# tiems90/mosaic

Measured on AMD Instinct MI355X. Metric: PIP-join points/sec (H3 res 9) at 1/2/4/8 GPUs + achieved HBM GB/s, higher is better.
Workload: dtype f64

## Files before the change

include/mosaic_gpu.h:

```cpp
#ifndef MOSAIC_GPU_H
#define MOSAIC_GPU_H

#include <stdint.h>

#ifdef __cplusplus
extern "C" {
#endif

#define MGPU_OK 0
#define MGPU_E_INVALID_ARG -1
#define MGPU_E_RESOLUTION -2
#define MGPU_E_NAN -3
#define MGPU_E_WKB -4
#define MGPU_E_CAPACITY -5
#define MGPU_E_DEVICE -6
#define MGPU_E_INTERNAL -7
#define MGPU_E_UNSUPPORTED -8
#define MGPU_E_EMPTY -9

#define MGPU_H3 0
#define MGPU_BNG 1

typedef struct mgpu_ctx mgpu_ctx;
typedef struct mgpu_chips mgpu_chips;
// ... 88 lines not shown

int32_t mgpu_grid_polyfill(mgpu_ctx* ctx, int32_t index_system, int32_t res, int64_t n_polys,
                           const int64_t* poly_part_off, const int64_t* part_ring_off, const int64_t* ring_off,
                           const double* xy, int64_t* out_cells, int64_t capacity, int64_t* out_offsets,
                           int64_t* out_total, void* stream);

int32_t mgpu_chips_upload(mgpu_ctx* ctx, int32_t index_system, int64_t n_chips, const int64_t* cell,
                          const int32_t* polygon_id, const uint8_t* is_core, const int64_t* wkb_offsets,
                          const uint8_t* wkb, mgpu_chips** out);
int32_t mgpu_chips_destroy(mgpu_chips* chips);
int32_t mgpu_chips_device_blob(const mgpu_chips* chips, void** device_ptr, int64_t* bytes);
int32_t mgpu_chips_from_device_blob(mgpu_ctx* ctx, const void* device_ptr, int64_t bytes, mgpu_chips** out);
int32_t mgpu_chips_info(const mgpu_chips* chips, int64_t* n_chips, int64_t* n_cells, int64_t* n_vertices);
int32_t mgpu_chips_raster_info(const mgpu_chips* chips, int64_t* mode, int64_t* n_classes);
int32_t mgpu_chips_polygons(const mgpu_chips* chips, int32_t* out_ids, int64_t cap, int64_t* out_n);

int32_t mgpu_chips_host_blob(int32_t index_system, int64_t n_chips, const int64_t* cell, const int32_t* polygon_id,
                             const uint8_t* is_core, const int64_t* wkb_offsets, const uint8_t* wkb, uint8_t** out,
                             int64_t* bytes);
int32_t mgpu_chips_host_blob_ex(int32_t index_system, int64_t n_chips, const int64_t* cell, const int32_t* polygon_id,
                                const uint8_t* is_core, const int64_t* wkb_offsets, const uint8_t* wkb,
                                const mgpu_build_opts* opts, uint8_t** out, int64_t* bytes);
int32_t mgpu_host_free(void* p);
int32_t mgpu_host_blob_info(const void* host_blob, int64_t bytes, int32_t* index_system, int64_t* n_chips,
                            int64_t* n_cells, int64_t* n_vertices);
int32_t mgpu_chips_upload_blob(mgpu_ctx* ctx, const void* host_blob, int64_t bytes, mgpu_chips** out);

#define MGPU_COMM_ID_BYTES 128
int32_t mgpu_comm_unique_id(uint8_t* out_id);
int32_t mgpu_comm_init(mgpu_ctx* ctx, const uint8_t* unique_id, int32_t rank, int32_t world);
int32_t mgpu_comm_info(mgpu_ctx* ctx, int32_t* rank, int32_t* world);
int32_t mgpu_comm_destroy(mgpu_ctx* ctx);
int32_t mgpu_chips_broadcast(mgpu_ctx* ctx, const mgpu_chips* chips, int32_t root, mgpu_chips** out, void* stream);
int32_t mgpu_pair_offsets(mgpu_ctx* ctx, int64_t local_pairs, int64_t* out_offset, int64_t* out_total,
                          int64_t* out_counts, void* stream);
int32_t mgpu_test_receive_blob(mgpu_ctx* ctx, const void* dev_blob, int32_t fail_alloc, mgpu_chips** out);

int32_t mgpu_ring_join(mgpu_ctx* ctx, int32_t index_system, int32_t res, int32_t k, int32_t loop_only,
                       const double* left_x, const double* left_y, int64_t n_left, const double* right_x,
                       const double* right_y, int64_t n_right, int64_t left_id_base, int32_t max_per_left,
                       double max_distance, int64_t capacity, int64_t* out_n, int64_t* out_left, int64_t* out_right,
                       double* out_dist, void* stream);
#define MGPU_RING_LEFT_OUTER 1
int32_t mgpu_ring_join_ex(mgpu_ctx* ctx, int32_t index_system, int32_t res, int32_t k, int32_t loop_only,
                          const double* left_x, const double* left_y, int64_t n_left, const double* right_x,
                          const double* right_y, int64_t n_right, int64_t left_id_base, int32_t max_per_left,
                          double max_distance, int32_t flags, int64_t capacity, int64_t* out_n, int64_t* out_left,
                          int64_t* out_right, double* out_dist, void* stream);
int32_t mgpu_ring_join_final(mgpu_ctx* ctx, int32_t index_system, int32_t res, const double* left_x,
                             const double* left_y, const double* radius, const int32_t* k_iterated, int64_t n_left,
                             const double* right_x, const double* right_y, int64_t n_right, int64_t left_id_base,
                             int32_t max_per_left, double max_distance, int32_t flags, int64_t capacity,
                             int64_t* out_n, int64_t* out_left, int64_t* out_right, double* out_dist, void* stream);

int32_t mgpu_st_contains(mgpu_ctx* ctx, const mgpu_chips* chips, const int64_t* chip_row,
                         const double* x, const double* y, int64_t n, int8_t* out, void* stream);

int32_t mgpu_pip_join(mgpu_ctx* ctx, const mgpu_chips* chips, int32_t index_system, int32_t res,
                      const double* x, const double* y, const int64_t* point_id, int64_t point_id_base,
                      int64_t n, int64_t capacity, int64_t* out_n_pairs, int64_t* out_point_id,
                      int32_t* out_polygon_id, void* stream, mgpu_stats* stats);

int32_t mgpu_pip_join_fetch(mgpu_ctx* ctx, int64_t capacity, int64_t* out_n_pairs, int64_t* out_point_id,
                            int32_t* out_polygon_id, void* stream);

int32_t mgpu_pip_join_count(mgpu_ctx* ctx, const mgpu_chips* chips, int32_t index_system, int32_t res,
                            const double* x, const double* y, const int64_t* weight, int64_t n, int64_t n_slots,
                            int64_t* count, int64_t* sum, int32_t accumulate, void* stream, mgpu_stats* stats);

int32_t mgpu_pip_join_lookup(mgpu_ctx* ctx, const mgpu_chips* chips, int32_t index_system, int32_t res,
                             const double* x, const double* y, int64_t n, int32_t null_id,
                             int32_t* out_polygon, int32_t* out_matches, void* stream, mgpu_stats* stats);

typedef struct mgpu_cell_agg mgpu_cell_agg;
int32_t mgpu_cell_agg_create(mgpu_ctx* ctx, int32_t index_system, int32_t res, int32_t with_sum,
                             int64_t initial_cells, mgpu_cell_agg** out);
int32_t mgpu_cell_agg_add_points(mgpu_ctx* ctx, mgpu_cell_agg* agg, const double* x, const double* y,
                                 const int64_t* weight, int64_t n, void* stream, mgpu_stats* stats);
int32_t mgpu_cell_agg_add_cells(mgpu_ctx* ctx, mgpu_cell_agg* agg, const int64_t* cells, const uint8_t* valid,
                                int64_t valid_offset, const int64_t* weight, int64_t n, void* stream);
int32_t mgpu_cell_agg_add_counted(mgpu_ctx* ctx, mgpu_cell_agg* agg, const int64_t* cells, const int64_t* count,
                                  const int64_t* sum, int64_t n, void* stream);
int32_t mgpu_cell_agg_size(mgpu_ctx* ctx, const mgpu_cell_agg* agg, int64_t* n_cells, void* stream);
int32_t mgpu_cell_agg_fetch(mgpu_ctx* ctx, const mgpu_cell_agg* agg, int64_t capacity, int64_t* out_cell,
                            int64_t* out_count, int64_t* out_sum, int64_t* out_n, void* stream);
int32_t mgpu_cell_agg_clear(mgpu_ctx* ctx, mgpu_cell_agg* agg, void* stream);
int32_t mgpu_cell_agg_destroy(mgpu_cell_agg* agg);

int32_t mgpu_pip_join_async(mgpu_ctx* ctx, const mgpu_chips* chips, int32_t index_system, int32_t res,
                            const double* x, const double* y, const int64_t* point_id, int64_t point_id_base,
                            int64_t n, int64_t capacity, int64_t* d_n_pairs, int64_t* out_point_id,
                            int32_t* out_polygon_id, void* stream);
int32_t mgpu_pip_join_finish(mgpu_ctx* ctx, int64_t* out_n_pairs, mgpu_stats* stats);
int32_t mgpu_ctx_reserve(mgpu_ctx* ctx, int64_t max_points);

int32_t mgpu_last_near_ties(mgpu_ctx* ctx, int64_t* out_index, int64_t cap, int64_t* out_n);

int32_t mgpu_pip_join_host(mgpu_ctx* ctx, const mgpu_chips* chips, int32_t index_system, int32_t res,
                           const double* x, const double* y, const int64_t* point_id, int64_t n,
                           int64_t capacity, int64_t* out_n_pairs, int64_t* out_point_id,
                           int32_t* out_polygon_id);

typedef struct mgpu_tess mgpu_tess;
int32_t mgpu_tessellate(int32_t index_system, int32_t res, int64_t n_polys, const int32_t* polygon_id,
                        const int64_t* poly_part_off, const int64_t* part_ring_off, const int64_t* ring_off,
                        const double* xy, int32_t keep_core_geometries, mgpu_tess** out);
#define MGPU_CORE_MOSAICFILL 0
#define MGPU_CORE_CLIP 1
#define MGPU_CORE_DISTANCE 2
int32_t mgpu_tessellate_ex(int32_t index_system, int32_t res, int64_t n_polys, const int32_t* polygon_id,
                           const int64_t* poly_part_off, const int64_t* part_ring_off, const int64_t* ring_off,
                           const double* xy, int32_t keep_core_geometries, int32_t core_rule, mgpu_tess** out);
#define MGPU_CHIPS_OVERLAY 0
#define MGPU_CHIPS_SUTHERLAND_HODGMAN 1
int32_t mgpu_tessellate_geom(int32_t index_system, int32_t res, int64_t n_polys, const int32_t* polygon_id,
                             const int64_t* poly_part_off, const int64_t* part_ring_off, const int64_t* ring_off,
                             const double* xy, const uint8_t* poly_type, int32_t keep_core_geometries,
                             int32_t core_rule, int32_t chip_geometry, mgpu_tess** out);
int32_t mgpu_tess_result_stats(const mgpu_tess* t, int64_t* out6);
int32_t mgpu_tess_result_core_stats(const mgpu_tess* t, int64_t* out, int32_t n);
int32_t mgpu_tess_result_sizes(const mgpu_tess* t, int64_t* n_chips, int64_t* wkb_bytes);
int32_t mgpu_tess_result_copy(const mgpu_tess* t, int64_t* cell, int32_t* polygon_id, uint8_t* is_core,
                              int64_t* wkb_offsets, uint8_t* wkb);
int32_t mgpu_tess_result_undecided(const mgpu_tess* t, int64_t* n, int64_t* wkb_bytes, int64_t* cell, int32_t* poly,
                                   uint8_t* kind_kept_core, int64_t* wkb_offsets, uint8_t* wkb);
int32_t mgpu_tess_destroy(mgpu_tess* t);

int32_t mgpu_test_chip_contains_host(int32_t index_system, int64_t n_chips, const int64_t* cell,
                                     const int32_t* polygon_id, const uint8_t* is_core, const int64_t* wkb_offsets,
                                     const uint8_t* wkb, int64_t n, const int64_t* chip_row, const double* x,
                                     const double* y, int8_t* out_join_path, int8_t* out_point_locator);

int32_t mgpu_test_overlay_verify(int32_t on, int64_t* out2);

int32_t mgpu_test_parse_number(const char* s, int32_t len, double* out);
int32_t mgpu_test_h3_elementary_host(int32_t fn, const double* a, const double* b, int64_t n, double* out);
int32_t mgpu_test_h3_route_host(const double* lon, const double* lat, int64_t n, int32_t res, int64_t* out_cell);
int32_t mgpu_test_h3_glibc_host(const double* lon, const double* lat, int64_t n, int32_t res, int64_t* out_cell);
int32_t mgpu_test_h3_boundary_host(const int64_t* cells, int64_t n, double* out_lonlat, int32_t* out_nverts,
                                   double* out_center);
int32_t mgpu_test_cell_geometry_host(int32_t index_system, const int64_t* cells, int64_t n, double* out_xy,
                                     int32_t* out_nverts, double* out_center, double* out_area);
int32_t mgpu_test_grid_polyfill_host(int32_t index_system, int32_t res, int64_t n_polys, const int64_t* poly_part_off,
                                     const int64_t* part_ring_off, const int64_t* ring_off, const double* xy,
                                     int64_t* out_cells, int64_t capacity, int64_t* out_offsets, int64_t* out_total);
int32_t mgpu_test_grid_polyfill_last(int64_t* out8);
int32_t mgpu_test_geometry_kring_host(int32_t index_system, int64_t n_geoms, const int64_t* row_off, const int64_t* cell,
                                      const uint8_t* is_core, int32_t k, int32_t loop_only, int64_t* out_cells,
                                      int64_t capacity, int64_t* out_offsets, int64_t* out_total);
int32_t mgpu_test_geometry_kring_last(int64_t* out8);
int32_t mgpu_test_h3_cell_wkb_host(int64_t cell, uint8_t* out, int64_t cap, int64_t* out_len);
int32_t mgpu_test_decode_point(int32_t format, const uint8_t* data, int64_t len, double* x, double* y);
int32_t mgpu_test_join_counters(mgpu_ctx* ctx, uint64_t* out16);
int32_t mgpu_test_poly_slots_host(const int32_t* polygon_id, int64_t n, int32_t* out_ids, int64_t* out_n,
                                  uint32_t* out_slot_of_row);

int32_t mgpu_test_internal_centroid(int64_t n, const int32_t* type_id, const int64_t* row_part, const int64_t* part_ring,
                                    const int64_t* ring_off, const double* xy, double* x, double* y, int32_t* status);

int32_t mgpu_test_blob_contains_host(const void* host_blob, int64_t bytes, int64_t n, const int64_t* chip_row,
                                     const double* x, const double* y, int8_t* out);

int32_t mgpu_test_raster_host(int32_t index_system, int32_t res, int64_t n_chips, const int64_t* cell,
                              const int32_t* polygon_id, const uint8_t* is_core, const int64_t* wkb_offsets,
                              const uint8_t* wkb, int64_t n, const double* x, const double* y, int8_t* out_kind,
                              uint32_t* out_first, uint32_t* out_mask, int32_t* out_chip_poly);

int32_t mgpu_test_cell_answers_host(int32_t index_system, int32_t res, int64_t n_chips, const int64_t* cell,
                                    const int32_t* polygon_id, const uint8_t* is_core, const int64_t* wkb_offsets,
                                    const uint8_t* wkb, int64_t n, const double* x, const double* y, int8_t* out_kind,
                                    uint32_t* out_first, uint32_t* out_mask, int32_t* out_chip_poly);

int32_t mgpu_test_whole_cells_host(int32_t index_system, int32_t res, int64_t n_chips, const int64_t* cell,
                                   const int32_t* polygon_id, const uint8_t* is_core, const int64_t* wkb_offsets,
                                   const uint8_t* wkb, int64_t n, const double* x, const double* y, int8_t* out_kind,
                                   uint32_t* out_first, uint32_t* out_mask, int32_t* out_chip_poly);

#ifdef __cplusplus
}
#endif

#endif
```

mosaic_amd/_native.py:

```python
import ctypes
import os

_HERE = os.path.dirname(os.path.abspath(__file__))
LIB_PATH = os.environ.get("MOSAIC_AMD_LIB") or os.path.join(_HERE, "libmosaic_gpu.so")

MGPU_OK = 0
MGPU_E_INVALID_ARG = -1
MGPU_E_RESOLUTION = -2
MGPU_E_NAN = -3
MGPU_E_WKB = -4
MGPU_E_CAPACITY = -5
MGPU_RING_LEFT_OUTER = 1
MGPU_E_DEVICE = -6
MGPU_E_INTERNAL = -7
MGPU_E_UNSUPPORTED = -8
MGPU_E_EMPTY = -9

MGPU_H3 = 0
MGPU_BNG = 1

EXPORTS = (
    "mgpu_last_error", "mgpu_version", "mgpu_join_tile_points", "mgpu_ctx_create", "mgpu_ctx_destroy", "mgpu_check_resolution",
    "mgpu_points_to_cells", "mgpu_points_to_cells_host", "mgpu_bng_format", "mgpu_bng_parse",
    "mgpu_bng_format_device", "mgpu_format_cells_device", "mgpu_grid_kring",
    "mgpu_chips_upload", "mgpu_chips_destroy", "mgpu_chips_device_blob", "mgpu_chips_from_device_blob",
    "mgpu_chips_info", "mgpu_st_contains", "mgpu_pip_join", "mgpu_pip_join_async", "mgpu_pip_join_finish", "mgpu_ctx_reserve",
    "mgpu_last_near_ties",    "mgpu_pip_join_host", "mgpu_tessellate", "mgpu_tess_result_sizes", "mgpu_tess_result_copy", "mgpu_tessellate_ex", "mgpu_tessellate_geom", "mgpu_tess_result_undecided", "mgpu_tess_result_stats", "mgpu_tess_result_core_stats",
    "mgpu_tess_destroy", "mgpu_test_chip_contains_host", "mgpu_test_raster_host", "mgpu_test_cell_answers_host", "mgpu_test_whole_cells_host", "mgpu_pip_join_fetch",
    "mgpu_chips_host_blob", "mgpu_host_free", "mgpu_host_blob_info", "mgpu_chips_upload_blob",
    "mgpu_comm_unique_id", "mgpu_comm_init", "mgpu_comm_info", "mgpu_comm_destroy", "mgpu_chips_broadcast",
    "mgpu_pair_offsets", "mgpu_test_blob_contains_host", "mgpu_points_from_geometry", "mgpu_geometry_to_cells",
    "mgpu_geometry_to_cells_arrow", "mgpu_pip_join_arrow", "mgpu_test_parse_number", "mgpu_test_decode_point",
    "mgpu_test_h3_elementary_host", "mgpu_test_h3_route_host", "mgpu_test_h3_boundary_host", "mgpu_test_h3_cell_wkb_host",
    "mgpu_ctx_set_option", "mgpu_ctx_get_option", "mgpu_build_opts_default", "mgpu_chips_host_blob_ex",
    "mgpu_test_h3_glibc_host", "mgpu_internal_geometry_to_cells", "mgpu_test_internal_centroid", "mgpu_test_join_counters",
    "mgpu_test_receive_blob", "mgpu_ring_join", "mgpu_ring_join_ex", "mgpu_ring_join_final",
    "mgpu_test_overlay_verify",
    "mgpu_chips_polygons", "mgpu_pip_join_count", "mgpu_test_poly_slots_host", "mgpu_chips_raster_info",
    "mgpu_pip_join_lookup",
    "mgpu_cell_agg_create", "mgpu_cell_agg_add_points", "mgpu_cell_agg_add_cells", "mgpu_cell_agg_add_counted",
    "mgpu_cell_agg_size", "mgpu_cell_agg_fetch", "mgpu_cell_agg_clear", "mgpu_cell_agg_destroy",
    "mgpu_cells_to_centers", "mgpu_cells_to_boundaries", "mgpu_cells_boundary_wkb", "mgpu_cells_area",
    "mgpu_test_cell_geometry_host",
    "mgpu_grid_polyfill", "mgpu_test_grid_polyfill_last", "mgpu_test_grid_polyfill_host",
    "mgpu_geometry_kring", "mgpu_test_geometry_kring_host", "mgpu_test_geometry_kring_last",
)
MGPU_GEOM_WKB = 0
MGPU_GEOM_WKT = 1
MGPU_GEOM_HEX = 2
MGPU_GEOM_GEOJSON = 3
MGPU_COMM_ID_BYTES = 128
MGPU_PIPELINE_AUTO = -1
MGPU_PIPELINE_FUSED = 0
MGPU_PIPELINE_SPLIT = 1
MGPU_PIPELINE_BINNED = 2
MGPU_LIBM_REFERENCE = 0
MGPU_LIBM_CORRECTLY_ROUNDED = 1


class MosaicGpuError(RuntimeError):

    def __init__(self, code, msg):
        super().__init__("%s (status %d)" % (msg, code))
        self.code = code


class IllegalArgumentException(MosaicGpuError, ValueError):
    pass


class IllegalStateException(MosaicGpuError):
    pass


class CapacityError(MosaicGpuError):
    def __init__(self, code, msg, required):
        super().__init__(code, msg)
        self.required = required


class MgpuStats(ctypes.Structure):
    _fields_ = [("n_points", ctypes.c_int64), ("n_pairs", ctypes.c_int64), ("n_near_ties", ctypes.c_int64),
                ("n_candidates", ctypes.c_int64), ("kernel_ms", ctypes.c_float),
                ("stream_kernel_ms", ctypes.c_float), ("mixed_kernel_ms", ctypes.c_float),
                ("emit_kernel_ms", ctypes.c_float), ("pipeline", ctypes.c_int32), ("libm_overrides", ctypes.c_int32)]

    def as_dict(self):
        return {k: getattr(self, k) for k, _ in self._fields_}


class BuildOpts(ctypes.Structure):
    _fields_ = [("raster", ctypes.c_int32), ("raster_bng", ctypes.c_int32), ("raster_sub", ctypes.c_int32),
                ("raster_milli", ctypes.c_int32)]


_lib = None

P = ctypes.c_void_p
I32 = ctypes.c_int32
I64 = ctypes.c_int64


def lib():
    global _lib
    if _lib is not None:
        return _lib
    if not os.path.exists(LIB_PATH):
        raise RuntimeError("mosaic_amd/libmosaic_gpu.so is not built: run `python -c 'import __graft_entry__ as g; "
                           "g.build()'` (the HIP path has no CPU fallback)")
    L = ctypes.CDLL(LIB_PATH)
    sig = {
        "mgpu_last_error": (ctypes.c_char_p, []),
        "mgpu_version": (ctypes.c_char_p, []),
        "mgpu_join_tile_points": (ctypes.c_int32, []),
        "mgpu_ctx_create": (I32, [I32, ctypes.POINTER(P)]),
        "mgpu_ctx_destroy": (I32, [P]),
        "mgpu_check_resolution": (I32, [I32, I32]),
        "mgpu_points_to_cells": (I32, [P, I32, I32, P, P, I64, P, P, ctypes.POINTER(MgpuStats)]),
        "mgpu_points_to_cells_host": (I32, [P, I32, I32, P, P, I64, P]),
        "mgpu_bng_format": (I32, [P, I64, P, I64, P]),
        "mgpu_bng_format_device": (I32, [P, P, I64, P, I64, P, ctypes.POINTER(I64), P]),
        "mgpu_format_cells_device": (I32, [P, I32, P, I64, P, I64, P, ctypes.POINTER(I64), P]),
        "mgpu_grid_kring": (I32, [P, I32, P, I64, I32, I32, P, I64, P, ctypes.POINTER(I64), P]),
        "mgpu_bng_parse": (I32, [P, P, I64, P]),
        "mgpu_chips_upload": (I32, [P, I32, I64, P, P, P, P, P, ctypes.POINTER(P)]),
        "mgpu_chips_destroy": (I32, [P]),
        "mgpu_chips_device_blob": (I32, [P, ctypes.POINTER(P), ctypes.POINTER(I64)]),
        "mgpu_chips_from_device_blob": (I32, [P, P, I64, ctypes.POINTER(P)]),
        "mgpu_chips_info": (I32, [P, ctypes.POINTER(I64), ctypes.POINTER(I64), ctypes.POINTER(I64)]),
        "mgpu_chips_raster_info": (I32, [P, ctypes.POINTER(I64), ctypes.POINTER(I64)]),
        "mgpu_st_contains": (I32, [P, P, P, P, P, I64, P, P]),
        "mgpu_pip_join": (I32, [P, P, I32, I32, P, P, P, I64, I64, I64, ctypes.POINTER(I64), P, P, P,
                                ctypes.POINTER(MgpuStats)]),
        "mgpu_pip_join_async": (I32, [P, P, I32, I32, P, P, P, I64, I64, I64, P, P, P, P]),
        "mgpu_pip_join_finish": (I32, [P, ctypes.POINTER(I64), ctypes.POINTER(MgpuStats)]),
        "mgpu_ctx_reserve": (I32, [P, I64]),
        "mgpu_last_near_ties": (I32, [P, P, I64, ctypes.POINTER(I64)]),
        "mgpu_pip_join_host": (I32, [P, P, I32, I32, P, P, P, I64, I64, ctypes.POINTER(I64), P, P]),
        "mgpu_tessellate": (I32, [I32, I32, I64, P, P, P, P, P, I32, ctypes.POINTER(P)]),
        "mgpu_tessellate_ex": (I32, [I32, I32, I64, P, P, P, P, P, I32, I32, ctypes.POINTER(P)]),
        "mgpu_tessellate_geom": (I32, [I32, I32, I64, P, P, P, P, P, P, I32, I32, I32, ctypes.POINTER(P)]),
        "mgpu_tess_result_undecided": (I32, [P, P, P, P, P, P, P, P]),
        "mgpu_tess_result_stats": (I32, [P, P]),
        "mgpu_tess_result_core_stats": (I32, [P, P, I32]),
        "mgpu_tess_result_sizes": (I32, [P, ctypes.POINTER(I64), ctypes.POINTER(I64)]),
        "mgpu_tess_result_copy": (I32, [P, P, P, P, P, P]),
        "mgpu_tess_destroy": (I32, [P]),
        "mgpu_test_chip_contains_host": (I32, [I32, I64, P, P, P, P, P, I64, P, P, P, P, P]),
        "mgpu_pip_join_fetch": (I32, [P, I64, ctypes.POINTER(I64), P, P, P]),
        "mgpu_test_raster_host": (I32, [I32, I32, I64, P, P, P, P, P, I64, P, P, P, P, P, P]),
        "mgpu_test_cell_answers_host": (I32, [I32, I32, I64, P, P, P, P, P, I64, P, P, P, P, P, P]),
        "mgpu_test_whole_cells_host": (I32, [I32, I32, I64, P, P, P, P, P, I64, P, P, P, P, P, P]),
        "mgpu_chips_host_blob": (I32, [I32, I64, P, P, P, P, P, ctypes.POINTER(P), ctypes.POINTER(I64)]),
        "mgpu_host_free": (I32, [P]),
        "mgpu_host_blob_info": (I32, [P, I64, ctypes.POINTER(I32), ctypes.POINTER(I64), ctypes.POINTER(I64),
                                      ctypes.POINTER(I64)]),
        "mgpu_chips_upload_blob": (I32, [P, P, I64, ctypes.POINTER(P)]),
        "mgpu_comm_unique_id": (I32, [P]),
        "mgpu_comm_init": (I32, [P, P, I32, I32]),
        "mgpu_comm_info": (I32, [P, ctypes.POINTER(I32), ctypes.POINTER(I32)]),
        "mgpu_comm_destroy": (I32, [P]),
        "mgpu_chips_broadcast": (I32, [P, P, I32, ctypes.POINTER(P), P]),
        "mgpu_pair_offsets": (I32, [P, I64, ctypes.POINTER(I64), ctypes.POINTER(I64), P, P]),
        "mgpu_test_blob_contains_host": (I32, [P, I64, I64, P, P, P, P]),
        "mgpu_points_from_geometry": (I32, [P, I32, P, P, P, I64, I64, P, P, P]),
        "mgpu_geometry_to_cells": (I32, [P, I32, I32, I32, P, P, P, I64, I64, P, P, P, ctypes.POINTER(MgpuStats)]),
        "mgpu_geometry_to_cells_arrow": (I32, [P, I32, I32, P, P, P, P, P]),
        "mgpu_pip_join_arrow": (I32, [P, P, I32, I32, P, P, P, I64, ctypes.POINTER(I64), P, P, P,
                                      ctypes.POINTER(MgpuStats)]),
        "mgpu_test_parse_number": (I32, [ctypes.c_char_p, I32, ctypes.POINTER(ctypes.c_double)]),
        "mgpu_test_decode_point": (I32, [I32, P, I64, ctypes.POINTER(ctypes.c_double), ctypes.POINTER(ctypes.c_double)]),
        "mgpu_test_h3_elementary_host": (I32, [I32, P, P, I64, P]),
        "mgpu_test_h3_route_host": (I32, [P, P, I64, I32, P]),
        "mgpu_test_h3_boundary_host": (I32, [P, I64, P, P, P]),
        "mgpu_test_overlay_verify": (I32, [ctypes.c_int32, P]),
        "mgpu_test_h3_cell_wkb_host": (I32, [I64, P, I64, P]),
        "mgpu_ctx_set_option": (I32, [P, ctypes.c_char_p, I64]),
        "mgpu_ctx_get_option": (I32, [P, ctypes.c_char_p, ctypes.POINTER(I64)]),
        "mgpu_build_opts_default": (None, [ctypes.POINTER(BuildOpts)]),
        "mgpu_chips_host_blob_ex": (I32, [I32, I64, P, P, P, P, P, ctypes.POINTER(BuildOpts), ctypes.POINTER(P),
                                          ctypes.POINTER(I64)]),
        "mgpu_test_h3_glibc_host": (I32, [P, P, I64, I32, P]),
        "mgpu_internal_geometry_to_cells": (I32, [P, I32, I32, I64, P, P, P, P, P, P, I64, P, P, P,
                                                  ctypes.POINTER(MgpuStats)]),
        "mgpu_test_internal_centroid": (I32, [I64, P, P, P, P, P, P, P, P]),
        "mgpu_test_join_counters": (I32, [P, P]),
        "mgpu_test_receive_blob": (I32, [P, P, I32, ctypes.POINTER(P)]),
        "mgpu_chips_polygons": (I32, [P, P, I64, ctypes.POINTER(I64)]),
        "mgpu_pip_join_count": (I32, [P, P, I32, I32, P, P, P, I64, I64, P, P, I32, P, ctypes.POINTER(MgpuStats)]),
        "mgpu_pip_join_lookup": (I32, [P, P, I32, I32, P, P, I64, I32, P, P, P, ctypes.POINTER(MgpuStats)]),
        "mgpu_test_poly_slots_host": (I32, [P, I64, P, ctypes.POINTER(I64), P]),
        "mgpu_cell_agg_create": (I32, [P, I32, I32, I32, I64, ctypes.POINTER(P)]),
        "mgpu_cell_agg_add_points": (I32, [P, P, P, P, P, I64, P, ctypes.POINTER(MgpuStats)]),
        "mgpu_cell_agg_add_cells": (I32, [P, P, P, P, I64, P, I64, P]),
        "mgpu_cell_agg_add_counted": (I32, [P, P, P, P, P, I64, P]),
        "mgpu_cell_agg_size": (I32, [P, P, ctypes.POINTER(I64), P]),
        "mgpu_cell_agg_fetch": (I32, [P, P, I64, P, P, P, ctypes.POINTER(I64), P]),
        "mgpu_cell_agg_clear": (I32, [P, P, P]),
        "mgpu_cell_agg_destroy": (I32, [P]),
        "mgpu_cells_to_centers": (I32, [P, I32, P, P, I64, I64, P, P, P, P]),
        "mgpu_cells_to_boundaries": (I32, [P, I32, P, P, I64, I64, P, P, P, P]),
        "mgpu_cells_boundary_wkb": (I32, [P, I32, P, P, I64, I64, P, I64, P, ctypes.POINTER(I64), P, P]),
        "mgpu_cells_area": (I32, [P, I32, P, P, I64, I64, P, P, P]),
        "mgpu_test_cell_geometry_host": (I32, [I32, P, I64, P, P, P, P]),
        "mgpu_grid_polyfill": (I32, [P, I32, I32, I64, P, P, P, P, P, I64, P, ctypes.POINTER(I64), P]),
        "mgpu_test_grid_polyfill_last": (I32, [P]),
        "mgpu_test_grid_polyfill_host": (I32, [I32, I32, I64, P, P, P, P, P, I64, P, ctypes.POINTER(I64)]),
        "mgpu_geometry_kring": (I32, [P, I32, I64, P, P, P, I32, I32, P, I64, P, ctypes.POINTER(I64), P]),
        "mgpu_test_geometry_kring_host": (I32, [I32, I64, P, P, P, I32, I32, P, I64, P, ctypes.POINTER(I64)]),
        "mgpu_test_geometry_kring_last": (I32, [P]),
        "mgpu_ring_join": (I32, [P, I32, I32, I32, I32, P, P, I64, P, P, I64, I64, I32, ctypes.c_double, I64,
                                 ctypes.POINTER(I64), P, P, P, P]),
        "mgpu_ring_join_ex": (I32, [P, I32, I32, I32, I32, P, P, I64, P, P, I64, I64, I32, ctypes.c_double, I32,
                                    I64, ctypes.POINTER(I64), P, P, P, P]),
        "mgpu_ring_join_final": (I32, [P, I32, I32, P, P, P, P, I64, P, P, I64, I64, I32, ctypes.c_double, I32, I64,
                                       ctypes.POINTER(I64), P, P, P, P]),
    }
    for name, (rt, args) in sig.items():
        f = getattr(L, name)
        f.restype = rt
        f.argtypes = args
    _lib = L
    return L


def last_error():
    m = lib().mgpu_last_error()
    return m.decode() if m else ""


def check(status, what="", required=None):
    if status == MGPU_OK:
        return
    msg = last_error() or what
    if status == MGPU_E_CAPACITY:
        raise CapacityError(status, msg, required)
    if status in (MGPU_E_RESOLUTION, MGPU_E_NAN, MGPU_E_INTERNAL, MGPU_E_EMPTY):
        raise IllegalStateException(status, msg)
    if status in (MGPU_E_INVALID_ARG, MGPU_E_WKB):
        raise IllegalArgumentException(status, msg)
    raise MosaicGpuError(status, msg)
```

mosaic_amd/chips.py:

```python
import ctypes

import numpy as np

from . import _native as N


class ChipTable:

    def __init__(self, cell, polygon_id, is_core, wkb_offsets, wkb, index_system=N.MGPU_H3):
        self.cell = np.ascontiguousarray(cell, dtype=np.int64)
        self.polygon_id = np.ascontiguousarray(polygon_id, dtype=np.int32)
        self.is_core = np.ascontiguousarray(is_core, dtype=np.uint8)
        self.wkb_offsets = np.ascontiguousarray(wkb_offsets, dtype=np.int64)
        self.wkb = np.ascontiguousarray(np.frombuffer(wkb, dtype=np.uint8) if isinstance(wkb, (bytes, bytearray))
                                        else wkb, dtype=np.uint8)
        self.index_system = int(index_system)
        n = self.cell.shape[0]
        assert self.polygon_id.shape[0] == n and self.is_core.shape[0] == n and self.wkb_offsets.shape[0] == n + 1

    def __len__(self):
        return self.cell.shape[0]

    def row(self, i):
        b, e = self.wkb_offsets[i], self.wkb_offsets[i + 1]
        return (bool(self.is_core[i]), int(self.cell[i]), bytes(self.wkb[b:e]) if e > b else None,
                int(self.polygon_id[i]))

    @classmethod
    def from_rows(cls, rows, index_system=N.MGPU_H3):
        rows = list(rows)
        blobs = [r[2] or b"" for r in rows]
        off = np.zeros(len(rows) + 1, dtype=np.int64)
        off[1:] = np.cumsum([len(b) for b in blobs])
        return cls([r[1] for r in rows], [r[3] for r in rows], [1 if r[0] else 0 for r in rows], off,
                   np.frombuffer(b"".join(blobs) or b"", dtype=np.uint8), index_system)

    def upload(self, ctx=None):
        from .context import default_context
        return DeviceChips(self, ctx or default_context())

    def stats(self):
        return {"chips": len(self), "core": int(self.is_core.sum()), "cells": int(np.unique(self.cell).shape[0]),
                "wkb_bytes": int(self.wkb_offsets[-1])}


class DeviceChips:

    def __init__(self, table, ctx, handle=None):
        self.ctx = ctx
        self.table = table
        if handle is None:
            h = ctypes.c_void_p()
            wkb = table.wkb if table.wkb.size else np.zeros(1, np.uint8)
            N.check(N.lib().mgpu_chips_upload(ctx.handle, table.index_system, len(table), table.cell.ctypes.data,
                                              table.polygon_id.ctypes.data, table.is_core.ctypes.data,
                                              table.wkb_offsets.ctypes.data, wkb.ctypes.data, ctypes.byref(h)))
            handle = h
        self.handle = handle

    @classmethod
    def from_device_blob(cls, ctx, ptr, nbytes, table=None):
        h = ctypes.c_void_p()
        N.check(N.lib().mgpu_chips_from_device_blob(ctx.handle, ptr, int(nbytes), ctypes.byref(h)))
        return cls(table, ctx, handle=h)

    def device_blob(self):
        p = ctypes.c_void_p()
        b = ctypes.c_int64()
        N.check(N.lib().mgpu_chips_device_blob(self.handle, ctypes.byref(p), ctypes.byref(b)))
        return p.value, b.value

    def info(self):
        a, b, c = ctypes.c_int64(), ctypes.c_int64(), ctypes.c_int64()
        N.check(N.lib().mgpu_chips_info(self.handle, ctypes.byref(a), ctypes.byref(b), ctypes.byref(c)))
        p, n = self.device_blob()
        m, k = ctypes.c_int64(), ctypes.c_int64()
        N.check(N.lib().mgpu_chips_raster_info(self.handle, ctypes.byref(m), ctypes.byref(k)))
        return {"chips": a.value, "cells": b.value, "vertices": c.value, "bytes": n, "raster_mode": m.value,
                "raster_ncls": k.value}

    def polygons(self):
        if getattr(self, "_polygons", None) is not None:
            return self._polygons
        n = ctypes.c_int64()
        st = N.lib().mgpu_chips_polygons(self.handle, None, 0, ctypes.byref(n))
        if st != N.MGPU_E_CAPACITY:
            N.check(st)
        ids = np.zeros(n.value, np.int32)
        N.check(N.lib().mgpu_chips_polygons(self.handle, ids.ctypes.data, n.value, ctypes.byref(n)))
        ids.setflags(write=False)
        self._polygons = ids
        return ids

    def polygons_device(self):
        import torch
        if getattr(self, "_polygons_dev", None) is None:
            self._polygons_dev = torch.from_numpy(self.polygons().copy()).to(self.ctx.device)
        return self._polygons_dev

    def close(self):
        if self.handle:
            N.lib().mgpu_chips_destroy(self.handle)
            self.handle = None

    def __del__(self):
        try:
            self.close()
        except Exception:
            pass


class Polygons:

    def __init__(self, poly_id, poly_part_off, part_ring_off, ring_off, xy, poly_type=None):
        self.poly_id = np.ascontiguousarray(poly_id, dtype=np.int32)
        self.poly_part_off = np.ascontiguousarray(poly_part_off, dtype=np.int64)
        self.part_ring_off = np.ascontiguousarray(part_ring_off, dtype=np.int64)
        self.ring_off = np.ascontiguousarray(ring_off, dtype=np.int64)
        self.xy = np.ascontiguousarray(xy, dtype=np.float64).reshape(-1, 2)
        self.poly_type = None if poly_type is None else np.ascontiguousarray(poly_type, dtype=np.uint8)
        assert self.poly_type is None or self.poly_type.shape[0] == self.poly_id.shape[0]

    def __len__(self):
        return self.poly_id.shape[0]

    @classmethod
    def from_npz(cls, path):
        z = np.load(path, allow_pickle=False)
        return cls(z["poly_id"], z["poly_part_off"], z["part_ring_off"], z["ring_off"], z["xy"],
                   z["poly_type"] if "poly_type" in z.files else None)

    @classmethod
    def from_lists(cls, polys, poly_type=None):
        ids, pp, pr, ro, xy = [], [0], [0], [0], []
        for pid, parts in polys:
            ids.append(pid)
            for part in parts:
                for ring in part:
                    xy.extend(ring)
                    ro.append(len(xy))
                pr.append(len(ro) - 1)
            pp.append(len(pr) - 1)
        return cls(ids, pp, pr, ro, np.array(xy, dtype=np.float64).reshape(-1, 2), poly_type)

    def select(self, idx):
        out = []
        for p in idx:
            parts = []
            for q in range(self.poly_part_off[p], self.poly_part_off[p + 1]):
                rings = []
                for r in range(self.part_ring_off[q], self.part_ring_off[q + 1]):
                    rings.append([tuple(v) for v in self.xy[self.ring_off[r]:self.ring_off[r + 1]]])
                parts.append(rings)
            out.append((int(self.poly_id[p]), parts))
        return Polygons.from_lists(out, None if self.poly_type is None else self.poly_type[list(idx)])

    def bounds(self):
        return self.xy[:, 0].min(), self.xy[:, 1].min(), self.xy[:, 0].max(), self.xy[:, 1].max()


CORE_RULES = {"mosaicfill": 0, "clip": 1, "distance": 2}
CORE_STATS = ("rows", "core", "demoted", "promoted", "dropped", "ambiguous", "carved_tests", "band_tests",
              "core_below_r", "border_above_r", "band_dropped", "dp_sensitive", "unresolved", "carved_empty",
              "overlay_chips", "multi_piece", "coerced", "coerce_nodes", "lower_dim")
CHIP_GEOMETRY = {"overlay": 0, "sutherland_hodgman": 1}


def tessellate(polygons, index_system, resolution, keep_core_geometries=True, core_rule="mosaicfill",
               chip_geometry="overlay"):
    res = index_system.get_resolution(resolution)
    L = N.lib()
    h = ctypes.c_void_p()
    p = polygons
    st = L.mgpu_tessellate_geom(index_system.code, res, len(p), p.poly_id.ctypes.data, p.poly_part_off.ctypes.data,
                                p.part_ring_off.ctypes.data, p.ring_off.ctypes.data, p.xy.ctypes.data,
                                None if p.poly_type is None else p.poly_type.ctypes.data,
                                1 if keep_core_geometries else 0, CORE_RULES[core_rule],
                                CHIP_GEOMETRY[chip_geometry], ctypes.byref(h))
    N.check(st, "tessellation failed")
    try:
        stats = np.zeros(len(CORE_STATS), np.int64)
        N.check(L.mgpu_tess_result_core_stats(h, stats.ctypes.data, len(CORE_STATS)))
        n, b = ctypes.c_int64(), ctypes.c_int64()
        N.check(L.mgpu_tess_result_sizes(h, ctypes.byref(n), ctypes.byref(b)))
        cell = np.zeros(n.value, np.int64)
        pid = np.zeros(n.value, np.int32)
        core = np.zeros(n.value, np.uint8)
        off = np.zeros(n.value + 1, np.int64)
        wkb = np.zeros(max(b.value, 1), np.uint8)
        N.check(L.mgpu_tess_result_copy(h, cell.ctypes.data, pid.ctypes.data, core.ctypes.data, off.ctypes.data,
                                        wkb.ctypes.data))
        nu, ub = ctypes.c_int64(), ctypes.c_int64()
        N.check(L.mgpu_tess_result_undecided(h, ctypes.byref(nu), ctypes.byref(ub), None, None, None, None, None))
        ucell, upoly = np.zeros(nu.value, np.int64), np.zeros(nu.value, np.int32)
        ukkc, uoff, uwkb = np.zeros((nu.value, 3), np.uint8), np.zeros(nu.value + 1, np.int64), np.zeros(max(ub.value, 1), np.uint8)
        N.check(L.mgpu_tess_result_undecided(h, ctypes.byref(nu), ctypes.byref(ub), ucell.ctypes.data, upoly.ctypes.data,
                                             ukkc.ctypes.data, uoff.ctypes.data, uwkb.ctypes.data))
    finally:
        L.mgpu_tess_destroy(h)
    t = ChipTable(cell, pid, core, off, wkb[:b.value], index_system.code)
    t.core_stats = dict(zip(CORE_STATS, stats.tolist()))
    t.undecided = ChipTable(ucell, upoly, ukkc[:, 2], uoff, uwkb[:ub.value], index_system.code)
    t.undecided.kind, t.undecided.kept = ukkc[:, 0].copy(), ukkc[:, 1].copy()
    return t
```

mosaic_amd/csrc/capi.cpp:

```cpp
#include <hip/hip_runtime.h>

#include <algorithm>
#include <cmath>
#include <cstdarg>
#include <cstdio>
#include <cstring>
#include <cstdlib>
#include <string>
#include <memory>
#include <functional>
#include <mutex>
#include <vector>

#include "../../include/mosaic_arrow.h"
#include "../../include/mosaic_gpu.h"
#include "error.h"
#include "h3_core.h"
#include "kernels.h"
#include "parallel.h"
#include "poly_slots.h"
#include "capi_internal.h"
#include "chip_build.h"
#include "geom_decode.h"
#include "h3_glibc.h"
// ... 111 lines not shown
  }
  return hipStreamSynchronize(s);
}

struct TieRec {
  int64_t pos;
  double x, y;
  uint64_t key;
};

int32_t read_ties(mgpu_ctx* ctx, int64_t n, std::vector<TieRec>& out) {
  out.resize((size_t)n);
  const uint64_t* head = ctx->pin + 16;
  const int64_t nh = std::min(n, kTqHead);
  if (nh) memcpy(out.data(), head + 2, (size_t)nh * 32);
  if (n > nh) HIP_TRY(hipMemcpy(out.data() + nh, ctx->tq + 2 + 4 * nh, (size_t)(n - nh) * 32, hipMemcpyDeviceToHost));
  return MGPU_OK;
}

std::vector<std::pair<int64_t, uint64_t>> libm_reference_keys(std::vector<TieRec>& ties, int res) {
  std::sort(ties.begin(), ties.end(), [](const TieRec& a, const TieRec& b) { return a.pos < b.pos; });
  std::vector<std::pair<int64_t, uint64_t>> out(ties.size());
  mgpu::parallel_for((int64_t)ties.size(), 256, [&](int64_t b, int64_t e, int) {
    for (int64_t k = b; k < e; k++) out[k] = {ties[k].pos, mgpu::h3glibc::lattice_key(ties[k].x, ties[k].y, res)};
  });
  return out;
}

std::vector<std::pair<int64_t, uint64_t>> libm_second_opinion(const std::vector<TieRec>& ties, int res, bool cells) {
  std::vector<uint64_t> ref(ties.size());
  mgpu::parallel_for((int64_t)ties.size(), 256, [&](int64_t b, int64_t e, int) {
    for (int64_t k = b; k < e; k++)
      ref[k] = cells ? mgpu::h3glibc::point_to_cell(ties[k].x, ties[k].y, res)
                     : mgpu::h3glibc::lattice_key(ties[k].x, ties[k].y, res);
  });
  std::vector<std::pair<int64_t, uint64_t>> diff;
  for (size_t k = 0; k < ties.size(); k++)
    if (ref[k] != ties[k].key) diff.push_back({ties[k].pos, ref[k]});
  std::sort(diff.begin(), diff.end());
  return diff;
}

int32_t check_res(int32_t is, int32_t res) {
  if (is == MGPU_H3) {
    if (res < 0 || res > 15) return fail(MGPU_E_RESOLUTION, "H3 resolution has to be between 0 and 15; found %d", res);
    return MGPU_OK;
  }
  if (is == MGPU_BNG) {
    if (res == 0 || res < -6 || res > 6) return fail(MGPU_E_RESOLUTION, "BNG resolution not supported; found %d", res);
    return MGPU_OK;
  }
  return fail(MGPU_E_INVALID_ARG, "unknown index system %d (0 = H3, 1 = BNG)", is);
}

int32_t set_device(int dev) {
  HIP_TRY(hipSetDevice(dev));
  return MGPU_OK;
}

}

namespace mgpu {
int32_t begin_call(mgpu_ctx* ctx) {
  if (int32_t st = set_device(ctx->device)) return st;
  return ensure_ws(ctx, 1);
}
}

extern "C" {

const char* mgpu_last_error(void) { return g_err.c_str(); }
const char* mgpu_version(void) { return "mosaic-mi355x 0.1.0 (gfx950)"; }
int32_t mgpu_join_tile_points(void) { return (int32_t)mgpu::join_tile_points(); }

int32_t mgpu_check_resolution(int32_t index_system, int32_t res) { return check_res(index_system, res); }

int32_t mgpu_ctx_create(int32_t device_id, mgpu_ctx** out) {
  if (!out) return fail(MGPU_E_INVALID_ARG, "out is NULL");
  int n = 0;
  HIP_TRY(hipGetDeviceCount(&n));
  if (device_id < 0 || device_id >= n) return fail(MGPU_E_INVALID_ARG, "device %d not present (%d GPUs)", device_id, n);
  HIP_TRY(hipSetDevice(device_id));
  mgpu_ctx* c = new mgpu_ctx();
  c->device = device_id;
  int32_t st = MGPU_OK;
  if (hipEventCreate(&c->ev0) != hipSuccess || hipEventCreate(&c->ev1) != hipSuccess ||
      hipEventCreate(&c->ev2) != hipSuccess || hipEventCreate(&c->ev3) != hipSuccess ||
      hipHostMalloc((void**)&c->pin, kPinWords * 8, hipHostMallocDefault) != hipSuccess)
    st = fail(MGPU_E_DEVICE, "mgpu_ctx_create: events / pinned page");
  if (!st && hipHostGetDevicePointer((void**)&c->pin_dev, c->pin, 0) != hipSuccess)
    st = fail(MGPU_E_DEVICE, "mgpu_ctx_create: the pinned page is not device-visible");
  if (!st) st = ensure_ws(c, 1);
  if (!st) st = ensure_tq(c, kTqInit);
  if (st) {
    mgpu_ctx_destroy(c);
    return st;
  }
  *out = c;
  return MGPU_OK;
}

int32_t mgpu_ctx_destroy(mgpu_ctx* ctx) {
  if (!ctx) return MGPU_OK;
  mgpu_comm_destroy(ctx);
  hipSetDevice(ctx->device);
  if (ctx->split_ws) hipFree(ctx->split_ws);
  if (ctx->bin_ws) hipFree(ctx->bin_ws);
  if (ctx->scratch) hipFree(ctx->scratch);
  if (ctx->redo) hipFree(ctx->redo);
  if (ctx->tq) hipFree(ctx->tq);
  if (ctx->ovr) hipFree(ctx->ovr);
  if (ctx->ws) hipFree(ctx->ws);
  if (ctx->pin) hipHostFree(ctx->pin);
  if (ctx->ev0) hipEventDestroy(ctx->ev0);
  if (ctx->ev1) hipEventDestroy(ctx->ev1);
  if (ctx->ev2) hipEventDestroy(ctx->ev2);
  if (ctx->ev3) hipEventDestroy(ctx->ev3);
  delete ctx;
  return MGPU_OK;
}

int32_t mgpu_ctx_set_option(mgpu_ctx* ctx, const char* key, int64_t v) {
  if (!ctx || !key) return fail(MGPU_E_INVALID_ARG, "ctx/key is NULL");
  mgpu_options& o = ctx->opt;
  const std::string k = key;
  auto bad = [&]() { return fail(MGPU_E_INVALID_ARG, "option %s: value %lld out of range", key, (long long)v); };
  if (k == "h3_libm") {
    if (v != MGPU_LIBM_REFERENCE && v != MGPU_LIBM_CORRECTLY_ROUNDED) return bad();
    o.h3_libm = v;
  } else if (k == "pipeline") {
    if (v < MGPU_PIPELINE_AUTO || v > MGPU_PIPELINE_BINNED) return bad();
    o.pipeline = v;
  } else if (k == "bin_count") {
    if (v < 1 || v > mgpu::bin_max()) return bad();
    o.bin_count = v;
  } else if (k == "bin_min_mb") {
    if (v < 0) return bad();
    o.bin_min_mb = v;
  } else if (k == "bin_min_points") {
    if (v < 0) return bad();
    o.bin_min_points = v;
  } else if (k == "bin_xcd") {
    if (v != 0 && v != 1) return bad();
    o.bin_xcd = v;
  } else if (k == "bin_keys") {
    if (v != 0 && v != 1) return bad();
    o.bin_keys = v;
  } else if (k == "ring_batch") {
    if (v < 1) return bad();
    o.ring_batch = v;
  } else if (k == "bng_split") {
    if (v != 0 && v != 1) return bad();
    o.bng_split = v;
  } else if (k == "count_lds_slots") {
    if (v < 0 || v > mgpu::kCountLdsSlotsMax) return bad();
    o.count_lds_slots = v;
  } else if (k == "count_groups") {
    if (v < 0 || v > mgpu::kCountGroupsMax) return bad();
    o.count_groups = v;
  } else if (k == "cellagg_groups") {
    if (v < 0 || v > mgpu::kCountGroupsMax) return bad();
    o.cellagg_groups = v;
  } else if (k == "cellagg_bin_min") {
    if (v < 0) return bad();
    o.cellagg_bin_min = v;
  } else if (k == "cellagg_lds") {
    if (v != 0 && v != 1) return bad();
    o.cellagg_lds = v;
  } else if (k == "kring_batch") {
    if (v < 0 || v > 2147483647LL) return bad();
    o.kring_batch = v;
  } else if (k == "polyfill_slab") {
    if (v < 256 || v > ((int64_t)1 << 28)) return bad();
    o.polyfill_slab = v;
  } else if (k == "geomring_slab") {
    if (v < 1 || v > ((int64_t)1 << 24)) return bad();
    o.geomring_slab = v;
  } else if (k == "geomring_lds_slots") {
    if (v != 0 && v < 64) return bad();
    o.geomring_lds_slots = v;
  } else if (k == "spin_us") {
    if (v < 0 || v > 10000000) return bad();
    o.spin_us = v;
  } else if (k == "raster" || k == "raster_bng") {
    if (v != 0 && v != 1) return bad();
    (k == "raster" ? o.raster : o.raster_bng) = v;
  } else if (k == "raster_sub") {
    if (!(v == 0 || (v >= 2 && v <= 16))) return bad();
    o.raster_sub = v;
  } else if (k == "raster_milli") {
    if (v < 10 || v > 1000) return bad();
    o.raster_milli = v;
  } else {
    return fail(MGPU_E_INVALID_ARG, "unknown option %s", key);
  }
  return MGPU_OK;
}

int32_t mgpu_ctx_get_option(const mgpu_ctx* ctx, const char* key, int64_t* v) {
  if (!ctx || !key || !v) return fail(MGPU_E_INVALID_ARG, "NULL argument");
  const mgpu_options& o = ctx->opt;
  const std::pair<const char*, int64_t> all[] = {
      {"h3_libm", o.h3_libm},       {"pipeline", o.pipeline}, {"bin_count", o.bin_count},
      {"bin_min_mb", o.bin_min_mb}, {"bin_min_points", o.bin_min_points}, {"bin_xcd", o.bin_xcd},
      {"bin_keys", o.bin_keys},     {"spin_us", o.spin_us},   {"ring_batch", o.ring_batch},       {"raster", o.raster},     {"raster_bng", o.raster_bng},
      {"bng_split", o.bng_split},   {"count_lds_slots", o.count_lds_slots}, {"count_groups", o.count_groups},
      {"kring_batch", o.kring_batch}, {"cellagg_groups", o.cellagg_groups}, {"cellagg_lds", o.cellagg_lds}, {"cellagg_bin_min", o.cellagg_bin_min},
      {"raster_sub", o.raster_sub}, {"raster_milli", o.raster_milli}, {"polyfill_slab", o.polyfill_slab},
      {"geomring_slab", o.geomring_slab}, {"geomring_lds_slots", o.geomring_lds_slots}};
  for (const auto& kv : all)
    if (strcmp(kv.first, key) == 0) {
      *v = kv.second;
      return MGPU_OK;
    }
  return fail(MGPU_E_INVALID_ARG, "unknown option %s", key);
}

int32_t mgpu_ctx_reserve(mgpu_ctx* ctx, int64_t max_points) {
  if (!ctx) return fail(MGPU_E_INVALID_ARG, "ctx is NULL");
  if (int32_t st = set_device(ctx->device)) return st;
  const int64_t tiles = mgpu::join_tiles(max_points);
  return ensure_ws(ctx, tiles, max_points);
}

}

int32_t cells_impl(mgpu_ctx* ctx, int32_t is, int32_t res, const double* x, const double* y, int64_t n,
                          int64_t* out_cell, hipStream_t s, const uint8_t* valid, int64_t voff, mgpu_stats* stats) {
  auto* counters = (unsigned long long*)ctx->ws;
  auto* ties = (unsigned long long*)((uint8_t*)ctx->ws + ws_layout(1, 0).ties);
  int64_t n_ties = 0, n_fixed = 0;
  for (int attempt = 0;; attempt++) {
    HIP_TRY(hipMemsetAsync(counters, 0, kWsCounters, s));
    HIP_TRY(hipMemsetAsync(ties, 0, 8, s));
    HIP_TRY(hipMemsetAsync(ctx->tq, 0, 16, s));
    HIP_TRY(hipEventRecord(ctx->ev0, s));
    HIP_TRY(mgpu::launch_cells(is, res, x, y, n, out_cell, counters, ties, kTieCap, ctx->tq, ctx->tq_cap, s, valid, voff));
    HIP_TRY(hipEventRecord(ctx->ev1, s));
    HIP_TRY(hipMemcpyAsync(ctx->pin, counters, 16 * 8, hipMemcpyDeviceToHost, s));
    HIP_TRY(hipMemcpyAsync(ctx->pin + 16, ctx->tq, (2 + 4 * kTqHead) * 8, hipMemcpyDeviceToHost, s));
    HIP_TRY(stream_wait(ctx, s));
    if (ctx->pin[2]) {
      if (is == MGPU_BNG) return fail(MGPU_E_NAN, "NaN coordinates are not supported. (%llu points)", (unsigned long long)ctx->pin[2]);
      return fail(MGPU_E_INVALID_ARG, "Latitude or longitude were invalid. (%llu points)", (unsigned long long)ctx->pin[2]);
    }
    n_ties = (int64_t)ctx->pin[16];
    if (n_ties > ctx->tq_cap) {
      if (attempt >= 2) return fail(MGPU_E_INTERNAL, "near-tie queue overflowed twice");
      if (int32_t st = ensure_tq(ctx, n_ties + n_ties / 4 + 1024)) return st;
      continue;
    }
    break;
  }
  if (stats) {
    memset(stats, 0, sizeof *stats);
    stats->n_points = n;
    stats->n_near_ties = n_ties;
    float ms = 0;
    hipEventElapsedTime(&ms, ctx->ev0, ctx->ev1);
    stats->kernel_ms = stats->stream_kernel_ms = ms;
  }
  if (is == MGPU_H3 && n_ties > 0 && ctx->opt.h3_libm == MGPU_LIBM_REFERENCE) {
    std::vector<TieRec> tr;
    if (int32_t st = read_ties(ctx, n_ties, tr)) return st;
    const auto diff = libm_second_opinion(tr, res, true);
    n_fixed = (int64_t)diff.size();
    if (n_fixed) {
      std::vector<int64_t> hv(2 * diff.size());
      for (size_t k = 0; k < diff.size(); k++) hv[k] = diff[k].first, hv[diff.size() + k] = (int64_t)diff[k].second;
      if (int32_t st = ensure_ovr(ctx, (int64_t)hv.size())) return st;
      HIP_TRY(hipMemcpyAsync(ctx->ovr, hv.data(), hv.size() * 8, hipMemcpyHostToDevice, s));
      HIP_TRY(mgpu::launch_scatter_i64((const int64_t*)ctx->ovr, (const int64_t*)ctx->ovr + n_fixed, n_fixed, out_cell, s));
      HIP_TRY(stream_wait(ctx, s));
    }
  }
  if (stats) stats->libm_overrides = (int32_t)n_fixed;
  return MGPU_OK;
}

extern "C" {

int32_t mgpu_points_to_cells(mgpu_ctx* ctx, int32_t is, int32_t res, const double* x, const double* y, int64_t n,
                             int64_t* out_cell, void* stream, mgpu_stats* stats) {
  if (!ctx) return fail(MGPU_E_INVALID_ARG, "ctx is NULL");
  if (int32_t r = check_res(is, res)) return r;
  if (n < 0 || (n > 0 && (!x || !y || !out_cell))) return fail(MGPU_E_INVALID_ARG, "bad point arrays");
  if (int32_t st = set_device(ctx->device)) return st;
  if (int32_t st = ensure_ws(ctx, 1)) return st;
  return cells_impl(ctx, is, res, x, y, n, out_cell, (hipStream_t)stream, nullptr, 0, stats);
}

int32_t mgpu_format_cells_device(mgpu_ctx* ctx, int32_t index_system, const int64_t* cells, int64_t n, char* out,
                                 int64_t out_bytes, int64_t* out_offsets, int64_t* out_total, void* stream) {
  if (!ctx || n < 0 || (n > 0 && (!cells || !out)) || !out_offsets || out_bytes < 0)
    return fail(MGPU_E_INVALID_ARG, "format_cells_device: bad arguments");
  if (index_system != MGPU_H3 && index_system != MGPU_BNG)
    return fail(MGPU_E_INVALID_ARG, "unknown index system %d (0 = H3, 1 = BNG)", index_system);
  if (int32_t st = set_device(ctx->device)) return st;
  hipStream_t s = (hipStream_t)stream;
  if (int32_t st = ensure_ws(ctx, mgpu::join_tiles(n))) return st;
  auto* counters = (unsigned long long*)ctx->ws;
  auto* chunk = (int64_t*)((uint8_t*)ctx->ws + ws_layout(mgpu::join_tiles(n), 0).where);
  HIP_TRY(hipMemsetAsync(counters, 0, kWsCounters, s));
  HIP_TRY(mgpu::launch_format_cells(index_system, cells, n, out, out_bytes, out_offsets, chunk, counters, s));
  unsigned long long h[4] = {0};
  int64_t total = 0;
  HIP_TRY(hipMemcpyAsync(h, counters, sizeof h, hipMemcpyDeviceToHost, s));
  HIP_TRY(hipMemcpyAsync(&total, out_offsets + n, sizeof total, hipMemcpyDeviceToHost, s));
  HIP_TRY(hipStreamSynchronize(s));
  if (out_total) *out_total = total;
  if (h[2]) return fail(MGPU_E_INVALID_ARG, "%llu BNG cell ids have no string form", h[2]);
  if (total > out_bytes) return fail(MGPU_E_CAPACITY, "format_cells_device: %lld bytes needed, %lld given",
                                     (long long)total, (long long)out_bytes);
  return MGPU_OK;
}

int32_t mgpu_grid_kring(mgpu_ctx* ctx, int32_t index_system, const int64_t* cells, int64_t n, int32_t k,
                        int32_t loop_only, int64_t* out_cells, int64_t capacity, int64_t* out_offsets,
                        int64_t* out_total, void* stream) {
  if (!ctx || n < 0 || (n > 0 && !cells) || !out_offsets || capacity < 0 || (capacity > 0 && !out_cells))
    return fail(MGPU_E_INVALID_ARG, "grid_kring: bad arguments");
  if (index_system != MGPU_BNG && index_system != MGPU_H3)
    return fail(MGPU_E_INVALID_ARG, "grid_kring: unknown index system %d", index_system);
  if (k < 0 || k > 1024) return fail(MGPU_E_INVALID_ARG, "grid_kring: k must be in [0, 1024]");
  if (int32_t st = set_device(ctx->device)) return st;
  hipStream_t s = (hipStream_t)stream;
  if (int32_t st = ensure_ws(ctx, mgpu::join_tiles(n))) return st;
  const WsLayout L = ws_layout(mgpu::join_tiles(n), 0);
  auto* base = (uint8_t*)ctx->ws;
  auto* counters = (unsigned long long*)base;
  auto* chunk = (int64_t*)(base + L.where);
  auto* mc = (int64_t*)(base + L.recs);
  auto* fb_idx = (uint32_t*)(base + L.recs + (size_t)std::max<int64_t>(n, 1) * 8);
  HIP_TRY(hipMemsetAsync(counters, 0, kWsCounters, s));
  HIP_TRY(mgpu::launch_kring_count(index_system, cells, n, k, loop_only, mc, chunk, fb_idx, counters, s));
  unsigned long long h[6] = {0};
  HIP_TRY(hipMemcpyAsync(h, counters, sizeof h, hipMemcpyDeviceToHost, s));
  HIP_TRY(hipStreamSynchronize(s));
  if (h[2] && index_system == MGPU_H3)
    return fail(MGPU_E_INVALID_ARG, "%llu cells are not H3 cell ids", h[2]);
  if (h[2])
    return fail(MGPU_E_INVALID_ARG, "%llu cells are not BNG cells or reach ids BNGIndexSystem.isValid cannot parse "
                "(NumberFormatException in the reference)", h[2]);
  const int64_t n_fb = (int64_t)h[3];
  uint64_t* scratch = nullptr;
  struct Free {
    uint64_t*& p;
    ~Free() {
      if (p) hipFree(p);
    }
  } free_scratch{scratch};
  int64_t batch = 0;
  if (n_fb) {
    const int64_t words = mgpu::kring_fallback_words(k);
    batch = std::max<int64_t>(1, std::min<int64_t>(n_fb, ((int64_t)256 << 20) / 8 / words));
    if (ctx->opt.kring_batch > 0) batch = std::min(batch, ctx->opt.kring_batch);
    HIP_TRY(hipMalloc(&scratch, (size_t)batch * words * 8));
    for (int64_t j0 = 0; j0 < n_fb; j0 += batch)
      HIP_TRY(mgpu::launch_kring_fallback(cells, fb_idx, j0, std::min(n_fb, j0 + batch), k, loop_only, mc, chunk,
                                          out_offsets, out_cells, capacity, scratch, 0, counters, s));
  }
  HIP_TRY(mgpu::launch_kring_write(index_system, cells, n, k, loop_only, mc, chunk, out_offsets, out_cells, capacity,
                                   s));
  for (int64_t j0 = 0; j0 < n_fb; j0 += batch)
    HIP_TRY(mgpu::launch_kring_fallback(cells, fb_idx, j0, std::min(n_fb, j0 + batch), k, loop_only, mc, chunk,
                                        out_offsets, out_cells, capacity, scratch, 1, counters, s));
  int64_t total = 0;
  HIP_TRY(hipMemcpyAsync(h, counters, sizeof h, hipMemcpyDeviceToHost, s));
  HIP_TRY(hipMemcpyAsync(&total, out_offsets + n, sizeof total, hipMemcpyDeviceToHost, s));
  HIP_TRY(hipStreamSynchronize(s));
  if (out_total) *out_total = total;
  if (h[4])
    return fail(MGPU_E_INTERNAL, "grid_kring: %llu pentagon walks overflowed their hash set (inconsistent tables)", h[4]);
  if (total > capacity)
    return fail(MGPU_E_CAPACITY, "grid_kring: %lld ids, capacity %lld", (long long)total, (long long)capacity);
  return MGPU_OK;
}

int32_t mgpu_bng_format_device(mgpu_ctx* ctx, const int64_t* cells, int64_t n, char* out, int64_t out_bytes,
                               int64_t* out_offsets, int64_t* out_total, void* stream) {
  return mgpu_format_cells_device(ctx, MGPU_BNG, cells, n, out, out_bytes, out_offsets, out_total, stream);
}

int32_t mgpu_points_to_cells_host(mgpu_ctx* ctx, int32_t is, int32_t res, const double* x, const double* y, int64_t n,
                                  int64_t* out_cell) {
  if (!ctx) return fail(MGPU_E_INVALID_ARG, "ctx is NULL");
  if (n == 0) return check_res(is, res);
  if (int32_t st = set_device(ctx->device)) return st;
  double *dx = nullptr, *dy = nullptr;
  int64_t* dc = nullptr;
  HIP_TRY(hipMalloc(&dx, n * 8));
  HIP_TRY(hipMalloc(&dy, n * 8));
  HIP_TRY(hipMalloc(&dc, n * 8));
  HIP_TRY(hipMemcpy(dx, x, n * 8, hipMemcpyHostToDevice));
  HIP_TRY(hipMemcpy(dy, y, n * 8, hipMemcpyHostToDevice));
  int32_t st = mgpu_points_to_cells(ctx, is, res, dx, dy, n, dc, nullptr, nullptr);
  if (st == MGPU_OK) HIP_TRY(hipMemcpy(out_cell, dc, n * 8, hipMemcpyDeviceToHost));
  hipFree(dx);
  hipFree(dy);
  hipFree(dc);
  return st;
}


}

static mgpu_build_opts build_opts_of(const mgpu_ctx* ctx) {
  mgpu_build_opts o;
  o.raster = (int32_t)ctx->opt.raster;
  o.raster_bng = (int32_t)ctx->opt.raster_bng;
  o.raster_sub = (int32_t)ctx->opt.raster_sub;
  o.raster_milli = (int32_t)ctx->opt.raster_milli;
  return o;
}

namespace mgpu {
int32_t adopt_device_blob(mgpu_ctx* ctx, void* dev_blob, int64_t bytes, mgpu_chips** out) {
  BlobHeader hdr;
  HIP_TRY(hipMemcpy(&hdr, dev_blob, sizeof hdr, hipMemcpyDeviceToHost));
  if (int32_t st = check_header(hdr, bytes)) return st;
  mgpu_chips* ch = new mgpu_chips();
  ch->device = ctx->device;
  ch->blob = dev_blob;
  ch->bytes = (size_t)bytes;
  ch->index_system = hdr.index_system;
  ch->view = view_from_header(hdr, (uint8_t*)ch->blob);
  ch->n_vertices = hdr.n_vertices;
  *out = ch;
  return MGPU_OK;
}
}

struct PolySlotsDev {
  std::vector<int32_t> ids;
  int32_t* d_ids = nullptr;
  uint32_t* d_chip_slot = nullptr;
  uint32_t* d_dense = nullptr;
};

static std::mutex g_slots_mu;

static void free_poly_slots(mgpu_chips* chips) {
  auto* ps = (PolySlotsDev*)chips->slots;
  if (!ps) return;
  if (ps->d_ids) hipFree(ps->d_ids);
  if (ps->d_chip_slot) hipFree(ps->d_chip_slot);
  if (ps->d_dense) hipFree(ps->d_dense);
  delete ps;
  chips->slots = nullptr;
}

static int32_t ensure_poly_slots(const mgpu_chips* chips, const PolySlotsDev** out) {
  std::lock_guard<std::mutex> lock(g_slots_mu);
  if (chips->slots) {
    *out = (const PolySlotsDev*)chips->slots;
    return MGPU_OK;
  }
  if (int32_t st = set_device(chips->device)) return st;
  const int64_t nch = chips->view.n_chips;
  std::vector<int32_t> poly((size_t)nch);
  if (nch) HIP_TRY(hipMemcpy(poly.data(), chips->view.chip_poly, (size_t)nch * 4, hipMemcpyDeviceToHost));
  mgpu::PolySlots hs = mgpu::poly_slots(poly.data(), nch);
  auto ps = std::make_unique<PolySlotsDev>();
  auto upload = [&](auto** d, const void* src, size_t bytes) -> hipError_t {
    if (hipError_t e = hipMalloc((void**)d, std::max<size_t>(bytes, 4))) return e;
    return bytes ? hipMemcpy(*d, src, bytes, hipMemcpyHostToDevice) : hipSuccess;
  };
  hipError_t e = upload(&ps->d_ids, hs.ids.data(), hs.ids.size() * 4);
  if (e == hipSuccess) e = upload(&ps->d_chip_slot, hs.slot_of_row.data(), hs.slot_of_row.size() * 4);
  if (e == hipSuccess && mgpu::poly_slots_dense(hs.ids)) {
    std::vector<uint32_t> dense((size_t)((int64_t)hs.ids.back() - hs.ids.front() + 1), 0u);
    for (size_t k = 0; k < hs.ids.size(); k++) dense[(size_t)((int64_t)hs.ids[k] - hs.ids.front())] = (uint32_t)k;
    e = upload(&ps->d_dense, dense.data(), dense.size() * 4);
  }
  if (e != hipSuccess) {
    if (ps->d_ids) hipFree(ps->d_ids);
    if (ps->d_chip_slot) hipFree(ps->d_chip_slot);
    if (ps->d_dense) hipFree(ps->d_dense);
    return fail(MGPU_E_DEVICE, "polygon slots: %s", hipGetErrorString(e));
  }
  ps->ids = std::move(hs.ids);
  chips->slots = ps.release();
  *out = (const PolySlotsDev*)chips->slots;
  return MGPU_OK;
}

static hipError_t stage_to_device(void* d, size_t bytes, const std::function<void(uint8_t*, size_t, size_t)>& fill) {
  constexpr size_t kPiece = (size_t)64 << 20;
  if (bytes <= 2 * kPiece) {
    std::vector<uint8_t> tmp(bytes);
    mgpu::parallel_for((int64_t)((bytes + (1 << 20) - 1) >> 20), 1, [&](int64_t b, int64_t en, int) {
      const size_t lo = (size_t)b << 20, hi = std::min(bytes, (size_t)en << 20);
      fill(tmp.data() + lo, lo, hi - lo);
    });
    return hipMemcpy(d, tmp.data(), bytes, hipMemcpyHostToDevice);
  }
  void* stage[2] = {nullptr, nullptr};
  hipEvent_t done[2] = {nullptr, nullptr};
  hipStream_t s = nullptr;
  hipError_t e = hipStreamCreateWithFlags(&s, hipStreamNonBlocking);
  for (int k = 0; k < 2 && e == hipSuccess; k++) {
    e = hipHostMalloc(&stage[k], kPiece, hipHostMallocDefault);
    if (e == hipSuccess) e = hipEventCreateWithFlags(&done[k], hipEventDisableTiming);
  }
  for (size_t off = 0, k = 0; off < bytes && e == hipSuccess; off += kPiece, k ^= 1) {
    const size_t n = std::min(kPiece, bytes - off);
    if (off >= 2 * kPiece) e = hipEventSynchronize(done[k]);
    if (e != hipSuccess) break;
    auto* dst = (uint8_t*)stage[k];
    mgpu::parallel_for((int64_t)((n + (1 << 20) - 1) >> 20), 1, [&](int64_t b, int64_t en, int) {
      const size_t lo = (size_t)b << 20, hi = std::min(n, (size_t)en << 20);
      fill(dst + lo, off + lo, hi - lo);
    });
    e = hipMemcpyAsync((uint8_t*)d + off, stage[k], n, hipMemcpyHostToDevice, s);
    if (e == hipSuccess) e = hipEventRecord(done[k], s);
  }
  if (s) {
    const hipError_t e2 = hipStreamSynchronize(s);
    if (e == hipSuccess) e = e2;
    hipStreamDestroy(s);
  }
  for (int k = 0; k < 2; k++) {
    if (done[k]) hipEventDestroy(done[k]);
    if (stage[k]) hipHostFree(stage[k]);
  }
  return e;
}

extern "C" {

int32_t mgpu_chips_upload_blob(mgpu_ctx* ctx, const void* host_blob, int64_t bytes, mgpu_chips** out) {
  if (!ctx || !out) return fail(MGPU_E_INVALID_ARG, "ctx/out is NULL");
  if (int32_t st = mgpu_host_blob_info(host_blob, bytes, nullptr, nullptr, nullptr, nullptr)) return st;
  if (int32_t st = set_device(ctx->device)) return st;
  void* d = nullptr;
  HIP_TRY(hipMalloc(&d, (size_t)bytes));
  hipError_t e = stage_to_device(d, (size_t)bytes, [&](uint8_t* dst, size_t off, size_t n) {
    memcpy(dst, (const uint8_t*)host_blob + off, n);
  });
  if (e != hipSuccess) {
    hipFree(d);
    return fail(MGPU_E_DEVICE, "hipMemcpy: %s", hipGetErrorString(e));
  }
  int32_t st = mgpu::adopt_device_blob(ctx, d, bytes, out);
  if (st) hipFree(d);
  return st;
}

int32_t mgpu_chips_upload(mgpu_ctx* ctx, int32_t index_system, int64_t n_chips, const int64_t* cell,
                          const int32_t* polygon_id, const uint8_t* is_core, const int64_t* wkb_offsets,
                          const uint8_t* wkb, mgpu_chips** out) {
  if (!ctx || !out) return fail(MGPU_E_INVALID_ARG, "ctx/out is NULL");
  mgpu::HostBlob host;
  mgpu::BlobHeader hdr;
  if (int32_t st = set_device(ctx->device)) return st;
  void* d = nullptr;
  size_t bytes = 0;
  const mgpu::BlobSink sink = [&](size_t total, const std::vector<mgpu::BlobPiece>& pieces) -> int32_t {
    BLOB_T0();
    HIP_TRY(hipMalloc(&d, total));
    BLOB_MARK("sink:malloc");
    bytes = total;
    const hipError_t e = stage_to_device(d, total, [&](uint8_t* dst, size_t off, size_t n) {
      mgpu::fill_from_pieces(pieces, dst, off, n);
    });
    if (e != hipSuccess) return fail(MGPU_E_DEVICE, "hipMemcpy: %s", hipGetErrorString(e));
    return MGPU_OK;
  };
  BLOB_T0();
  int32_t st = mgpu::build_blob(index_system, n_chips, cell, polygon_id, is_core, wkb_offsets, wkb, host, hdr,
                                build_opts_of(ctx), &sink);
  BLOB_MARK("upl:build");
  if (st == MGPU_OK) st = mgpu::adopt_device_blob(ctx, d, (int64_t)bytes, out);
  BLOB_MARK("upl:adopt");
  if (st && d) hipFree(d);
  return st;
}

int32_t mgpu_chips_destroy(mgpu_chips* chips) {
  if (!chips) return MGPU_OK;
  hipSetDevice(chips->device);
  if (chips->blob) hipFree(chips->blob);
  free_poly_slots(chips);
  delete chips;
  return MGPU_OK;
}

int32_t mgpu_chips_info(const mgpu_chips* chips, int64_t* n_chips, int64_t* n_cells, int64_t* n_vertices) {
  if (!chips) return fail(MGPU_E_INVALID_ARG, "chips is NULL");
  if (n_chips) *n_chips = chips->view.n_chips;
  if (n_cells) *n_cells = chips->view.n_cells;
  if (n_vertices) *n_vertices = chips->n_vertices;
  return MGPU_OK;
}

int32_t mgpu_chips_raster_info(const mgpu_chips* chips, int64_t* mode, int64_t* n_classes) {
  if (!chips) return fail(MGPU_E_INVALID_ARG, "chips is NULL");
  if (mode) *mode = chips->view.raster_mode;
  if (n_classes) *n_classes = chips->view.raster_mode != mgpu::kRasterNone ? (int64_t)chips->view.raster_ncls : 0;
  return MGPU_OK;
}

int32_t mgpu_chips_device_blob(const mgpu_chips* chips, void** device_ptr, int64_t* bytes) {
  if (!chips || !device_ptr || !bytes) return fail(MGPU_E_INVALID_ARG, "NULL argument");
  *device_ptr = chips->blob;
  *bytes = (int64_t)chips->bytes;
  return MGPU_OK;
}

int32_t mgpu_chips_from_device_blob(mgpu_ctx* ctx, const void* device_ptr, int64_t bytes, mgpu_chips** out) {
  if (!ctx || !device_ptr || !out || bytes <= 0) return fail(MGPU_E_INVALID_ARG, "NULL argument");
  if (int32_t st = set_device(ctx->device)) return st;
  if (bytes < (int64_t)mgpu::kBlobHeaderBytes) return fail(MGPU_E_INVALID_ARG, "blob too small");
  mgpu::BlobHeader hdr;
  HIP_TRY(hipMemcpy(&hdr, device_ptr, sizeof hdr, hipMemcpyDeviceToHost));
  if (int32_t st = mgpu::check_header(hdr, bytes)) return st;
  void* d = nullptr;
  HIP_TRY(hipMalloc(&d, bytes));
  hipError_t e = hipMemcpy(d, device_ptr, bytes, hipMemcpyDeviceToDevice);
  if (e != hipSuccess) {
    hipFree(d);
    return fail(MGPU_E_DEVICE, "hipMemcpy: %s", hipGetErrorString(e));
  }
  int32_t st = mgpu::adopt_device_blob(ctx, d, bytes, out);
  if (st) hipFree(d);
  return st;
}

int32_t mgpu_st_contains(mgpu_ctx* ctx, const mgpu_chips* chips, const int64_t* chip_row, const double* x,
                         const double* y, int64_t n, int8_t* out, void* stream) {
  if (!ctx || !chips) return fail(MGPU_E_INVALID_ARG, "ctx/chips is NULL");
  if (n < 0 || (n > 0 && (!chip_row || !x || !y || !out))) return fail(MGPU_E_INVALID_ARG, "bad arrays");
  if (int32_t st = set_device(ctx->device)) return st;
  if (chips->device != ctx->device)
    return fail(MGPU_E_INVALID_ARG, "chip table lives on device %d, context on device %d", chips->device, ctx->device);
  hipStream_t s = (hipStream_t)stream;
  if (int32_t st = ensure_ws(ctx, 1)) return st;
  auto* counters = (unsigned long long*)ctx->ws;
  HIP_TRY(hipMemsetAsync(counters, 0, kWsCounters, s));
  HIP_TRY(mgpu::launch_st_contains(chips->view, chip_row, x, y, n, out, counters, s));
  unsigned long long h[4] = {0};
  HIP_TRY(hipMemcpyAsync(h, counters, sizeof h, hipMemcpyDeviceToHost, s));
  HIP_TRY(hipStreamSynchronize(s));
  if (h[2])
    return fail(MGPU_E_INVALID_ARG, "st_contains: %llu chip rows outside [0, %u)", h[2], chips->view.n_chips);
  return MGPU_OK;
}


static bool plan_bins(const mgpu_options& o, const mgpu_chips* chips, int32_t is, int32_t res, int64_t n,
                      const uint8_t* valid, const mgpu::JoinArgs& a, mgpu::BinArgs& b) {
  const bool forced = o.pipeline == MGPU_PIPELINE_BINNED;
  if (!(forced || o.pipeline == MGPU_PIPELINE_AUTO) || n <= 0 || valid || !a.res_match) return false;
  if (n >= (int64_t)1 << 32 || chips->view.max_cell_chips > 32) return false;
  const mgpu::ChipTableView& v = chips->view;
  double x0, y0, W, H, aspect;
  if (is == MGPU_H3) {
    if (v.probe_mode == mgpu::kProbeCellId || !(v.bbox[2] - v.bbox[0] < 360.0) || !(v.bbox[3] - v.bbox[1] < 180.0))
      return false;
    x0 = v.bbox[0], y0 = v.bbox[1], W = v.bbox[2] - v.bbox[0], H = v.bbox[3] - v.bbox[1];
    const double latc = std::min(std::max(std::fabs(v.bbox[1]), std::fabs(v.bbox[3])), 85.0);
    aspect = W * std::cos(latc * kPi / 180.0) / std::max(H, 1e-12);
  } else {
    if (v.probe_mode != mgpu::kProbeDense || res != v.res || v.bng_edge == 0) return false;
    const mgpu::DenseFace& D = v.dense[0];
    x0 = (double)D.a0 * v.bng_edge, y0 = (double)D.b0 * v.bng_edge;
    W = (double)D.w * v.bng_edge, H = (double)D.h * v.bng_edge;
    aspect = W / std::max(H, 1e-12);
  }
  if (!(W > 0) || !(H > 0)) return false;
  if (!forced && ((double)chips->bytes < (double)o.bin_min_mb * 1048576.0 || n < o.bin_min_points)) return false;
  const int nb = (int)std::min<int64_t>(std::max<int64_t>(o.bin_count, 1), mgpu::bin_max());
  int nbx = (int)std::lround(std::sqrt(nb * aspect));
  nbx = std::min(std::max(nbx, 1), nb);
  const int nby = std::max(nb / nbx, 1);
  b.x0 = x0, b.y0 = y0;
  b.nbx = nbx, b.nby = nby;
  b.inv_bx = nbx / W, b.inv_by = nby / H;
  b.xcd_runs = (int32_t)o.bin_xcd;
  return true;
}

static int32_t join_impl(mgpu_ctx* ctx, const mgpu_chips* chips, int32_t is, int32_t res, const double* x,
                         const double* y, const int64_t* point_id, int64_t id_base, int64_t n, int64_t capacity,
                         int64_t* out_point, int32_t* out_poly, hipStream_t s, bool timed,
                         const uint8_t* valid = nullptr, int64_t valid_off = 0, int64_t n_ovr = 0,
                         int tie_host = 0, int64_t count_pool = -1) {
  if (!ctx || !chips) return fail(MGPU_E_INVALID_ARG, "ctx/chips is NULL");
  if (int32_t r = check_res(is, res)) return r;
  if (chips->index_system != is)
    return fail(MGPU_E_INVALID_ARG, "chip table built for index system %d, join asked for %d", chips->index_system, is);
  if (chips->device != ctx->device)
    return fail(MGPU_E_INVALID_ARG, "chip table lives on device %d, context on device %d", chips->device, ctx->device);
  if (n < 0 || (n > 0 && (!x || !y))) return fail(MGPU_E_INVALID_ARG, "bad point arrays");
  if (capacity < 0 || (capacity > 0 && (!out_point || !out_poly))) return fail(MGPU_E_INVALID_ARG, "bad output arrays");
  if (int32_t st = set_device(ctx->device)) return st;
  int64_t tiles = mgpu::join_tiles(n);
  const bool emit = count_pool < 0;
  const int64_t pool = emit ? capacity : count_pool;
  if (int32_t st = ensure_ws(ctx, tiles, pool)) return st;
  auto* base = (uint8_t*)ctx->ws;
  const WsLayout L = ws_layout(tiles, pool);
  const mgpu_options& o = ctx->opt;
  mgpu::JoinArgs a;
  a.x = x;
  a.y = y;
  a.n = n;
  a.n_tiles = tiles;
  a.res = res;
  a.res_match = (is == MGPU_BNG || chips->view.res < 0 || chips->view.res == res) ? 1 : 0;
  a.chips = chips->view;
  a.counters = (unsigned long long*)base;
  a.pool_used = a.counters + 5;
  a.n_dirty = (uint32_t*)(a.counters + 6);
  a.dirty = (uint32_t*)(base + L.dirty);
  a.pool_cap = pool;
  a.tile_count = (uint32_t*)(base + L.count);
  a.tile_where = (uint64_t*)(base + L.where);
  a.recs = (uint64_t*)(base + L.recs);
  a.tie_queue = ctx->tq;
  a.tie_cap = ctx->tq_cap;
  a.ovr = ctx->ovr;
  a.n_ovr = n_ovr;
  a.tie_host = (is == MGPU_H3 && tie_host) ? 1 : 0;
  a.pos_of = nullptr;
  mgpu::EmitArgs e;
  e.tile_count = a.tile_count;
  e.group_off = (uint64_t*)(base + L.off);
  a.group_sum = (uint32_t*)(base + L.gsum);
  a.group_cand = a.group_sum + (tiles / 32 + 1);
  e.tile_where = a.tile_where;
  e.recs = a.recs;
  e.point_id = point_id;
  e.id_base = id_base;
  e.capacity = capacity;
  e.out_point = out_point;
  e.out_poly = out_poly;
  a.valid = valid;
  a.valid_off = valid_off;
  a.mixed_idx = nullptr;
  a.mixed_res = nullptr;
  a.chunk_mixed = nullptr;
  a.extra = nullptr;
  a.n_extra = nullptr;
  a.poly_answers = 0;
  static_assert(kWsCounters == mgpu::kCounterWords * 8, "launch_join_clear clears the counters");
  HIP_TRY(mgpu::launch_join_clear(a.counters, ctx->tq, s));
  const bool bng_grid = is == MGPU_BNG && chips->view.raster_mode == mgpu::kRasterNone &&
                        chips->view.probe_mode == mgpu::kProbeDense && o.bng_split;
  const bool split = (o.pipeline == MGPU_PIPELINE_AUTO || o.pipeline == MGPU_PIPELINE_SPLIT) && n > 0 &&
                     (chips->view.raster_mode != mgpu::kRasterNone || bng_grid) && a.res_match &&
                     (is == MGPU_H3 || res == chips->view.res) && chips->view.max_cell_chips <= 32;
  mgpu::SplitArgs sa{};
  if (split) {
    const int64_t nc = mgpu::split_chunks(n), C = mgpu::split_chunk();
    size_t off = 0;
    auto carve = [&](size_t bytes) {
      const size_t o_ = off;
      off = align_up(off + bytes, 256);
      return o_;
    };
    const size_t o_codes = carve((size_t)nc * C * 4), o_idx = carve((size_t)nc * C * 2), o_res = carve((size_t)nc * C * 8);
    const size_t o_pairs = carve(nc * 4), o_mixed = carve(nc * 4), o_cand = carve(nc * 4), o_off = carve(nc * 8);
    const size_t o_extra = carve((size_t)nc * (C / mgpu::join_tile_points()) * 4);
    if (off > ctx->split_bytes) {
      if (ctx->split_ws) HIP_TRY(hipFree(ctx->split_ws));
      ctx->split_ws = nullptr;
      ctx->split_bytes = 0;
      HIP_TRY(hipMalloc(&ctx->split_ws, off));
      ctx->split_bytes = off;
    }
    auto* sb = (uint8_t*)ctx->split_ws;
    sa.codes = sb + o_codes;
    sa.mixed_idx = (uint16_t*)(sb + o_idx);
    sa.chunk_pairs = (uint32_t*)(sb + o_pairs);
    sa.chunk_mixed = (uint32_t*)(sb + o_mixed);
    sa.chunk_off = (uint64_t*)(sb + o_off);
    a.extra = sa.extra = (uint32_t*)(sb + o_extra);
    a.n_extra = (uint32_t*)(a.counters + 7);
    a.group_sum = sa.chunk_pairs;
    a.group_cand = (uint32_t*)(sb + o_cand);
    a.mixed_idx = sa.mixed_idx;
    a.mixed_res = (uint64_t*)(sb + o_res);
    a.chunk_mixed = sa.chunk_mixed;
    sa.point_id = point_id;
    sa.id_base = id_base;
    sa.capacity = capacity;
    sa.out_point = out_point;
    sa.out_poly = out_poly;
    sa.j = a;
  }
  mgpu::BinArgs ba{};
  const bool binned = !split && plan_bins(o, chips, is, res, n, valid, a, ba);
  if (binned) {
    const int64_t nc = mgpu::split_chunks(n), C = mgpu::split_chunk();
    const int64_t K = mgpu::bin_chunks(n), G = mgpu::bin_groups(n), nb = (int64_t)ba.nbx * ba.nby;
    size_t off = 0;
    auto carve = [&](size_t bytes) {
      const size_t o_ = off;
      off = align_up(off + bytes, 256);
      return o_;
    };
    const size_t o_perm = carve((size_t)n * 4), o_rorig = carve((size_t)n * 8);
    const size_t o_bx = carve((size_t)n * 8), o_by = carve((size_t)n * 8),
                 o_pre = carve((size_t)K * nb * 4), o_res = carve((size_t)nc * C * 8), o_cnt = carve((size_t)K * nb * 4),
                 o_gs = carve((size_t)G * nb * 4), o_pairs = carve(nc * 4), o_off = carve(nc * 8),
                 o_gperm = carve(nc * 4), o_gcand = carve(nc * 4);
    const mgpu::ChipTableView& cv = chips->view;
    uint64_t grid_entries = 0;
    for (int f = 0; f < 20; f++) grid_entries = std::max<uint64_t>(grid_entries, (uint64_t)cv.dense[f].base + (uint64_t)cv.dense[f].w * cv.dense[f].h);
    const bool keyed = is == MGPU_H3 && cv.probe_mode == mgpu::kProbeDense && o.bin_keys && grid_entries < (1ull << 30);
    const size_t o_key = keyed ? carve((size_t)n * 4) : 0;
    if (off > ctx->bin_bytes) {
      if (ctx->bin_ws) HIP_TRY(hipFree(ctx->bin_ws));
      ctx->bin_ws = nullptr;
      ctx->bin_bytes = 0;
      HIP_TRY(hipMalloc(&ctx->bin_ws, off));
      ctx->bin_bytes = off;
    }
    auto* bb = (uint8_t*)ctx->bin_ws;
    ba.x = x;
    ba.y = y;
    ba.bx = (double*)(bb + o_bx);
    ba.by = (double*)(bb + o_by);
    ba.pre = (uint32_t*)(bb + o_pre);
    ba.perm = (uint32_t*)(bb + o_perm);
    ba.res = (uint64_t*)(bb + o_rorig);
    ba.cnt = (uint32_t*)(bb + o_cnt);
    ba.gsum = (uint32_t*)(bb + o_gs);
    ba.key = keyed ? (uint32_t*)(bb + o_key) : nullptr;
    mgpu::JoinArgs j = a;
    j.bin_key = ba.key;
    j.x = ba.bx;
    j.y = ba.by;
    j.mixed_idx = nullptr;
    j.chunk_mixed = nullptr;
    j.poly_answers = 1;
    j.pos_of = ba.perm;
    j.mixed_res = (uint64_t*)(bb + o_res);
    j.group_sum = (uint32_t*)(bb + o_gperm);
    j.group_cand = (uint32_t*)(bb + o_gcand);
    ba.s.j = j;
    ba.s.chunk_pairs = (uint32_t*)(bb + o_pairs);
    ba.s.chunk_off = (uint64_t*)(bb + o_off);
    ba.s.point_id = point_id;
    ba.s.id_base = id_base;
    ba.s.capacity = capacity;
    ba.s.out_point = out_point;
    ba.s.out_poly = out_poly;
    HIP_TRY(hipMemsetAsync(bb + o_gperm, 0, align_up(nc * 4, 256) + nc * 4, s));
  } else if (!split) {
    HIP_TRY(hipMemsetAsync(base + L.gsum, 0, 2 * ((size_t)tiles / 32 + 1) * 4, s));
  }
  if (timed) HIP_TRY(hipEventRecord(ctx->ev0, s));
  if (split)
    HIP_TRY(mgpu::launch_split(is, sa, s, timed ? ctx->ev2 : nullptr, timed ? ctx->ev3 : nullptr, emit));
  else if (binned)
    HIP_TRY(mgpu::launch_binned(is, ba, s, timed ? ctx->ev3 : nullptr, timed ? ctx->ev2 : nullptr, emit));
  else
    HIP_TRY(mgpu::launch_join(is, a, e, s, timed ? ctx->ev2 : nullptr, emit));
  if (timed) HIP_TRY(hipEventRecord(ctx->ev1, s));
  auto& L2 = ctx->last;
  L2.split = split;
  L2.sargs = sa;
// ... 578 lines not shown

int32_t mgpu_internal_geometry_to_cells(mgpu_ctx* ctx, int32_t index_system, int32_t res, int64_t n,
                                        const int32_t* type_id, const int64_t* row_part, const int64_t* part_ring,
                                        const int64_t* ring_off, const double* xy, const uint8_t* valid,
                                        int64_t valid_offset, int64_t* out_cell, uint8_t* out_valid, void* stream,
                                        mgpu_stats* stats) {
  if (!ctx) return fail(MGPU_E_INVALID_ARG, "ctx is NULL");
  if (int32_t r = check_res(index_system, res)) return r;
  if (n < 0 || (n > 0 && (!out_cell || !type_id || !row_part || !part_ring || !ring_off || !xy)))
    return fail(MGPU_E_INVALID_ARG, "bad internal geometry arrays");
  if (int32_t st = set_device(ctx->device)) return st;
  hipStream_t s = (hipStream_t)stream;
  if (int32_t st = ensure_ws(ctx, 1)) return st;
  if (int32_t st = ensure_scratch(ctx, (size_t)std::max<int64_t>(n, 1) * 16)) return st;
  double* x = (double*)ctx->scratch;
  double* y = x + std::max<int64_t>(n, 1);
  HIP_TRY(hipMemsetAsync(ctx->ws, 0, kWsCounters, s));
  HIP_TRY(mgpu::launch_decode_internal(type_id, row_part, part_ring, ring_off, xy, valid, valid_offset, n, x, y,
                                       (unsigned long long*)ctx->ws, s));
  if (int32_t st = decode_status(ctx, 4, s)) return st;
  if (int32_t st = cells_impl(ctx, index_system, res, x, y, n, out_cell, s, valid, valid_offset, stats)) return st;
  if (out_valid) {
    HIP_TRY(mgpu::launch_valid_and(valid, valid_offset, nullptr, 0, n, out_valid, s));
    HIP_TRY(stream_wait(ctx, s));
  }
  return MGPU_OK;
}

int32_t mgpu_geometry_to_cells_arrow(mgpu_ctx* ctx, int32_t index_system, int32_t res,
                                     const struct ArrowDeviceArray* geom, const struct ArrowSchema* schema,
                                     int64_t* out_cell, uint8_t* out_valid, void* stream) {
  if (!ctx || !geom || !schema || !schema->format) return fail(MGPU_E_INVALID_ARG, "NULL argument");
  const char f = schema->format[0];
  if (!((f == 'z' || f == 'Z' || f == 'u' || f == 'U') && schema->format[1] == 0))
    return fail(MGPU_E_INVALID_ARG, "geometry column format '%s': binary (WKB) or utf8 (WKT) expected", schema->format);
  if (geom->device_type != ARROW_DEVICE_ROCM || geom->device_id != ctx->device)
    return fail(MGPU_E_INVALID_ARG, "geometry column not on this context's GPU");
  if (geom->array.n_buffers < 3 || !geom->array.buffers) return fail(MGPU_E_INVALID_ARG, "not a binary Arrow array");
  if (geom->sync_event) HIP_TRY(hipEventSynchronize((hipEvent_t)geom->sync_event));
  const bool o32 = f == 'z' || f == 'u';
  const uint8_t* offs = (const uint8_t*)geom->array.buffers[1] + (size_t)geom->array.offset * (o32 ? 4 : 8);
  const uint8_t* valid = geom->array.null_count != 0 ? (const uint8_t*)geom->array.buffers[0] : nullptr;
  return geometry_cells(ctx, index_system, res, (f == 'z' || f == 'Z') ? MGPU_GEOM_WKB : MGPU_GEOM_WKT,
                        (const uint8_t*)geom->array.buffers[2], offs, o32 ? 1 : 0, valid, geom->array.offset,
                        geom->array.length, out_cell, out_valid, (hipStream_t)stream, nullptr);
}

int32_t mgpu_pip_join_arrow(mgpu_ctx* ctx, const mgpu_chips* chips, int32_t index_system, int32_t res,
                            const struct ArrowDeviceArray* x, const struct ArrowDeviceArray* y,
                            const struct ArrowDeviceArray* point_id, int64_t capacity, int64_t* out_n_pairs,
                            int64_t* out_point_id, int32_t* out_polygon_id, void* stream, mgpu_stats* stats) {
  if (!ctx) return fail(MGPU_E_INVALID_ARG, "ctx is NULL");
  if (int32_t st = set_device(ctx->device)) return st;
  hipStream_t s = (hipStream_t)stream;
  const void *xd, *yd, *pd = nullptr;
  const uint8_t *xv, *yv, *pv = nullptr;
  int64_t xo, yo, po = 0;
  if (int32_t st = arrow_column(ctx, x, 8, &xd, &xv, &xo, "x")) return st;
  if (int32_t st = arrow_column(ctx, y, 8, &yd, &yv, &yo, "y")) return st;
  const int64_t n = x->array.length;
  if (y->array.length != n) return fail(MGPU_E_INVALID_ARG, "x and y differ in length");
  if (point_id) {
    if (int32_t st = arrow_column(ctx, point_id, 8, &pd, &pv, &po, "point_id")) return st;
    if (point_id->array.length != n) return fail(MGPU_E_INVALID_ARG, "point_id and x differ in length");
    if (pv) return fail(MGPU_E_INVALID_ARG, "point_id has nulls");
  }
  const uint8_t* valid = nullptr;
  int64_t voff = 0;
  if (xv && yv) {
    if (int32_t st = ensure_scratch(ctx, (size_t)(n + 7) / 8 + 1)) return st;
    HIP_TRY(mgpu::launch_valid_and(xv, xo, yv, yo, n, (uint8_t*)ctx->scratch, s));
    valid = (const uint8_t*)ctx->scratch;
  } else if (xv || yv) {
    valid = xv ? xv : yv;
    voff = xv ? xo : yo;
  }
  return pip_join_sync(ctx, chips, index_system, res, (const double*)xd, (const double*)yd, (const int64_t*)pd,
                       point_id ? 0 : x->array.offset, n, capacity, out_n_pairs, out_point_id, out_polygon_id, stream, stats, valid,
                       voff);
}

int32_t mgpu_test_parse_number(const char* s, int32_t len, double* out) {
  return mgpu::dec::parse_number(s, len, out);
}

int32_t mgpu_test_h3_elementary_host(int32_t fn, const double* a, const double* b, int64_t n, double* out) {
  namespace X = mgpu::exact;
  for (int64_t i = 0; i < n; ++i) {
    const double x = a[i], y = b ? b[i] : 0.0;
    double r = 0.0;
    switch (fn) {
      case 0: r = X::cr_sin(x); break;
      case 1: r = X::cr_cos(x); break;
      case 2: r = X::cr_tan(x); break;
      case 3: r = X::cr_acos(x); break;
      case 4: r = X::cr_atan2(x, y); break;
      case 5: r = X::x80_to_double(X::x80_add(X::x80_from_double(x), X::kX2Pi)); break;
      case 6: r = X::x80_to_double(X::x80_add(X::x80_from_double(x), X::x80_neg(X::kX2Pi))); break;
      case 7: r = X::x80_to_double(X::x80_mul(X::x80_from_double(x), X::kXSqrt7)); break;
      case 8: r = X::x80_to_double(X::x80_div(X::x80_from_double(x), X::kXSin60)); break;
      case 9: r = X::x80_to_double(X::x80_add(X::x80_from_double(x), X::x80_neg(X::kXAp7Rot))); break;
      case 10: r = X::x80_to_double(X::x80_div(X::x80_from_double(x), X::kXSqrt7)); break;
      case 11: r = X::x80_to_double(X::x80_add(X::x80_from_double(x), X::kXAp7Rot)); break;
      case 12: r = X::x80_cmp(X::x80_from_double(x), X::kXEpsilon) < 0 ? 1.0 : 0.0; break;
      case 13: r = X::x80_cmp(X::x80_from_double(x), X::kX2Pi) >= 0 ? 1.0 : 0.0; break;
      case 14: r = X::cr_asin(x); break;
      case 15: r = X::cr_atan(x); break;
      default: return MGPU_E_INVALID_ARG;
    }
    out[i] = r;
  }
  return MGPU_OK;
}

int32_t mgpu_test_h3_route_host(const double* lon, const double* lat, int64_t n, int32_t res, int64_t* out_cell) {
  if (res < 0 || res > 15) return MGPU_E_RESOLUTION;
  mgpu::parallel_for(n, 4096, [&](int64_t b, int64_t e, int) {
    for (int64_t i = b; i < e; ++i) {
      bool tie;
      out_cell[i] = (int64_t)mgpu::h3::point_to_cell(lon[i], lat[i], res, &tie);
    }
  });
  return MGPU_OK;
}

int32_t mgpu_test_h3_glibc_host(const double* lon, const double* lat, int64_t n, int32_t res, int64_t* out_cell) {
  if (res < 0 || res > 15) return MGPU_E_RESOLUTION;
  mgpu::parallel_for(n, 4096, [&](int64_t b, int64_t e, int) {
    for (int64_t i = b; i < e; ++i) out_cell[i] = (int64_t)mgpu::h3glibc::point_to_cell(lon[i], lat[i], res);
  });
  return MGPU_OK;
}

int32_t mgpu_test_decode_point(int32_t format, const uint8_t* data, int64_t len, double* x, double* y) {
  switch (format) {
    case MGPU_GEOM_WKB: return mgpu::geom::wkb_centroid(data, len, x, y);
    case MGPU_GEOM_WKT: return mgpu::geom::wkt_centroid((const char*)data, len, x, y);
    case MGPU_GEOM_HEX: return mgpu::geom::hex_centroid((const char*)data, len, x, y);
    case MGPU_GEOM_GEOJSON: return mgpu::geom::json_centroid((const char*)data, len, x, y);
  }
  return mgpu::geom::kDecUnsupported;
}

int32_t mgpu_test_join_counters(mgpu_ctx* ctx, uint64_t* out16) {
  if (!ctx || !out16) return fail(MGPU_E_INVALID_ARG, "bad arguments");
  memset(out16, 0, 16 * 8);
  if (!ctx->ws) return MGPU_OK;
  if (int32_t st = set_device(ctx->device)) return st;
  HIP_TRY(hipDeviceSynchronize());
  HIP_TRY(hipMemcpy(out16, ctx->ws, 16 * 8, hipMemcpyDeviceToHost));
  return MGPU_OK;
}

int32_t mgpu_test_internal_centroid(int64_t n, const int32_t* type_id, const int64_t* row_part, const int64_t* part_ring,
                                    const int64_t* ring_off, const double* xy, double* x, double* y, int32_t* status) {
  for (int64_t i = 0; i < n; i++)
    status[i] = mgpu::geom::internal_centroid(type_id[i], row_part[i], row_part[i + 1], part_ring, ring_off, xy, &x[i], &y[i]);
  return MGPU_OK;
}

}
```

mosaic_amd/csrc/capi_internal.h:

```cpp
#pragma once
#include <hip/hip_runtime.h>
#include <stdint.h>

#include "../../include/mosaic_gpu.h"
#include "chip_table.h"
#include "kernels.h"

struct mgpu_options {
  int64_t h3_libm = MGPU_LIBM_REFERENCE;
  int64_t pipeline = MGPU_PIPELINE_AUTO;
  int64_t bin_count = 64;
  int64_t bin_min_mb = 256;
  int64_t bin_min_points = 1 << 21;
  int64_t bin_xcd = 1;
  int64_t bin_keys = 0;
  int64_t spin_us = 2000;
  int64_t ring_batch = (int64_t)1 << 26;
  int64_t count_lds_slots = 4096;
  int64_t count_groups = 0;
  int64_t kring_batch = 0;
  int64_t cellagg_groups = 0;
  int64_t cellagg_lds = 1;
  int64_t cellagg_bin_min = (int64_t)1 << 22;
  int64_t polyfill_slab = (int64_t)1 << 24;
  int64_t geomring_slab = (int64_t)1 << 16;
  int64_t geomring_lds_slots = 0;
  int64_t bng_split = 0;
  int64_t raster = 1, raster_bng = 0, raster_sub = 16, raster_milli = 250;
};

struct mgpu_ctx {
  int device = 0;
  mgpu_options opt;
  void* ws = nullptr;
  size_t ws_bytes = 0;
  hipEvent_t ev0 = nullptr, ev1 = nullptr, ev2 = nullptr, ev3 = nullptr;
  void* comm = nullptr;
  void* split_ws = nullptr;
  size_t split_bytes = 0;
  void* bin_ws = nullptr;
  size_t bin_bytes = 0;
  uint64_t* tq = nullptr;
  int64_t tq_cap = 0;
  uint64_t* ovr = nullptr;
  int64_t ovr_cap = 0;
  uint64_t* pin = nullptr;
  uint64_t* pin_dev = nullptr;
  void* scratch = nullptr;
  size_t scratch_bytes = 0;
  void* redo = nullptr;
  size_t redo_bytes = 0;
  struct {
    bool valid = false, pool_ok = false;
    const mgpu_chips* chips = nullptr;
    int32_t is = 0, res = 0;
    const double *x = nullptr, *y = nullptr;
    const int64_t* point_id = nullptr;
    int64_t id_base = 0, n = 0, total = 0;
    const uint8_t* pts_valid = nullptr;
    int64_t pts_valid_off = 0;
    mgpu::EmitArgs emit{};
    mgpu::JoinArgs jargs{};
    int64_t n_tiles = 0;
    int64_t n_ovr = 0;
    int tie_host = 0;
    bool split = false;
    mgpu::SplitArgs sargs{};
    bool binned = false;
    mgpu::BinArgs bargs{};
    bool async_pending = false;
    int64_t* d_n_pairs = nullptr;
    void* stream = nullptr;
    int64_t capacity = 0;
    int64_t* out_point = nullptr;
    int32_t* out_poly = nullptr;
    int64_t pool = 0, pool_used = 0;
  } last;
};

struct mgpu_chips {
  int device = 0;
  int32_t index_system = MGPU_H3;
  void* blob = nullptr;
  size_t bytes = 0;
  mgpu::ChipTableView view{};
  int64_t n_vertices = 0;
  mutable void* slots = nullptr;
};

namespace mgpu {
int32_t set_error(int32_t code, const char* fmt, ...);
int64_t blob_bytes_of_header(const void* header);
constexpr int64_t kBlobHeaderSize = 1024;
int32_t adopt_device_blob(mgpu_ctx* ctx, void* dev_blob, int64_t bytes, mgpu_chips** out);
int32_t begin_call(mgpu_ctx* ctx);
}

int32_t cells_impl(mgpu_ctx* ctx, int32_t is, int32_t res, const double* x, const double* y, int64_t n,
                   int64_t* out_cell, hipStream_t s, const uint8_t* valid, int64_t voff, mgpu_stats* stats);
int32_t ensure_scratch(mgpu_ctx* ctx, size_t bytes);
```

mosaic_amd/csrc/chip_build.cpp:

```cpp

#include <hip/hip_runtime.h>

#include <algorithm>
#include <unordered_map>
#include <unordered_set>
#include <chrono>
#include <sched.h>
#include <array>
#include <atomic>
#include <cmath>
#include <cstdio>
#include <cstring>
#include <cstdlib>
#include <limits>
#include <map>
#include <string>
#include <functional>
#include <tuple>
#include <mutex>
#include <thread>
#include <vector>

#include "../../include/mosaic_gpu.h"
#include "bng_core.h"
#include "chip_build.h"
#include "chip_table.h"
#include "error.h"
#include "h3_core.h"
#include "parallel.h"
#include "pip_core.h"
#include "raster.h"
#include "wkb.h"
#include "h3_boundary.h"

namespace {

size_t align_up(size_t v, size_t a) { return (v + a - 1) / a * a; }

}

namespace mgpu {
mgpu::ChipTableView view_from_header(const BlobHeader& h, uint8_t* base) {
  mgpu::ChipTableView v;
  v.slots = (const mgpu::HashSlot*)(base + h.off[kArrSlots]);
  v.hash_mask = h.hash_mask;
  v.max_probe = h.max_probe;
  v.n_chips = h.n_chips;
  v.n_cells = h.n_cells;
  v.chip_poly = (const int32_t*)(base + h.off[kArrChipPoly]);
  v.chip_flags = (const uint8_t*)(base + h.off[kArrChipFlags]);
  v.chip_part = (const uint32_t*)(base + h.off[kArrChipPart]);
  v.chip_env = (const double*)(base + h.off[kArrChipEnv]);
  v.chip_row = (const int64_t*)(base + h.off[kArrChipRow]);
  v.part_ring = (const uint32_t*)(base + h.off[kArrPartRing]);
  v.ring_vtx = (const uint32_t*)(base + h.off[kArrRingVtx]);
  v.ring_env = (const double*)(base + h.off[kArrRingEnv]);
  v.vtx = (const double*)(base + h.off[kArrVtx]);
  v.row_to_chip = (const uint32_t*)(base + h.off[kArrRowToChip]);
  v.chip_strip = (const uint32_t*)(base + h.off[kArrChipStrip]);
  v.chip_sy = (const double*)(base + h.off[kArrChipSy]);
  v.strip_edge = (const uint32_t*)(base + h.off[kArrStripEdge]);
  v.edges = (const double*)(base + h.off[kArrEdges]);
  v.edge_ring = (const uint8_t*)(base + h.off[kArrEdgeRing]);
  v.chip_hdr = (const mgpu::ChipHdr*)(base + h.off[kArrChipHdr]);
  v.grid = (const uint64_t*)(base + h.off[kArrGrid]);
  for (int f = 0; f < 20; f++) v.dense[f] = h.dense[f];
  v.probe_mode = h.probe_mode;
  v.res = h.res;
  v.face_mask = h.face_mask;
  for (int k = 0; k < 4; k++) v.bbox[k] = h.bbox[k];
  v.k_res = h.k_res;
  v.bng_edge = h.bng_edge;
  v.bng_inv_edge = h.bng_inv_edge;
  v.max_cell_chips = h.max_cell_chips;
  v.raster_mode = h.raster_mode;
  v.raster_nx = h.raster_nx;
  v.raster_ny = h.raster_ny;
  v.raster_pix = h.raster_pix;
  v.raster_px0 = h.raster_px0;
  v.raster_py0 = h.raster_py0;
  v.raster_x0 = h.raster_x0;
  v.raster_y0 = h.raster_y0;
  v.raster_inv_dx = h.raster_inv_dx;
  v.raster_inv_dy = h.raster_inv_dy;
  for (int k = 0; k < 4; k++) v.raster_pc[k] = h.raster_pc[k];
  v.raster = (const uint16_t*)(base + h.off[kArrRaster]);
  v.raster_cls = (const uint64_t*)(base + h.off[kArrRasterCls]);
  v.raster_sub_n = h.raster_sub_n;
  v.raster_sub_w = h.raster_sub_w;
  v.raster_band_shift = h.raster_band_shift;
  v.raster_nband = h.raster_nband;
  v.raster_band = h.raster_nband ? (const uint32_t*)(base + h.off[kArrRasterBand]) : nullptr;
  v.raster_rank = h.raster_sub_n && !h.raster_nband ? (const mgpu::RankWord*)(base + h.off[kArrRasterRank]) : nullptr;
  v.cell_ans_g = h.cell_ans_g;
  v.cell_ans_sw = h.cell_ans_sw;
  v.cell_ans_inv_sw = h.cell_ans_sw ? 1.0 / h.cell_ans_sw : 0.0;
  v.cell_ans_row = h.cell_ans_g ? (const uint32_t*)(base + h.off[kArrCellAnsRow]) : nullptr;
  v.cell_ans = (const uint16_t*)(base + h.off[kArrCellAns]);
  v.raster_sub = (const uint16_t*)(base + h.off[kArrRasterSub]);
  v.raster_pal = h.raster_pal ? (const uint64_t*)(base + h.off[kArrRasterPal]) : nullptr;
  v.raster_idx2 = (const uint8_t*)(base + h.off[kArrRasterIdx2]);
  v.raster_bshift = h.raster_bshift;
  v.raster_bnx = h.raster_bnx;
  v.raster_bny = h.raster_bny;
  v.raster_blk = h.raster_bshift ? (const uint16_t*)(base + h.off[kArrRasterBlk]) : nullptr;
  v.raster_ncls = h.raster_ncls;
  v.raster_cls_poly = (const int32_t*)(base + h.off[kArrRasterClsPoly]);
  return v;
}
}

namespace {

bool build_bng_dense(const std::vector<mgpu::HashSlot>& cells, int32_t* res_out, mgpu::DenseFace* D,
                     uint32_t* edge_out, std::vector<uint64_t>& grid) {
  if (cells.empty()) return false;
  auto p10 = [](int k) {
    int64_t v = 1;
    while (k-- > 0) v *= 10;
    return v;
  };
  int p = -1;
  for (int q = 1; q <= 6; q++)
    if ((int64_t)cells[0].cell >= p10(2 * q + 3) && (int64_t)cells[0].cell < 2 * p10(2 * q + 3)) p = q;
  if (p < 0) return false;
  const bool quad = cells[0].cell % 10 != 0;
  if (quad && p > 5) return false;
  const int res = quad ? -(p + 1) : p;
  const int64_t d = p10(6 - p);
  const int64_t edge = quad ? d / 2 : d;
  const int64_t B = p10(p - 1);
  std::vector<std::pair<int64_t, int64_t>> cr(cells.size());
  int64_t c0 = INT64_MAX, c1 = INT64_MIN, r0 = INT64_MAX, r1 = INT64_MIN;
  for (size_t k = 0; k < cells.size(); k++) {
    const int64_t id = (int64_t)cells[k].cell;
    int64_t rem = id - p10(2 * p + 3);
    if (rem < 0 || rem >= p10(2 * p + 3)) return false;
    const int64_t eL = rem / p10(2 * p + 1);
    rem %= p10(2 * p + 1);
    const int64_t nL = rem / p10(2 * p - 1);
    rem %= p10(2 * p - 1);
    const int64_t eB = rem / p10(p);
    rem %= p10(p);
    const int64_t nB = rem / 10, q = rem % 10;
    if (eB >= B || nB >= B || (quad ? (q < 1 || q > 4) : q != 0)) return false;
    int64_t col = eL * B + eB, row = nL * B + nB;
    if (quad) col = 2 * col + (q == 3 || q == 4), row = 2 * row + (q == 2 || q == 3);
    int64_t back = 0;
    mgpu::bng::point_to_cell((col + 0.5) * (double)edge, (row + 0.5) * (double)edge, res, &back);
    if (back != id || (col + 1) * edge > 10000000 || (row + 1) * edge > 10000000) return false;
    cr[k] = {col, row};
    c0 = std::min(c0, col), c1 = std::max(c1, col), r0 = std::min(r0, row), r1 = std::max(r1, row);
  }
  const int64_t total = (c1 - c0 + 1) * (r1 - r0 + 1);
  if (total > std::max<int64_t>(16 * (int64_t)cells.size(), 1 << 20) || total > (1LL << 26)) return false;
  memset(D, 0, sizeof(mgpu::DenseFace));
  D->a0 = (int32_t)c0;
  D->b0 = (int32_t)r0;
  D->w = (uint32_t)(c1 - c0 + 1);
  D->h = (uint32_t)(r1 - r0 + 1);
  D->base = 0;
  grid.assign((size_t)total, 0);
  for (size_t k = 0; k < cells.size(); k++) {
    const mgpu::HashSlot& e = cells[k];
    grid[(size_t)((cr[k].second - r0) * D->w + (cr[k].first - c0))] =
        (uint64_t)e.first | ((uint64_t)e.count << 32) | ((uint64_t)e.core_mask << 48);
  }
  *res_out = res;
  *edge_out = (uint32_t)edge;
  return true;
}

constexpr double kPi = 3.14159265358979323846;

double angle_between(const double* a, const double* b) {
  double d = a[0] * b[0] + a[1] * b[1] + a[2] * b[2];
  d = d > 1 ? 1 : (d < -1 ? -1 : d);
  return acos(d);
}

constexpr int64_t kMaxDimCII[17] = {2, -1, 14, -1, 98, -1, 686, -1, 4802, -1, 33614, -1, 235298, -1, 1647086, -1, 11529602};

bool build_lattice(const std::vector<mgpu::HashSlot>& cells, std::vector<std::pair<uint64_t, uint32_t>>& keys,
                   int* res_out, uint32_t* face_mask, double bbox[4], std::vector<uint8_t>* interior_out = nullptr) {
  namespace H = mgpu::h3;
  if (cells.empty()) return false;
  int res = (int)((cells[0].cell >> 52) & 15);
  if (res < 5) return false;
  const double rho = 0.3 / pow(H::kSqrt7, res);
  double k_res = H::k_of_res(res);
  if (interior_out) interior_out->assign(cells.size(), 0);
  const int64_t grain = 4096;
  const int T = mgpu::parallel_slots((int64_t)cells.size(), grain);
  std::vector<std::vector<std::pair<uint64_t, uint32_t>>> tkeys(T);
  std::vector<std::array<double, 4>> text(T, std::array<double, 4>{1e9, -1e9, 1e9, -1e9});
  std::atomic<bool> bad{false};
// ... 2064 lines not shown
```

mosaic_amd/csrc/chip_table.h:

```cpp
#pragma once
#include <stdint.h>

#ifdef __HIPCC__
#define MGPU_HDI_FWD __host__ __device__ __forceinline__
#else
#define MGPU_HDI_FWD inline
#endif

namespace mgpu {

enum ChipFlags : uint8_t {
  kChipCore = 1,
  kChipRect = 2,
  kChipMulti = 4,
  kChipEmpty = 8,
  kChipNoGeom = 16,
  kChipNoStrips = 32,
};

constexpr int kMaxStrips = 64;
constexpr int kStripRings = 32;

MGPU_HDI_FWD int strip_of(double y, double y0, double inv_h, int S) {
  double v = (y - y0) * inv_h;
  int s = v < (double)S ? (int)v : S - 1;
  return s < 0 ? 0 : s;
}

struct alignas(16) HashSlot {
  uint64_t cell;
  uint32_t first;
  uint16_t count;
  uint16_t core_mask;
};

constexpr int kGrid = 16;
struct alignas(64) ChipHdr {
  double env[4];
  double sx, sy;
  double inv_h;
  uint32_t strip_base;
  uint16_t n_strips;
  uint8_t flags;
  uint8_t single_ring;
  uint32_t grid[kGrid];
};
static_assert(sizeof(ChipHdr) == 128, "ChipHdr is two lines");

enum GridState { kCellOut = 0, kCellIn = 1, kCellMixed = 2 };

MGPU_HDI_FWD int grid_index(double v, double v0, double scale) {
  double g = (v - v0) * scale;
  int i = g < (double)kGrid ? (int)g : kGrid - 1;
  return i < 0 ? 0 : i;
}

struct DenseFace {
  int32_t a0, b0;
  uint32_t w, h;
  uint32_t base;
};

struct alignas(8) RankWord {
  uint32_t bits;
  uint32_t base;
};

struct ChipTableView {
  const HashSlot* slots;
  uint32_t hash_mask;
  uint32_t max_probe;
  uint32_t n_chips;
  uint32_t n_cells;
  const int32_t* chip_poly;
  const uint8_t* chip_flags;
  const uint32_t* chip_part;
  const double* chip_env;
  const int64_t* chip_row;
  const uint32_t* part_ring;
  const uint32_t* ring_vtx;
  const double* ring_env;
  const double* vtx;
  const uint32_t* row_to_chip;
  const uint32_t* chip_strip;
  const double* chip_sy;
  const uint32_t* strip_edge;
  const double* edges;
  const uint8_t* edge_ring;
  const ChipHdr* chip_hdr;
  int32_t probe_mode;
  int32_t res;
  uint32_t face_mask;
  double bbox[4];
  double k_res;
  const uint64_t* grid;
  DenseFace dense[20];
  uint32_t bng_edge;
  double bng_inv_edge;
  uint32_t max_cell_chips;
  int32_t raster_mode;
  uint32_t raster_nx, raster_ny;
  uint32_t raster_pix;
  int32_t raster_px0, raster_py0;
  double raster_x0, raster_y0, raster_inv_dx, raster_inv_dy;
  uint32_t raster_pc[4];
  const uint16_t* raster;
  const uint64_t* raster_cls;
  const int32_t* raster_cls_poly;
  uint32_t raster_ncls;
  uint32_t raster_sub_n, raster_sub_w;
  const RankWord* raster_rank;
  uint32_t raster_band_shift, raster_nband;
  const uint32_t* raster_band;
  uint32_t cell_ans_g, cell_ans_sw;
  double cell_ans_inv_sw;
  const uint32_t* cell_ans_row;
  const uint16_t* cell_ans;
  const uint16_t* raster_sub;
  const uint64_t* raster_pal;
  const uint8_t* raster_idx2;
  uint32_t raster_bshift, raster_bnx, raster_bny;
  const uint16_t* raster_blk;
};

enum RasterMode { kRasterNone = 0, kRasterLonLat = 1, kRasterBng = 2 };
constexpr uint32_t kCellAnsChips = 15;
constexpr uint16_t kCellAnsMixed = 0xFFFF;
constexpr uint32_t kNoCellAns = 0xFFFFFFFFu;
constexpr uint64_t kCellAnsFlag = 1ull << 47;
constexpr uint32_t kCoreWhole = 0x8000u;
MGPU_HDI_FWD uint32_t grid_count(uint64_t e, bool ans) {
  return (uint32_t)(e >> 32) & ((ans && (e & kCellAnsFlag)) ? 0xFu : 0xFFFFu);
}
MGPU_HDI_FWD uint32_t cell_ans_index(uint64_t e) { return (uint32_t)((e >> 36) & 0x7FF) | (uint32_t)(e >> 63) << 11; }
constexpr uint16_t kPixEmpty = 0;
constexpr uint16_t kPixMixed = 0xFFFF;
constexpr uint64_t kPalFull = 1ull << 63;

enum ProbeMode { kProbeCellId = 0, kProbeLattice = 1, kProbeDense = 2 };

#ifdef __HIPCC__
#define MGPU_HDI __host__ __device__ __forceinline__
#else
#define MGPU_HDI inline
#endif

MGPU_HDI uint32_t cell_hash(uint64_t cell) {
  uint64_t z = cell * 0x9E3779B97F4A7C15ULL;
  z ^= z >> 29;
  z *= 0xBF58476D1CE4E5B9ULL;
  return (uint32_t)(z >> 32);
}

}
```

mosaic_amd/csrc/kernels.h:

```cpp
#pragma once
#include <hip/hip_runtime.h>
#include <stdint.h>

#include "../../include/mosaic_gpu.h"
#include "chip_table.h"

namespace mgpu {

struct JoinArgs {
  const double* x;
  const double* y;
  int64_t n;
  int64_t n_tiles;
  int res;
  int res_match;
  ChipTableView chips;
  uint32_t* tile_count;
  uint32_t* group_sum;
  uint32_t* group_cand;
  uint64_t* tile_where;
  uint64_t* recs;
  int64_t pool_cap;
  unsigned long long* pool_used;
  uint32_t* dirty;
  uint32_t* n_dirty;
  unsigned long long* counters;
  uint64_t* tie_queue;
  int64_t tie_cap;
  const uint64_t* ovr;
  int64_t n_ovr;
  int tie_host;
  const uint32_t* pos_of;
  const uint16_t* mixed_idx;
  uint64_t* mixed_res;
  const uint32_t* chunk_mixed;
  uint32_t* extra;
  uint32_t* n_extra;

  const uint8_t* valid;
  int64_t valid_off;
  int poly_answers;
  const uint32_t* bin_key = nullptr;
  uint32_t* in_chunk_pairs = nullptr;
};

struct RedoArgs {
  const uint32_t* list;
  uint32_t* old;
  uint8_t* affected;
  uint32_t* changed;
  uint32_t* first;
};

struct SplitArgs {
  JoinArgs j;
  void* codes;
  uint32_t* chunk_pairs;
  uint32_t* chunk_mixed;
  uint16_t* mixed_idx;
  uint32_t* extra;
  uint64_t* chunk_off;
  const int64_t* point_id;
  int64_t id_base;
  int64_t capacity;
  int64_t* out_point;
  int32_t* out_poly;
  const uint32_t* redo_first = nullptr;
  const uint8_t* redo_affected = nullptr;
};
int64_t split_chunk();
int64_t split_chunk_tiles();
int64_t split_chunks(int64_t n);
hipError_t launch_split(int is, const SplitArgs& a, hipStream_t s, hipEvent_t after_classify, hipEvent_t after_mixed,
                        bool emit = true);
hipError_t launch_split_emit(int is, const SplitArgs& a, hipStream_t s);
hipError_t launch_split_redo(int is, const SplitArgs& sa, const RedoArgs& R, int64_t n, hipStream_t s,
                             bool emit = true);

struct BinArgs {
  SplitArgs s;
  const double* x;
  const double* y;
  double* bx;
  double* by;
  uint32_t* perm;
  uint64_t* res;
  uint32_t* cnt;
  uint32_t* pre;
  uint32_t* gsum;
  double x0, y0, inv_bx, inv_by;
  int32_t nbx, nby;
  int32_t xcd_runs;
  uint32_t* key;
};
int64_t bin_chunk();
int64_t bin_chunks(int64_t n);
int64_t bin_groups(int64_t n);
int32_t bin_max();
hipError_t launch_binned(int is, const BinArgs& a, hipStream_t s, hipEvent_t after_bin, hipEvent_t after_join,
                         bool emit = true);
hipError_t launch_bin_emit(const BinArgs& a, hipStream_t s);

struct EmitArgs {
  const uint32_t* tile_count;
  uint64_t* group_off;
  const uint64_t* tile_where;
  const uint64_t* recs;
  const int64_t* point_id;
  int64_t id_base;
  int64_t capacity;
  int64_t* out_point;
  int32_t* out_poly;
  const uint32_t* redo_first = nullptr;
  const uint8_t* redo_affected = nullptr;
};


hipError_t launch_cells(int is, int res, const double* x, const double* y, int64_t n, int64_t* out,
                        unsigned long long* counters, unsigned long long* ties, int64_t tie_cap,
                        uint64_t* tie_queue, int64_t tq_cap, hipStream_t s, const uint8_t* valid = nullptr,
                        int64_t voff = 0);
constexpr int kCounterWords = 16;
hipError_t launch_join_clear(unsigned long long* counters, uint64_t* tie_queue, hipStream_t s);
hipError_t launch_join_readback(const unsigned long long* counters, const uint64_t* tie_queue, int tq_words,
                                uint64_t* pin, hipStream_t s);
hipError_t launch_scatter_i64(const int64_t* pos, const int64_t* val, int64_t n, int64_t* out, hipStream_t s);
hipError_t launch_gather_xy(const double* x, const double* y, const int64_t* pos, int64_t n, double* xy,
                            hipStream_t s);
hipError_t launch_decode_internal(const int32_t* type_id, const int64_t* row_part, const int64_t* part_ring,
                                  const int64_t* ring_off, const double* xy, const uint8_t* valid, int64_t voff,
                                  int64_t n, double* x, double* y, unsigned long long* counters, hipStream_t s);
hipError_t launch_decode_points(int format, const uint8_t* data, const void* offsets, int off32, const uint8_t* valid,
                                int64_t voff, int64_t n, double* x, double* y, unsigned long long* counters,
                                hipStream_t s);
hipError_t launch_scan_sums(int64_t* v, int64_t n, hipStream_t s);
hipError_t launch_valid_and(const uint8_t* a, int64_t aoff, const uint8_t* b, int64_t boff, int64_t n, uint8_t* out,
                            hipStream_t s);
int64_t join_tiles(int64_t n);
int64_t join_tile_points();
int64_t join_slot_records();
hipError_t launch_join(int is, const JoinArgs& a, const EmitArgs& e, hipStream_t s, hipEvent_t after_stream,
                       bool emit = true);
hipError_t launch_join_redo(int is, const JoinArgs& a, const EmitArgs& e, const RedoArgs& R, int64_t n, hipStream_t s,
                            bool emit = true);
hipError_t launch_emit(const EmitArgs& e, int64_t n_tiles, hipStream_t s);

struct CountArgs {
  const int32_t* ids;
  uint32_t n_slots;
  const uint32_t* chip_slot;
  const uint32_t* dense;
  int32_t min_id;
  uint32_t contiguous;
  uint32_t lds_slots;
  uint32_t hash_slots;
  uint32_t stage_n;
  const int64_t* weight;
  unsigned long long* count;
  unsigned long long* sum;
  uint32_t* dropped;
  uint32_t max_groups;
};
constexpr int64_t kCountLdsSlotsMax = 4096;
constexpr int64_t kCountGroupsMax = 65536;
constexpr uint32_t kCountHash = 4096;
constexpr int64_t kCountStageMax = 2048;
hipError_t launch_split_count(int is, const SplitArgs& a, const CountArgs& c, hipStream_t s);
hipError_t launch_tile_count(const EmitArgs& e, int64_t n_tiles, const CountArgs& c, hipStream_t s);
hipError_t launch_bin_count(const BinArgs& b, const CountArgs& c, hipStream_t s);

struct LookupArgs {
  int32_t* out_polygon;
  int32_t* out_matches;
  int32_t null_id;
  uint32_t* dropped;
};
hipError_t launch_split_lookup(int is, const SplitArgs& a, const LookupArgs& o, hipStream_t s);
hipError_t launch_tile_lookup(const EmitArgs& e, int64_t n, int64_t n_tiles, const LookupArgs& o, hipStream_t s);
hipError_t launch_bin_lookup(const BinArgs& b, const LookupArgs& o, hipStream_t s);
int64_t format_chunks(int64_t n);
hipError_t launch_format_cells(int is, const int64_t* cells, int64_t n, char* out, int64_t out_bytes,
                               int64_t* offsets, int64_t* chunk, unsigned long long* counters, hipStream_t s);
int64_t format_chunks(int64_t n);
hipError_t launch_kring_count(int is, const int64_t* cells, int64_t n, int k, int loop_only, int64_t* mc,
                              int64_t* chunk, uint32_t* fb_idx, unsigned long long* counters, hipStream_t s);
int64_t kring_fallback_words(int k);
int32_t kring_fallback_max_k();
hipError_t launch_kring_fallback(const int64_t* cells, const uint32_t* fb_idx, int64_t j0, int64_t j1, int k,
                                 int loop_only, int64_t* mc, int64_t* chunk, const int64_t* offsets, int64_t* out,
                                 int64_t capacity, uint64_t* scratch, int write, unsigned long long* counters,
                                 hipStream_t s);
hipError_t launch_kring_write(int is, const int64_t* cells, int64_t n, int k, int loop_only, const int64_t* mc,
                              int64_t* chunk, int64_t* offsets, int64_t* out, int64_t capacity, hipStream_t s);
int64_t sort_pairs_hist_words(int64_t n);
hipError_t launch_sort_pairs(unsigned long long** k0, unsigned long long** v0, unsigned long long** k1,
                             unsigned long long** v1, int64_t n, unsigned long long differ, uint32_t* hist, hipStream_t s);
hipError_t launch_st_contains(const ChipTableView& t, const int64_t* row, const double* x, const double* y, int64_t n,
                              int8_t* out, unsigned long long* counters, hipStream_t s);

}
```

mosaic_amd/csrc/kernels.hip:

```cpp
#include <hip/hip_runtime.h>
#include <stdint.h>
#include <type_traits>

#include <map>
#include <mutex>

#define H3T_QUAL static __constant__ const
#include "h3_core.h"
#include "bng_core.h"
#include "pip_core.h"
#include "h3_ring.h"
#include "kernels.h"
#include "raster.h"

namespace mgpu {

#ifndef MGPU_BLOCK
#define MGPU_BLOCK 64
#endif
constexpr int kBlock = MGPU_BLOCK;
constexpr int kItems = 4;
constexpr int kTile = kBlock * kItems;
constexpr int kStreamBlock = 256;
static_assert(kTile <= 1024, "point-in-tile indices are 10 bits");
// ... 964 lines not shown
    if (agg > (uint32_t)kSlot) {
      const unsigned long long off = atomicAdd(a.pool_used, (unsigned long long)agg);
      dst = off + agg <= (unsigned long long)a.pool_cap ? (uint64_t)a.n_tiles * kSlot + off : kNoDst;
    }
    a.tile_count[tile] = agg;
    a.tile_where[tile] = dst;
    if (agg) atomicAdd(&a.group_sum[tile / kScanGroup], agg);
    s_dst = dst;
  }
  const bool staged = agg <= (uint32_t)kOutCap;
  __syncthreads();
  const uint64_t dst = s_dst;
  uint64_t* const rec = dst == kNoDst ? nullptr : a.recs + dst;

  uint32_t pos = excl;
#pragma unroll 1
  for (int k = 0; k < kItems; k++) {
    const int li = l0 + k;
    if (!SLOW) {
      const uint32_t first = s_first[li];
      for (uint32_t m = s_mask[li]; m; m &= m - 1) {
        const int32_t poly = t.chip_poly[first + __builtin_ctz(m)];
        if (staged) {
          s_out_poly[pos] = poly;
          s_out_li[pos] = (uint16_t)li;
        } else if (rec) {
          rec[pos] = ((uint64_t)li << 32) | (uint32_t)poly;
        }
        pos++;
      }
      continue;
    }
    const uint32_t cnt = s_cnt[li];
    if (!cnt) continue;
    const uint32_t first = s_first[li];
    const int64_t p = MGPU_PT(li);
    uint32_t m = s_mask[li];
    const uint32_t nj = cnt < (uint32_t)kMaskBits ? cnt : (uint32_t)kMaskBits;
    for (uint32_t j = 0; j < cnt; j++) {
      bool hit;
      if (!SLOW || j < nj) {
        hit = (m >> j) & 1;
      } else {
        const Range r{first, cnt, 0};
        hit = chip_is_core(t, r, j) || pip::chip_contains_strips(t, first + j, a.x[p], a.y[p]);
      }
      if (!hit) continue;
      const int32_t poly = t.chip_poly[first + j];
      if (staged) {
        s_out_poly[pos] = poly;
        s_out_li[pos] = (uint16_t)li;
      } else if (rec) {
        rec[pos] = ((uint64_t)li << 32) | (uint32_t)poly;
      }
      pos++;
    }
  }
  MGPU_STAMP(4);
  if (!staged || !rec) return;
  __syncthreads();
#ifndef MGPU_NT_RECS
#define MGPU_NT_RECS 1
#endif
  for (uint32_t i = threadIdx.x; i < agg; i += kBlock) {
    const uint64_t v = ((uint64_t)s_out_li[i] << 32) | (uint32_t)s_out_poly[i];
#if MGPU_NT_RECS
    __builtin_nontemporal_store(v, &rec[i]);
#else
    rec[i] = v;
#endif
  }
  MGPU_STAMP(4);
}

#ifndef MGPU_WAVES_PER_EU
#define MGPU_WAVES_PER_EU 8
#endif
#if MGPU_WAVES_PER_EU
#define MGPU_JOIN_ATTR __attribute__((amdgpu_waves_per_eu(MGPU_WAVES_PER_EU)))
#else
#define MGPU_JOIN_ATTR
#endif
template <int IS>
__global__ __launch_bounds__(kBlock) MGPU_JOIN_ATTR void pip_join_kernel(JoinArgs a) {
  join_tile<IS, false>(a, blockIdx.x);
}

template <int IS>
__global__ __launch_bounds__(kBlock) void pip_fix_kernel(JoinArgs a) {
  const uint32_t nd = *a.n_dirty;
  for (uint32_t q = blockIdx.x; q < nd; q += gridDim.x) {
    join_tile<IS, true>(a, a.dirty[q]);
    __syncthreads();
  }
}

#ifndef MGPU_CLS_BLOCK
#define MGPU_CLS_BLOCK 256
#endif
constexpr int kClsBlock = MGPU_CLS_BLOCK;
constexpr int kClsItems = kChunk / kClsBlock;
static_assert(kClsItems * (kClsBlock / 64) == 64, "one wave scans a chunk's ballots");
constexpr uint32_t kCodeMixed32 = 0xFFFFFFFFu;

template <int IS>
struct CodeOf {
  using T = uint16_t;
};
template <>
struct CodeOf<MGPU_BNG> {
  using T = uint32_t;
};


__device__ __forceinline__ uint32_t bng_grid_class(const JoinArgs& a, int64_t p, double px, double py, bool* ok,
                                                     uint32_t* first) {
  const ChipTableView& t = a.chips;
  bool tie = false;
  uint32_t gi = kNoEntry;
  Range r = chip_probe<MGPU_BNG, false>(a, p, px, py, ok, &tie, &gi);
  if (!*ok) return kPixEmpty;
  uint64_t e = 0;
  if (gi != kNoEntry) {
    e = t.grid[gi];
    r = grid_range(e, t.cell_ans_row != nullptr);
  }
  *first = r.first;
  if (r.count == 0) return kPixEmpty;
  if (r.count <= 8 && (r.core & ((1u << r.count) - 1u)) == (1u << r.count) - 1u) return (1u << r.count) - 1u;
  if (t.cell_ans_row && (e & kCellAnsFlag)) {
    const uint32_t eI = (uint32_t)bng::d2i(px), nI = (uint32_t)bng::d2i(py), ed = t.bng_edge;
    const uint32_t col = div_fix(eI, ed, t.bng_inv_edge), row = div_fix(nI, ed, t.bng_inv_edge);
    const uint32_t u = div_fix(eI - col * ed, t.cell_ans_sw, t.cell_ans_inv_sw);
    const uint32_t v = div_fix(nI - row * ed, t.cell_ans_sw, t.cell_ans_inv_sw);
    const uint32_t ai = t.cell_ans_row[row - (uint32_t)t.dense[0].b0] + cell_ans_index(e);
    const uint16_t m = t.cell_ans[((size_t)ai * t.cell_ans_g + v) * t.cell_ans_g + u];
    if (m != kCellAnsMixed && m < 256u) return m;
  }
  return kPixMixed;
}

#ifndef MGPU_CFY_BLOCK
#define MGPU_CFY_BLOCK 512
#endif
constexpr int kCfyBlock = MGPU_CFY_BLOCK;
#ifndef MGPU_CFY_BATCH
#define MGPU_CFY_BATCH 4
#endif
#ifndef MGPU_CFY_WAVES
#define MGPU_CFY_WAVES 1
#endif
constexpr int kCfyBatch = MGPU_CFY_BATCH;

template <int N>
__device__ __forceinline__ void raster_class_batch(const ChipTableView& t, const uint16_t* blk, const uint32_t* band,
                                                   const uint32_t (&ri)[N], const uint32_t (&bi)[N],
                                                   const uint32_t (&sub)[N], uint32_t (&cl)[N]) {
  const uint32_t s2 = t.raster_sub_n * t.raster_sub_n;
  uint32_t c[N], bb[N], px[N], q[N];
  bool pix[N], ref[N];
#pragma unroll
  for (int k = 0; k < N; k++) {
    c[k] = blk[bi[k] != kNoPixel ? bi[k] : 0u];
    bb[k] = band[sub[k] >> 16];
  }
#pragma unroll
  for (int k = 0; k < N; k++) {
    pix[k] = ri[k] < kRasterFull && (bi[k] == kNoPixel || c[k] == kPixMixed);
    px[k] = t.raster[pix[k] ? ri[k] : 0u];
  }
#pragma unroll
  for (int k = 0; k < N; k++) {
    ref[k] = pix[k] && px[k] >= 0x8000u && px[k] != kPixMixed;
    const uint64_t i = ((uint64_t)bb[k] + (px[k] & 0x7FFFu)) * s2 + (sub[k] & 0xFFFFu);
    q[k] = t.raster_sub[ref[k] ? i : 0ull];
  }
#pragma unroll
  for (int k = 0; k < N; k++)
    cl[k] = ri[k] >= kRasterFull ? (ri[k] == kRasterFull ? kPixMixed : kPixEmpty) : ref[k] ? q[k] : pix[k] ? px[k] : c[k];
}

__device__ __forceinline__ bool cfy_staged(const ChipTableView& t, uint32_t nblk) {
  return t.raster_blk && nblk && t.raster_band && t.raster_nband && !t.raster_pal && t.raster_sub && t.raster_sub_n &&
         t.raster_nx && t.raster_ny;
}

template <int IS, class F>
__device__ __forceinline__ void cfy_dispatch(bool staged, bool nulls, F& run) {
  if constexpr (IS == MGPU_H3) {
    if (staged) {
      if (nulls) run(std::true_type{}, std::true_type{});
      else run(std::true_type{}, std::false_type{});
    } else {
      if (nulls) run(std::false_type{}, std::true_type{});
      else run(std::false_type{}, std::false_type{});
    }
  } else {
    run(std::false_type{}, std::true_type{});
  }
}

template <int IS>
__global__ __launch_bounds__(kCfyBlock) __attribute__((amdgpu_waves_per_eu(MGPU_CFY_WAVES))) void classify_wave_kernel(SplitArgs sa, int64_t n_chunks) {
  using Code = typename CodeOf<IS>::T;
  constexpr int kW = kCfyBlock / 64;
  constexpr int kItems = kChunk / 64;
  static_assert(kItems % kCfyBatch == 0, "MGPU_CFY_BATCH must divide the points per lane of a chunk");
  const JoinArgs& a = sa.j;
  const ChipTableView& t = a.chips;
  extern __shared__ uint16_t s_blk[];
  const int lane = threadIdx.x & 63, wave = threadIdx.x >> 6;
  const bool use_blk = IS == MGPU_H3 && t.raster_blk != nullptr;
  const bool bng_grid = IS == MGPU_BNG && t.raster_mode == kRasterNone;
  const uint32_t nblk = use_blk ? t.raster_bnx * t.raster_bny : 0u;
  uint32_t* s_band = (uint32_t*)(s_blk + ((nblk + 1) & ~1u));
  if (use_blk)
    for (uint32_t i = threadIdx.x; i < nblk; i += kCfyBlock) s_blk[i] = t.raster_blk[i];
  if (IS == MGPU_H3)
    for (uint32_t i = threadIdx.x; i < t.raster_nband; i += kCfyBlock) s_band[i] = t.raster_band[i];
  __syncthreads();
  Code* codes = (Code*)sa.codes;
  const unsigned long long below = (1ull << lane) - 1ull;
  bool any_bad = false;
  const int64_t ch_step = (int64_t)gridDim.x * kW;
  auto run_chunk = [&](int64_t ch, auto staged_c, auto nulls_c, auto full_c) {
    constexpr bool kStaged = decltype(staged_c)::value, kNulls = decltype(nulls_c)::value, kFull = decltype(full_c)::value;
    const int64_t c0 = ch * kChunk;
    uint32_t pairs = 0, nmixed = 0;
    for (int b = 0; b < kItems; b += kCfyBatch) {
      double bx[kCfyBatch], by[kCfyBatch];
#pragma unroll
      for (int k = 0; k < kCfyBatch; k++) {
        const int64_t p = c0 + (int64_t)(b + k) * 64 + lane;
        bx[k] = by[k] = 0.0;
        if (kFull || p < a.n) {
          bx[k] = __builtin_nontemporal_load(&a.x[p]);
          by[k] = __builtin_nontemporal_load(&a.y[p]);
        }
      }
      uint32_t ri[kCfyBatch], gix[kCfyBatch], sb[kCfyBatch], bi[kCfyBatch];
#pragma unroll
      for (int k = 0; k < kCfyBatch; k++) {
        ri[k] = kNoPixel;
        gix[k] = 0;
        sb[k] = 0;
        bi[k] = kNoPixel;
        const int64_t pk = c0 + (int64_t)(b + k) * 64 + lane;
        if ((kFull || pk < a.n) && (!kNulls || pt_valid(a.valid, a.valid_off, pk))) {
          bool ok = true;
          uint32_t g_ = 0, s_ = 0, b_ = kNoPixel;
          if (IS == MGPU_BNG && bng_grid) {
            const uint32_t m = bng_grid_class(a, pk, bx[k], by[k], &ok, &g_);
            ri[k] = m == kPixMixed ? kRasterFull : m;
          } else {
            ri[k] = raster_index<IS>(t, bx[k], by[k], &ok, &g_, &s_, &b_);
          }
          gix[k] = g_;
          sb[k] = s_;
          bi[k] = use_blk ? b_ : kNoPixel;
          any_bad |= !ok;
        }
      }
      uint32_t cl[kCfyBatch];
      uint64_t ge[kCfyBatch];
#ifndef MGPU_CFY_ABLATE
#define MGPU_CFY_ABLATE 0
#endif
      if constexpr (kStaged) {
        raster_class_batch<kCfyBatch>(t, s_blk, s_band, ri, bi, sb, cl);
#pragma unroll
        for (int k = 0; k < kCfyBatch; k++) ge[k] = 0ull;
      } else {
#pragma unroll
        for (int k = 0; k < kCfyBatch; k++) {
#if MGPU_CFY_ABLATE == 1
          cl[k] = ri[k] < kRasterFull ? (ri[k] & 1) : kPixEmpty;
#elif MGPU_CFY_ABLATE == 2
          cl[k] = ri[k] < kRasterFull && bi[k] != kNoPixel && s_blk[bi[k]] != kPixMixed ? s_blk[bi[k]] : kPixEmpty;
#elif MGPU_CFY_ABLATE == 3
          cl[k] = ri[k] < kRasterFull ? (bi[k] != kNoPixel && s_blk[bi[k]] != kPixMixed ? s_blk[bi[k]] : t.raster[ri[k]])
                                      : kPixEmpty;
#elif MGPU_CFY_ABLATE == 4
          cl[k] = ri[k] < kRasterFull ? t.raster[ri[k]] : kPixEmpty;
#elif MGPU_CFY_ABLATE == 5
          cl[k] = ri[k] < kRasterFull ? (bi[k] != kNoPixel && s_blk[bi[k]] != kPixMixed ? s_blk[bi[k]] : kPixMixed)
                                      : kPixEmpty;
#else
          if (IS == MGPU_BNG && bng_grid)
            cl[k] = ri[k] == kRasterFull ? kPixMixed : (ri[k] == kNoPixel ? kPixEmpty : ri[k]);
          else
            cl[k] = ri[k] < kRasterFull ? raster_class_blk(t, s_blk, ri[k], bi[k], sb[k], s_band)
                                        : (ri[k] == kRasterFull ? kPixMixed : kPixEmpty);
#endif
          if (IS == MGPU_BNG && bng_grid) ge[k] = gix[k];
          else ge[k] = (IS == MGPU_BNG && ri[k] < kRasterFull) ? t.grid[gix[k]] : 0ull;
        }
      }
#pragma unroll
      for (int k = 0; k < kCfyBatch; k++) {
        const int64_t p = c0 + (int64_t)(b + k) * 64 + lane;
        const bool valid = kFull || p < a.n;
        bool mixed = cl[k] == kPixMixed;
        Code code;
        if (IS == MGPU_H3) {
          code = (Code)cl[k];
          if (!mixed && cl[k] != kPixEmpty) {
            const uint32_t c = cl[k];
            pairs += c < t.raster_pc[0] ? 1u : c < t.raster_pc[1] ? 2u : c < t.raster_pc[2] ? 3u : c < t.raster_pc[3] ? 4u
                     : (uint32_t)__popc((uint32_t)(t.raster_cls[c] >> 32));
          }
        } else {
          const uint32_t first = (uint32_t)ge[k], m = cl[k];
          if (!mixed && m && !(m < 256u && first < (1u << 24))) mixed = true;
          code = (Code)(mixed ? kCodeMixed32 : (m ? (first << 8) | m : 0u));
          if (!mixed) pairs += __popc(m);
        }
        if (valid) MGPU_ST_INTER(code, &codes[p]);
        mixed = mixed && valid;
        const unsigned long long bal = __ballot(mixed);
        if (mixed) sa.mixed_idx[c0 + nmixed + (uint32_t)__popcll(bal & below)] = (uint16_t)((b + k) * 64 + lane);
        nmixed += (uint32_t)__popcll(bal);
      }
    }
    pairs = wave_sum_u32(pairs);
    if (lane == 0) {
      sa.chunk_pairs[ch] = pairs;
      sa.chunk_mixed[ch] = nmixed;
      a.group_cand[ch] = 0;
    }
  };
  auto run = [&](auto staged_c, auto nulls_c) {
    for (int64_t ch = (int64_t)blockIdx.x * kW + wave; ch < n_chunks; ch += ch_step) {
      if (IS == MGPU_H3 && (ch + 1) * kChunk <= a.n) {
        if constexpr (IS == MGPU_H3) run_chunk(ch, staged_c, nulls_c, std::true_type{});
      } else {
        run_chunk(ch, staged_c, nulls_c, std::false_type{});
      }
    }
  };
  cfy_dispatch<IS>(cfy_staged(t, nblk), a.valid != nullptr, run);
  count_wave(&a.counters[2], any_bad);
}


#ifndef MGPU_CFY_PAIR
#define MGPU_CFY_PAIR 1
#endif
typedef double dbl2_t __attribute__((ext_vector_type(2)));
template <int IS>
__global__ __launch_bounds__(kCfyBlock) __attribute__((amdgpu_waves_per_eu(MGPU_CFY_WAVES))) void classify_pair_kernel(SplitArgs sa, int64_t n_chunks) {
  using Code = typename CodeOf<IS>::T;
  constexpr int kW = kCfyBlock / 64;
  constexpr int kPairItems = kChunk / 128;
  constexpr int kPB = kCfyBatch / 2 > 0 ? kCfyBatch / 2 : 1;
  constexpr int kPts = 2 * kPB;
  static_assert(kPairItems % kPB == 0, "MGPU_CFY_BATCH / 2 must divide the pair items per lane of a chunk");
  const JoinArgs& a = sa.j;
  const ChipTableView& t = a.chips;
  extern __shared__ uint16_t s_blk[];
  const int lane = threadIdx.x & 63, wave = threadIdx.x >> 6;
  const bool use_blk = IS == MGPU_H3 && t.raster_blk != nullptr;
  const bool bng_grid = IS == MGPU_BNG && t.raster_mode == kRasterNone;
  const uint32_t nblk = use_blk ? t.raster_bnx * t.raster_bny : 0u;
  uint32_t* s_band = (uint32_t*)(s_blk + ((nblk + 1) & ~1u));
  if (use_blk)
    for (uint32_t i = threadIdx.x; i < nblk; i += kCfyBlock) s_blk[i] = t.raster_blk[i];
  if (IS == MGPU_H3)
    for (uint32_t i = threadIdx.x; i < t.raster_nband; i += kCfyBlock) s_band[i] = t.raster_band[i];
  __syncthreads();
  Code* codes = (Code*)sa.codes;
  const unsigned long long below = (1ull << lane) - 1ull;
  bool any_bad = false;
  const int64_t ch_step = (int64_t)gridDim.x * kW;
  auto run_chunk = [&](int64_t ch, auto staged_c, auto nulls_c, auto full_c) {
    constexpr bool kStaged = decltype(staged_c)::value, kNulls = decltype(nulls_c)::value, kFull = decltype(full_c)::value;
    const int64_t c0 = ch * kChunk;
    uint32_t pairs = 0, nmixed = 0;
    for (int b = 0; b < kPairItems; b += kPB) {
      double X[kPts], Y[kPts];
#pragma unroll
      for (int k = 0; k < kPB; k++) {
        const int64_t p = c0 + (int64_t)(b + k) * 128 + 2 * lane;
        if (kFull || p + 1 < a.n) {
          const dbl2_t vx = __builtin_nontemporal_load((const dbl2_t*)(a.x + p));
          const dbl2_t vy = __builtin_nontemporal_load((const dbl2_t*)(a.y + p));
          X[2 * k] = vx.x, X[2 * k + 1] = vx.y, Y[2 * k] = vy.x, Y[2 * k + 1] = vy.y;
        } else {
          X[2 * k] = Y[2 * k] = X[2 * k + 1] = Y[2 * k + 1] = 0.0;
          if (p < a.n) X[2 * k] = a.x[p], Y[2 * k] = a.y[p];
        }
      }
      uint32_t ri[kPts], gix[kPts], sb[kPts], bi[kPts];
#pragma unroll
      for (int j = 0; j < kPts; j++) {
        ri[j] = kNoPixel;
        gix[j] = 0;
        sb[j] = 0;
        bi[j] = kNoPixel;
        const int64_t pj = c0 + (int64_t)(b + j / 2) * 128 + 2 * lane + (j & 1);
        if ((kFull || pj < a.n) && (!kNulls || pt_valid(a.valid, a.valid_off, pj))) {
          bool ok = true;
          uint32_t g_ = 0, s_ = 0, b_ = kNoPixel;
          if (IS == MGPU_BNG && bng_grid) {
            const uint32_t m = bng_grid_class(a, pj, X[j], Y[j], &ok, &g_);
            ri[j] = m == kPixMixed ? kRasterFull : m;
          } else {
            ri[j] = raster_index<IS>(t, X[j], Y[j], &ok, &g_, &s_, &b_);
          }
          gix[j] = g_;
          sb[j] = s_;
          bi[j] = use_blk ? b_ : kNoPixel;
          any_bad |= !ok;
        }
      }
      uint32_t cl[kPts];
      uint64_t ge[kPts];
      if constexpr (kStaged) {
        raster_class_batch<kPts>(t, s_blk, s_band, ri, bi, sb, cl);
#pragma unroll
        for (int j = 0; j < kPts; j++) ge[j] = 0ull;
      } else {
#pragma unroll
        for (int j = 0; j < kPts; j++) {
          if (IS == MGPU_BNG && bng_grid) {
            cl[j] = ri[j] == kRasterFull ? kPixMixed : (ri[j] == kNoPixel ? kPixEmpty : ri[j]);
            ge[j] = gix[j];
          } else {
            cl[j] = ri[j] < kRasterFull ? raster_class_blk(t, s_blk, ri[j], bi[j], sb[j], s_band)
                                        : (ri[j] == kRasterFull ? kPixMixed : kPixEmpty);
            ge[j] = (IS == MGPU_BNG && ri[j] < kRasterFull) ? t.grid[gix[j]] : 0ull;
          }
        }
      }
      Code code[kPts];
      bool mixed[kPts];
#pragma unroll
      for (int j = 0; j < kPts; j++) {
        const int64_t pj = c0 + (int64_t)(b + j / 2) * 128 + 2 * lane + (j & 1);
        bool m = cl[j] == kPixMixed;
        if (IS == MGPU_H3) {
          code[j] = (Code)cl[j];
          if (!m && cl[j] != kPixEmpty) {
            const uint32_t c = cl[j];
            pairs += c < t.raster_pc[0] ? 1u : c < t.raster_pc[1] ? 2u : c < t.raster_pc[2] ? 3u : c < t.raster_pc[3] ? 4u
                     : (uint32_t)__popc((uint32_t)(t.raster_cls[c] >> 32));
          }
        } else {
          const uint32_t first = (uint32_t)ge[j], mm = cl[j];
          if (!m && mm && !(mm < 256u && first < (1u << 24))) m = true;
          code[j] = (Code)(m ? kCodeMixed32 : (mm ? (first << 8) | mm : 0u));
          if (!m) pairs += __popc(mm);
        }
        mixed[j] = m && (kFull || pj < a.n);
      }
#pragma unroll
      for (int k = 0; k < kPB; k++) {
        const int64_t p = c0 + (int64_t)(b + k) * 128 + 2 * lane;
        if (kFull || p + 1 < a.n) {
          if (sizeof(Code) == 2) {
            MGPU_ST_INTER((uint32_t)code[2 * k] | ((uint32_t)code[2 * k + 1] << 16), (uint32_t*)(codes + p));
          } else {
            typedef uint32_t u32x2_t __attribute__((ext_vector_type(2)));
            u32x2_t v;
            v.x = (uint32_t)code[2 * k];
            v.y = (uint32_t)code[2 * k + 1];
            MGPU_ST_INTER(v, (u32x2_t*)(codes + p));
          }
        } else if (p < a.n) {
          MGPU_ST_INTER(code[2 * k], &codes[p]);
        }
        const unsigned long long b0 = __ballot(mixed[2 * k]), b1 = __ballot(mixed[2 * k + 1]);
        const uint32_t r0 = nmixed + (uint32_t)__popcll(b0 & below) + (uint32_t)__popcll(b1 & below);
        const uint16_t li = (uint16_t)((b + k) * 128 + 2 * lane);
        if (mixed[2 * k]) sa.mixed_idx[c0 + r0] = li;
        if (mixed[2 * k + 1]) sa.mixed_idx[c0 + r0 + (mixed[2 * k] ? 1u : 0u)] = (uint16_t)(li + 1);
        nmixed += (uint32_t)(__popcll(b0) + __popcll(b1));
      }
    }
    pairs = wave_sum_u32(pairs);
    if (lane == 0) {
      sa.chunk_pairs[ch] = pairs;
      sa.chunk_mixed[ch] = nmixed;
      a.group_cand[ch] = 0;
    }
  };
  auto run = [&](auto staged_c, auto nulls_c) {
    for (int64_t ch = (int64_t)blockIdx.x * kW + wave; ch < n_chunks; ch += ch_step) {
      if (IS == MGPU_H3 && (ch + 1) * kChunk <= a.n) {
        if constexpr (IS == MGPU_H3) run_chunk(ch, staged_c, nulls_c, std::true_type{});
      } else {
        run_chunk(ch, staged_c, nulls_c, std::false_type{});
      }
    }
  };
  cfy_dispatch<IS>(cfy_staged(t, nblk), a.valid != nullptr, run);
  count_wave(&a.counters[2], any_bad);
}

#ifndef MGPU_MIXED_LEAN
#define MGPU_MIXED_LEAN 1
#endif
template <int IS>
__global__ __launch_bounds__(kBlock) MGPU_JOIN_ATTR void pip_mixed_kernel(JoinArgs a) {
  const uint32_t nm = a.chunk_mixed[blockIdx.x];
  if (threadIdx.x == 0 && nm > (uint32_t)kGTile) {
    const uint32_t more = (nm - 1) / kGTile;
    const uint32_t q = atomicAdd(a.n_extra, more);
    for (uint32_t t = 0; t < more; t++) a.extra[q + t] = blockIdx.x * kChunkTiles + 1 + t;
  }
  join_tile<IS, false, 2, MGPU_MIXED_LEAN != 0>(a, blockIdx.x * kChunkTiles);
}

template <int IS>
__global__ __launch_bounds__(kBlock) void pip_mixed_more_kernel(JoinArgs a) {
  const uint32_t n = *a.n_extra;
  for (uint32_t q = blockIdx.x; q < n; q += gridDim.x) {
    join_tile<IS, false, 2>(a, a.extra[q]);
    __syncthreads();
  }
}

template <int IS, int G>
__global__ __launch_bounds__(kBlock) void pip_mixed_fix_kernel(JoinArgs a) {
  const uint32_t nd = *a.n_dirty;
  for (uint32_t q = blockIdx.x; q < nd; q += gridDim.x) {
    join_tile<IS, true, G>(a, a.dirty[q]);
    __syncthreads();
  }
}

#ifndef MGPU_EMIT_LDSBAR
#define MGPU_EMIT_LDSBAR 1
#endif
__device__ __forceinline__ void lds_barrier() {
#if MGPU_EMIT_LDSBAR
  asm volatile("s_waitcnt lgkmcnt(0)\n\ts_barrier" ::: "memory");
#else
  __syncthreads();
#endif
}

__device__ __forceinline__ uint32_t chunk_excl_scan(uint32_t v, uint32_t* s_w, uint32_t* total) {
  const int lane = threadIdx.x & 63, wave = threadIdx.x >> 6;
  const uint32_t incl = wave_incl_scan(v);
  if (lane == 63) s_w[wave] = incl;
  lds_barrier();
  uint32_t before = 0, all = 0;
#pragma unroll
  for (int w = 0; w < kClsBlock / 64; w++) {
    before += w < wave ? s_w[w] : 0u;
    all += s_w[w];
  }
  *total = all;
  return before + incl - v;
}

constexpr int kEmitWin = 2048;
#ifndef MGPU_EMIT_SWZ
#define MGPU_EMIT_SWZ 1
#endif
__device__ __forceinline__ uint32_t emit_swz(uint32_t q) { return MGPU_EMIT_SWZ ? q ^ ((q >> 6) & 63u) : q; }
#ifndef MGPU_EMIT_NT
#define MGPU_EMIT_NT 1
#endif
#ifndef MGPU_EMIT_NT_OTHER
#define MGPU_EMIT_NT_OTHER 0
#endif
#ifndef MGPU_EMIT_WAVES
#define MGPU_EMIT_WAVES 7
#endif
#ifndef MGPU_EMIT_WAVES_BNG
#define MGPU_EMIT_WAVES_BNG 5
#endif
#ifndef MGPU_BIN_EMIT_WAVES
#define MGPU_BIN_EMIT_WAVES 5
#endif
constexpr int kEmitCls = 2048;
constexpr int kEmitMres = 512;
#ifndef MGPU_EMIT_MR
#define MGPU_EMIT_MR 1
#endif
__host__ __device__ inline uint32_t emit_cls_staged(const ChipTableView& t) {
  const uint32_t n = t.raster_ncls < t.raster_pc[0] ? t.raster_ncls : t.raster_pc[0];
  return n < (uint32_t)kEmitCls ? n : (uint32_t)kEmitCls;
}
constexpr int kEmitTrash = 64;
typedef uint32_t __attribute__((may_alias)) lds_u32;
template <int N>
__device__ __forceinline__ void emit_forget(uint32_t (&w)[N]) {
#pragma unroll
  for (int i = 0; i < N; i++) asm volatile("" : "+v"(w[i]));
}
template <int IS>
__global__ __launch_bounds__(kClsBlock) __attribute__((amdgpu_waves_per_eu(IS == MGPU_H3 ? MGPU_EMIT_WAVES : MGPU_EMIT_WAVES_BNG))) void split_emit_kernel(SplitArgs sa) {
  using Code = typename CodeOf<IS>::T;
  constexpr int kWords = kClsItems * (int)sizeof(Code) / 4;
  static_assert(kWords % 4 == 0 && kWords >= 4, "whole 16-byte code loads per thread (MGPU_CLS_BLOCK 256 or 512)");
  const JoinArgs& a = sa.j;
  const ChipTableView& t = a.chips;
  __shared__ uint32_t s_w[2][kClsBlock / 64];
  __shared__ uint32_t s_poly[kEmitWin + kEmitTrash];
  __shared__ uint16_t s_pt[kEmitWin + kEmitTrash];
  __shared__ uint64_t s_mr[MGPU_EMIT_MR ? kEmitMres : 1];
  extern __shared__ int32_t s_cp[];
  if (sa.redo_affected && blockIdx.x < *sa.redo_first && !sa.redo_affected[blockIdx.x]) return;
  const int64_t c0 = (int64_t)blockIdx.x * kChunk;
  const int64_t p0 = c0 + (int64_t)threadIdx.x * kClsItems;
  const Code kMixed = IS == MGPU_H3 ? (Code)kPixMixed : (Code)kCodeMixed32;
  uint32_t cw[kWords];
  if (p0 + kClsItems <= a.n) {
    const uint4* src = (const uint4*)((const Code*)sa.codes + p0);
#pragma unroll
    for (int i = 0; i < kWords / 4; i++) {
      const uint4 v = src[i];
      cw[4 * i] = v.x, cw[4 * i + 1] = v.y, cw[4 * i + 2] = v.z, cw[4 * i + 3] = v.w;
    }
  } else {
#pragma unroll
    for (int i = 0; i < kWords; i++) cw[i] = 0;
    const Code* cs = (const Code*)sa.codes;
    for (int k = 0; k < kClsItems; k++)
      if (p0 + k < a.n) {
        const uint32_t c = cs[p0 + k];
        if (sizeof(Code) == 2)
          cw[k >> 1] |= c << ((k & 1) * 16);
        else
          cw[k] = c;
      }
  }
  uint32_t ncp = 0;
  if (IS == MGPU_H3) {
    ncp = emit_cls_staged(t);
    for (uint32_t i = threadIdx.x; i < ncp; i += kClsBlock) s_cp[i] = t.raster_cls_poly[i];
  }
  constexpr uint32_t kMr = MGPU_EMIT_MR ? (uint32_t)kEmitMres : 0u;
#if MGPU_EMIT_MR
  {
    const uint32_t nm = sa.chunk_mixed[blockIdx.x], nms = nm < kMr ? nm : kMr;
    for (uint32_t i = threadIdx.x; i < nms; i += kClsBlock) {
      const uint64_t v = a.mixed_res[c0 + i];
      const uint32_t m = (uint32_t)(v >> 32);
      s_mr[i] = __popc(m) == 1 ? (uint64_t)(uint32_t)t.chip_poly[(uint32_t)v + __builtin_ctz(m)] | (1ull << 32) : v;
    }
  }
#endif
  auto code = [&](int k) -> Code {
    return sizeof(Code) == 2 ? (Code)(cw[k >> 1] >> ((k & 1) * 16)) : (Code)cw[k];
  };
// ... 1164 lines not shown

hipError_t launch_join_readback(const unsigned long long* counters, const uint64_t* tie_queue, int tq_words,
                                uint64_t* pin, hipStream_t s) {
  hipLaunchKernelGGL(join_readback_kernel, dim3(1), dim3(256), 0, s, counters, tie_queue, tq_words, pin);
  return hipGetLastError();
}

hipError_t launch_scatter_i64(const int64_t* pos, const int64_t* val, int64_t n, int64_t* out, hipStream_t s) {
  if (n <= 0) return hipSuccess;
  const int64_t blocks = std::min<int64_t>((n + 255) / 256, 1024);
  hipLaunchKernelGGL(scatter_i64_kernel, dim3((unsigned)blocks), dim3(256), 0, s, pos, val, n, out);
  return hipGetLastError();
}

hipError_t launch_gather_xy(const double* x, const double* y, const int64_t* pos, int64_t n, double* xy, hipStream_t s) {
  if (n <= 0) return hipSuccess;
  const int64_t blocks = std::min<int64_t>((n + 255) / 256, 1024);
  hipLaunchKernelGGL(gather_xy_kernel, dim3((unsigned)blocks), dim3(256), 0, s, x, y, pos, n, xy);
  return hipGetLastError();
}

__global__ __launch_bounds__(kStreamBlock) void valid_and_kernel(const uint8_t* __restrict__ a, int64_t aoff,
                                                               const uint8_t* __restrict__ b, int64_t boff, int64_t n,
                                                               uint8_t* __restrict__ out) {
  const int64_t byte = (int64_t)blockIdx.x * blockDim.x + threadIdx.x;
  if (byte * 8 >= n) return;
  uint8_t v = 0;
  for (int k = 0; k < 8; k++) {
    const int64_t p = byte * 8 + k;
    if (p < n && pt_valid(a, aoff, p) && pt_valid(b, boff, p)) v |= (uint8_t)(1u << k);
  }
  out[byte] = v;
}

hipError_t launch_valid_and(const uint8_t* a, int64_t aoff, const uint8_t* b, int64_t boff, int64_t n, uint8_t* out,
                            hipStream_t s) {
  if (n <= 0) return hipSuccess;
  const int64_t bytes = (n + 7) / 8;
  hipLaunchKernelGGL(valid_and_kernel, dim3((unsigned)((bytes + kStreamBlock - 1) / kStreamBlock)), dim3(kStreamBlock), 0,
                     s, a, aoff, b, boff, n, out);
  return hipGetLastError();
}

int64_t join_tiles(int64_t n) { return (n + kTile - 1) / kTile; }
int64_t join_tile_points() { return kTile; }
int64_t join_slot_records() { return kSlot; }

#ifndef MGPU_FIX_GRID
#define MGPU_FIX_GRID 8192
#endif
constexpr int64_t kFixGrid = MGPU_FIX_GRID;
hipError_t launch_join(int is, const JoinArgs& a, const EmitArgs& e, hipStream_t s, hipEvent_t after_stream, bool emit) {
  if (a.n_tiles <= 0) return hipSuccess;
  const unsigned fix_blocks = (unsigned)(a.n_tiles < kFixGrid ? a.n_tiles : kFixGrid);
  if (is == MGPU_H3) {
    hipLaunchKernelGGL(pip_join_kernel<MGPU_H3>, dim3((unsigned)a.n_tiles), dim3(kBlock), 0, s, a);
    if (after_stream) hipEventRecord(after_stream, s);
    hipLaunchKernelGGL(pip_fix_kernel<MGPU_H3>, dim3(fix_blocks), dim3(kBlock), 0, s, a);
  } else {
    hipLaunchKernelGGL(pip_join_kernel<MGPU_BNG>, dim3((unsigned)a.n_tiles), dim3(kBlock), 0, s, a);
    if (after_stream) hipEventRecord(after_stream, s);
    hipLaunchKernelGGL(pip_fix_kernel<MGPU_BNG>, dim3(fix_blocks), dim3(kBlock), 0, s, a);
  }
  hipLaunchKernelGGL(tile_scan_kernel, dim3(1), dim3(kScanBlock), 0, s, a.group_sum, a.group_cand,
                     (a.n_tiles + kScanGroup - 1) / kScanGroup, e.group_off, a.counters);
  if (emit)
    hipLaunchKernelGGL(pair_emit_kernel, dim3((unsigned)((a.n_tiles + kEmitTiles - 1) / kEmitTiles)),
                       dim3(kEmitBlock), 0, s, e, a.n_tiles);
  return hipGetLastError();
}

__global__ __launch_bounds__(256) void tile_unpair_kernel(JoinArgs a, RedoArgs R, int64_t n) {
  const int64_t i = (int64_t)blockIdx.x * 256 + threadIdx.x;
  if (i >= n) return;
  const uint32_t tile = R.list[i];
  const uint32_t c = a.tile_count[tile];
  R.old[i] = c;
  if (c) atomicSub(&a.group_sum[tile / kScanGroup], c);
  a.tile_count[tile] = 0;
  a.tile_where[tile] = kNoDst;
  R.affected[tile] = 1;
  a.dirty[i] = tile;
}

__global__ __launch_bounds__(256) void chunk_unpair_kernel(JoinArgs a, RedoArgs R) {
  __shared__ uint32_t s_w[4];
  const uint32_t chunk = R.list[blockIdx.x];
  const uint32_t nm = a.chunk_mixed[chunk];
  uint32_t mine = 0;
  for (uint32_t i = threadIdx.x; i < nm; i += 256) mine += __popc((uint32_t)(a.mixed_res[(int64_t)chunk * kChunk + i] >> 32));
  mine = wave_sum_u32(mine);
  if ((threadIdx.x & 63) == 0) s_w[threadIdx.x >> 6] = mine;
  __syncthreads();
  if (threadIdx.x == 0) {
    const uint32_t tot = s_w[0] + s_w[1] + s_w[2] + s_w[3];
    R.old[blockIdx.x] = a.group_sum[chunk];
    a.group_sum[chunk] -= tot;
    a.group_cand[chunk] = 0;
    R.affected[chunk] = 1;
    const uint32_t nt = (nm + kGTile - 1) / kGTile;
    const uint32_t q = atomicAdd(a.n_dirty, nt);
    for (uint32_t t = 0; t < nt; t++) a.dirty[q + t] = chunk * kChunkTiles + t;
  }
}

__global__ __launch_bounds__(256) void redo_compare_kernel(const uint32_t* counts, RedoArgs R, int64_t n) {
  const int64_t i = (int64_t)blockIdx.x * 256 + threadIdx.x;
  if (i < n && counts[R.list[i]] != R.old[i]) {
    atomicOr(R.changed, 1u);
    atomicMin(R.first, R.list[i]);
  }
}

hipError_t launch_join_redo(int is, const JoinArgs& a, const EmitArgs& e, const RedoArgs& R, int64_t n, hipStream_t s,
                            bool emit) {
  if (n <= 0) return hipSuccess;
  const unsigned g = (unsigned)((n + 255) / 256);
  hipLaunchKernelGGL(tile_unpair_kernel, dim3(g), dim3(256), 0, s, a, R, n);
  const unsigned fix_blocks = (unsigned)(n < kFixGrid ? n : kFixGrid);
  if (is == MGPU_H3)
    hipLaunchKernelGGL(pip_fix_kernel<MGPU_H3>, dim3(fix_blocks), dim3(kBlock), 0, s, a);
  else
    hipLaunchKernelGGL(pip_fix_kernel<MGPU_BNG>, dim3(fix_blocks), dim3(kBlock), 0, s, a);
  hipLaunchKernelGGL(redo_compare_kernel, dim3(g), dim3(256), 0, s, (const uint32_t*)a.tile_count, R, n);
  hipLaunchKernelGGL(tile_scan_kernel, dim3(1), dim3(kScanBlock), 0, s, a.group_sum, a.group_cand,
                     (a.n_tiles + kScanGroup - 1) / kScanGroup, e.group_off, a.counters, (const uint32_t*)R.changed);
  EmitArgs er = e;
  er.redo_first = R.first;
  er.redo_affected = R.affected;
  if (emit)
    hipLaunchKernelGGL(pair_emit_kernel, dim3((unsigned)((a.n_tiles + kEmitTiles - 1) / kEmitTiles)),
                       dim3(kEmitBlock), 0, s, er, a.n_tiles);
  return hipGetLastError();
}

int64_t split_chunk() { return kChunk; }
int64_t split_chunk_tiles() { return kChunkTiles; }
int64_t split_chunks(int64_t n) { return (n + kChunk - 1) / kChunk; }

static int resident_blocks(const void* kernel, int block, size_t lds) {
  int dev = 0, cus = 0, per = 0;
  hipGetDevice(&dev);
  hipDeviceGetAttribute(&cus, hipDeviceAttributeMultiprocessorCount, dev);
  if (hipOccupancyMaxActiveBlocksPerMultiprocessor(&per, kernel, block, lds) != hipSuccess || per < 1) per = 1;
  return std::max(cus, 1) * per;
}

template <int IS>
static void launch_emit(const SplitArgs& a, int64_t nc, hipStream_t s) {
  const size_t lds = IS == MGPU_H3 ? (size_t)emit_cls_staged(a.j.chips) * 4 : 0;
  hipLaunchKernelGGL(split_emit_kernel<IS>, dim3((unsigned)nc), dim3(kClsBlock), lds, s, a);
}

template <int IS>
static void launch_split_t(const SplitArgs& a, hipStream_t s, hipEvent_t after_classify, hipEvent_t after_mixed, bool emit) {
  const int64_t nc = split_chunks(a.j.n);
  const ChipTableView& ct = a.j.chips;
  const size_t nblk = (IS == MGPU_H3 && ct.raster_blk) ? (size_t)ct.raster_bnx * ct.raster_bny : 0;
  const size_t lds = IS == MGPU_H3 ? ((nblk + 1) & ~(size_t)1) * 2 + (size_t)ct.raster_nband * 4 : 0;
  const int64_t wg = (nc + kCfyBlock / 64 - 1) / (kCfyBlock / 64);
  if (lds > 64 * 1024) {
    hipFuncSetAttribute((const void*)classify_pair_kernel<IS>, hipFuncAttributeMaxDynamicSharedMemorySize, (int)lds);
    hipFuncSetAttribute((const void*)classify_wave_kernel<IS>, hipFuncAttributeMaxDynamicSharedMemorySize, (int)lds);
  }
  if (MGPU_CFY_PAIR && ((((uintptr_t)a.j.x) | ((uintptr_t)a.j.y)) & 15) == 0) {
    const int64_t grid = std::min<int64_t>(wg, (int64_t)resident_blocks((const void*)classify_pair_kernel<IS>, kCfyBlock, lds));
    hipLaunchKernelGGL(classify_pair_kernel<IS>, dim3((unsigned)grid), dim3(kCfyBlock), lds, s, a, nc);
  } else {
    const int64_t grid = std::min<int64_t>(wg, (int64_t)resident_blocks((const void*)classify_wave_kernel<IS>, kCfyBlock, lds));
    hipLaunchKernelGGL(classify_wave_kernel<IS>, dim3((unsigned)grid), dim3(kCfyBlock), lds, s, a, nc);
  }
  if (after_classify) hipEventRecord(after_classify, s);
  hipLaunchKernelGGL(pip_mixed_kernel<IS>, dim3((unsigned)nc), dim3(kBlock), 0, s, a.j);
  const int64_t more = std::min<int64_t>(nc, (int64_t)resident_blocks((const void*)pip_mixed_more_kernel<IS>, kBlock, 0));
  hipLaunchKernelGGL(pip_mixed_more_kernel<IS>, dim3((unsigned)more), dim3(kBlock), 0, s, a.j);
  const int64_t fix = nc * kChunkTiles < kFixGrid ? nc * kChunkTiles : kFixGrid;
  hipLaunchKernelGGL((pip_mixed_fix_kernel<IS, 2>), dim3((unsigned)fix), dim3(kBlock), 0, s, a.j);
  if (after_mixed) hipEventRecord(after_mixed, s);
  hipLaunchKernelGGL(tile_scan_kernel, dim3(1), dim3(kScanBlock), 0, s, a.chunk_pairs, a.j.group_cand, nc,
                     a.chunk_off, a.j.counters);
  if (emit) launch_emit<IS>(a, nc, s);
}

hipError_t launch_split(int is, const SplitArgs& a, hipStream_t s, hipEvent_t after_classify, hipEvent_t after_mixed,
                        bool emit) {
  if (a.j.n <= 0) return hipSuccess;
  if (is == MGPU_H3)
    launch_split_t<MGPU_H3>(a, s, after_classify, after_mixed, emit);
  else
    launch_split_t<MGPU_BNG>(a, s, after_classify, after_mixed, emit);
  return hipGetLastError();
}

hipError_t launch_split_redo(int is, const SplitArgs& sa, const RedoArgs& R, int64_t n, hipStream_t s, bool emit) {
  if (n <= 0) return hipSuccess;
  const int64_t nc = split_chunks(sa.j.n);
  hipLaunchKernelGGL(chunk_unpair_kernel, dim3((unsigned)n), dim3(256), 0, s, sa.j, R);
  const int64_t most = n * kChunkTiles;
  const unsigned fix = (unsigned)(most < kFixGrid ? most : kFixGrid);
  if (is == MGPU_H3)
    hipLaunchKernelGGL((pip_mixed_fix_kernel<MGPU_H3, 2>), dim3(fix), dim3(kBlock), 0, s, sa.j);
  else
    hipLaunchKernelGGL((pip_mixed_fix_kernel<MGPU_BNG, 2>), dim3(fix), dim3(kBlock), 0, s, sa.j);
  hipLaunchKernelGGL(redo_compare_kernel, dim3((unsigned)((n + 255) / 256)), dim3(256), 0, s,
                     (const uint32_t*)sa.chunk_pairs, R, n);
  hipLaunchKernelGGL(tile_scan_kernel, dim3(1), dim3(kScanBlock), 0, s, sa.chunk_pairs, sa.j.group_cand, nc,
                     sa.chunk_off, sa.j.counters, (const uint32_t*)R.changed);
  SplitArgs sr = sa;
  sr.redo_first = R.first;
  sr.redo_affected = R.affected;
  if (!emit) return hipGetLastError();
  if (is == MGPU_H3)
    launch_emit<MGPU_H3>(sr, nc, s);
  else
    launch_emit<MGPU_BNG>(sr, nc, s);
  return hipGetLastError();
}

hipError_t launch_split_emit(int is, const SplitArgs& a, hipStream_t s) {
  if (a.j.n <= 0) return hipSuccess;
  const int64_t nc = split_chunks(a.j.n);
  if (is == MGPU_H3)
    launch_emit<MGPU_H3>(a, nc, s);
  else
    launch_emit<MGPU_BNG>(a, nc, s);
  return hipGetLastError();
}

int64_t bin_chunk() { return kBinChunk; }
int64_t bin_chunks(int64_t n) { return (n + kBinChunk - 1) / kBinChunk; }
int64_t bin_groups(int64_t n) { return (bin_chunks(n) + kBinGroup - 1) / kBinGroup; }
int32_t bin_max() { return kBinMax; }

static void launch_bin_output(const BinArgs& a, hipStream_t s, bool emit) {
  const int64_t n = a.s.j.n, K = bin_chunks(n), nc = split_chunks(n);
  if (!MGPU_BIN_JOIN_COUNTS)
    hipLaunchKernelGGL(bin_gather_kernel, dim3((unsigned)K), dim3(kBinBlock), 0, s, a);
  hipLaunchKernelGGL(tile_scan_kernel, dim3(1), dim3(kScanBlock), 0, s, a.s.chunk_pairs, a.s.j.group_cand, nc,
                     a.s.chunk_off, a.s.j.counters);
  if (!emit) return;
  if (MGPU_BIN_JOIN_COUNTS)
    hipLaunchKernelGGL(bin_emit_gather_kernel, dim3((unsigned)K), dim3(kBinBlock), 0, s, a);
  else
    hipLaunchKernelGGL(bin_emit_kernel, dim3((unsigned)nc), dim3(kClsBlock), 0, s, a);
}

template <int IS>
static void launch_binned_t(const BinArgs& a, hipStream_t s, hipEvent_t after_bin, hipEvent_t after_join, bool emit) {
  const int64_t n = a.s.j.n, K = bin_chunks(n), G = bin_groups(n), nb = (int64_t)a.nbx * a.nby;
  hipLaunchKernelGGL(bin_hist_kernel, dim3((unsigned)K), dim3(kBinBlock), 0, s, a);
  hipLaunchKernelGGL(bin_colscan_kernel, dim3((unsigned)((nb + 255) / 256), (unsigned)G), dim3(256), 0, s, a, K);
  hipLaunchKernelGGL(bin_base_kernel, dim3(1), dim3(kBaseBlock), 0, s, a, G);
  if (IS == MGPU_H3 && a.key) {
    hipLaunchKernelGGL(bin_scatter_kernel<true>, dim3((unsigned)K), dim3(kBinBlock), 0, s, a);
  } else {
    hipLaunchKernelGGL(bin_scatter_kernel<false>, dim3((unsigned)K), dim3(kBinBlock), 0, s, a);
  }
  const int64_t nc = split_chunks(n), tiles = nc * kChunkTiles;
  JoinArgs j = a.s.j;
  if (MGPU_BIN_JOIN_COUNTS) {
    hipMemsetAsync(a.s.chunk_pairs, 0, (size_t)nc * sizeof(uint32_t), s);
    j.in_chunk_pairs = a.s.chunk_pairs;
  }
  if (after_bin) hipEventRecord(after_bin, s);
  const uint32_t per = a.xcd_runs ? (uint32_t)((tiles + 7) / 8) : 0u;
  const int64_t grid = per ? 8 * (int64_t)per : tiles;
  hipLaunchKernelGGL(pip_binned_kernel<IS>, dim3((unsigned)grid), dim3(kBlock), 0, s, j, per, (uint32_t)tiles);
  if (after_join) hipEventRecord(after_join, s);
  const int64_t fix = tiles < kFixGrid ? tiles : kFixGrid;
  hipLaunchKernelGGL((pip_mixed_fix_kernel<IS, 1>), dim3((unsigned)fix), dim3(kBlock), 0, s, j);
  launch_bin_output(a, s, emit);
}

hipError_t launch_binned(int is, const BinArgs& a, hipStream_t s, hipEvent_t after_bin, hipEvent_t after_join,
                         bool emit) {
  if (a.s.j.n <= 0) return hipSuccess;
  if (a.nbx < 1 || a.nby < 1 || (int64_t)a.nbx * a.nby > kBinMax) return hipErrorInvalidValue;
  if (is == MGPU_H3)
    launch_binned_t<MGPU_H3>(a, s, after_bin, after_join, emit);
  else
    launch_binned_t<MGPU_BNG>(a, s, after_bin, after_join, emit);
  return hipGetLastError();
}

hipError_t launch_bin_emit(const BinArgs& a, hipStream_t s) {
  if (a.s.j.n <= 0) return hipSuccess;
  if (MGPU_BIN_JOIN_COUNTS)
    hipLaunchKernelGGL(bin_emit_gather_kernel, dim3((unsigned)bin_chunks(a.s.j.n)), dim3(kBinBlock), 0, s, a);
  else
    hipLaunchKernelGGL(bin_emit_kernel, dim3((unsigned)split_chunks(a.s.j.n)), dim3(kClsBlock), 0, s, a);
  return hipGetLastError();
}

hipError_t launch_emit(const EmitArgs& e, int64_t n_tiles, hipStream_t s) {
  if (n_tiles <= 0) return hipSuccess;
  hipLaunchKernelGGL(pair_emit_kernel, dim3((unsigned)((n_tiles + kEmitTiles - 1) / kEmitTiles)), dim3(kEmitBlock), 0, s, e,
                     n_tiles);
  return hipGetLastError();
}

hipError_t launch_st_contains(const ChipTableView& t, const int64_t* row, const double* x, const double* y, int64_t n,
                              int8_t* out, unsigned long long* counters, hipStream_t s) {
  if (n <= 0) return hipSuccess;
  hipLaunchKernelGGL(st_contains_kernel, dim3((unsigned)((n + kStreamBlock - 1) / kStreamBlock)), dim3(kStreamBlock), 0, s, t, row, x,
                     y, n, out, counters);
  return hipGetLastError();
}

#include "count_kernels.inc"
#include "lookup_kernels.inc"

}
```

mosaic_amd/csrc/raster.h:

```cpp
#pragma once
#include <math.h>
#include <stdint.h>

#include "bng_core.h"
#include "chip_table.h"
#include "../../include/mosaic_gpu.h"

namespace mgpu {

constexpr uint32_t kNoPixel = 0xFFFFFFFFu;

MGPU_HDI bool pt_valid(const uint8_t* v, int64_t off, int64_t p) {
  if (!v) return true;
  const int64_t b = off + p;
  return (v[b >> 3] >> (b & 7)) & 1;
}

constexpr uint32_t kRasterFull = 0xFFFFFFFEu;
MGPU_HDI uint32_t div_fix(uint32_t v, uint32_t d, double inv) {
  const uint32_t q = (uint32_t)((double)v * inv);
  return q * d > v ? q - 1 : ((q + 1) * d <= v ? q + 1 : q);
}
template <int IS>
MGPU_HDI uint32_t raster_index(const ChipTableView& t, double px, double py, bool* ok, uint32_t* gi, uint32_t* sub,
                               uint32_t* blk = nullptr) {
  if (blk) *blk = kNoPixel;
  if (IS == MGPU_BNG) {
    *ok = px == px && py == py;
    if (!*ok) return kNoPixel;
    const int32_t eI = bng::d2i(px), nI = bng::d2i(py);
    if (!((uint32_t)eI < 10000000u && (uint32_t)nI < 10000000u)) return kRasterFull;
    const uint32_t col = div_fix((uint32_t)eI, t.raster_pix, t.raster_inv_dx);
    const uint32_t row = div_fix((uint32_t)nI, t.raster_pix, t.raster_inv_dy);
    const uint32_t ix = col - (uint32_t)t.raster_px0, iy = row - (uint32_t)t.raster_py0;
    if (ix >= t.raster_nx || iy >= t.raster_ny) return kNoPixel;
    if (t.raster_sub_n) {
      const double inv_w = 1.0 / (double)t.raster_sub_w;
      const uint32_t u = div_fix((uint32_t)eI - col * t.raster_pix, t.raster_sub_w, inv_w);
      const uint32_t v = div_fix((uint32_t)nI - row * t.raster_pix, t.raster_sub_w, inv_w);
      *sub = v * t.raster_sub_n + u;
    }
    const DenseFace& D = t.dense[0];
    *gi = D.base + (div_fix((uint32_t)nI, t.bng_edge, t.bng_inv_edge) - (uint32_t)D.b0) * D.w +
          (div_fix((uint32_t)eI, t.bng_edge, t.bng_inv_edge) - (uint32_t)D.a0);
    return iy * t.raster_nx + ix;
  }
  *ok = isfinite(px) && isfinite(py);
  if (!*ok || !(px >= t.bbox[0] && px <= t.bbox[2] && py >= t.bbox[1] && py <= t.bbox[3])) return kNoPixel;
  const double tx = (px - t.raster_x0) * t.raster_inv_dx, ty = (py - t.raster_y0) * t.raster_inv_dy;
  uint32_t ix = (uint32_t)tx, iy = (uint32_t)ty;
  ix = ix < t.raster_nx ? ix : t.raster_nx - 1;
  iy = iy < t.raster_ny ? iy : t.raster_ny - 1;
  if (blk && t.raster_bshift) *blk = (iy >> t.raster_bshift) * t.raster_bnx + (ix >> t.raster_bshift);
  if (t.raster_sub_n) {
    const double S = (double)t.raster_sub_n;
    uint32_t u = (uint32_t)((tx - (double)ix) * S), v = (uint32_t)((ty - (double)iy) * S);
    u = u < t.raster_sub_n ? u : t.raster_sub_n - 1;
    v = v < t.raster_sub_n ? v : t.raster_sub_n - 1;
    *sub = v * t.raster_sub_n + u;
    if (t.raster_band) *sub |= (iy >> t.raster_band_shift) << 16;
  }
  return iy * t.raster_nx + ix;
}

#ifndef MGPU_RANK_SPEC
#define MGPU_RANK_SPEC 0
#endif
MGPU_HDI uint32_t raster_class(const ChipTableView& t, uint32_t ri, uint32_t sub, const uint32_t* band = nullptr) {
  if (t.raster_band) {
    uint32_t cl = t.raster[ri];
    if (cl >= 0x8000u && cl != kPixMixed) {
      const uint64_t b = (uint64_t)(band ? band : t.raster_band)[sub >> 16] + (cl & 0x7FFFu);
      const uint32_t i = sub & 0xFFFFu, s2 = t.raster_sub_n * t.raster_sub_n;
      if (t.raster_pal) {
        const uint64_t P = t.raster_pal[b];
        const uint32_t q = t.raster_idx2[b * (s2 >> 2) + (i >> 2)];
        const uint32_t c = (uint32_t)(P >> (16 * ((q >> (2 * (i & 3))) & 3))) & 0x7FFFu;
        cl = (P & kPalFull) ? t.raster_sub[(P & 0xFFFFFFFFull) * s2 + i] : (c == 0x7FFFu ? kPixMixed : c);
      } else {
        cl = t.raster_sub[b * s2 + i];
      }
    }
    return cl;
  }
#if MGPU_RANK_SPEC
  const RankWord w = t.raster_rank ? t.raster_rank[ri >> 5] : RankWord{0u, 0u};
  uint32_t cl = t.raster[ri];
  if (cl == kPixMixed) {
#else
  uint32_t cl = t.raster[ri];
  if (cl == kPixMixed && t.raster_rank) {
    const RankWord w = t.raster_rank[ri >> 5];
#endif
    const uint32_t bit = 1u << (ri & 31);
    if (w.bits & bit) {
      const uint64_t b = (uint64_t)w.base + (uint64_t)__builtin_popcount(w.bits & (bit - 1));
      cl = t.raster_sub[b * t.raster_sub_n * t.raster_sub_n + sub];
    }
  }
  return cl;
}

MGPU_HDI uint32_t raster_class_blk(const ChipTableView& t, const uint16_t* blk_table, uint32_t ri, uint32_t bi,
                                   uint32_t sub, const uint32_t* band = nullptr) {
  const uint32_t c = bi != kNoPixel ? blk_table[bi] : kPixMixed;
  return c != kPixMixed ? c : raster_class(t, ri, sub, band);
}

}
```

Before: 114.3 billion.

## Add finer-grained uint8 block-class table in LDS for H3 classify kernels

Builds, at chip upload, a device table of 4x4, 8x4 or 4x8 raster-pixel blocks. Each entry holds a uint8 class when every pixel in the block agrees, otherwise a lookup marker. The classify kernels stage this table in LDS instead of the coarser uint16 block table, so more points resolve without reading the global raster. New 768-thread block variants with up to about 79 KB of LDS are enabled by default through the cfy_fine option. The larger LDS footprint may lower occupancy, and upload gains an extra kernel and synchronisation.

```diff
diff --git a/include/mosaic_gpu.h b/include/mosaic_gpu.h
--- a/include/mosaic_gpu.h
+++ b/include/mosaic_gpu.h
@@ -264,6 +264,8 @@
 int32_t mgpu_test_h3_cell_wkb_host(int64_t cell, uint8_t* out, int64_t cap, int64_t* out_len);
 int32_t mgpu_test_decode_point(int32_t format, const uint8_t* data, int64_t len, double* x, double* y);
 int32_t mgpu_test_join_counters(mgpu_ctx* ctx, uint64_t* out16);
+int32_t mgpu_test_fine_table(const mgpu_chips* chips, int64_t* dims, double* geom, uint16_t* out_classes,
+                             uint8_t* out_fine);
 int32_t mgpu_test_poly_slots_host(const int32_t* polygon_id, int64_t n, int32_t* out_ids, int64_t* out_n,
                                   uint32_t* out_slot_of_row);
 
diff --git a/mosaic_amd/_native.py b/mosaic_amd/_native.py
--- a/mosaic_amd/_native.py
+++ b/mosaic_amd/_native.py
@@ -37,7 +37,7 @@
     "mgpu_test_receive_blob", "mgpu_ring_join", "mgpu_ring_join_ex", "mgpu_ring_join_final",
     "mgpu_test_overlay_verify",
     "mgpu_chips_polygons", "mgpu_pip_join_count", "mgpu_test_poly_slots_host", "mgpu_chips_raster_info",
-    "mgpu_pip_join_lookup",
+    "mgpu_pip_join_lookup", "mgpu_test_fine_table",
     "mgpu_cell_agg_create", "mgpu_cell_agg_add_points", "mgpu_cell_agg_add_cells", "mgpu_cell_agg_add_counted",
     "mgpu_cell_agg_size", "mgpu_cell_agg_fetch", "mgpu_cell_agg_clear", "mgpu_cell_agg_destroy",
     "mgpu_cells_to_centers", "mgpu_cells_to_boundaries", "mgpu_cells_boundary_wkb", "mgpu_cells_area",
@@ -185,6 +185,7 @@
                                                   ctypes.POINTER(MgpuStats)]),
         "mgpu_test_internal_centroid": (I32, [I64, P, P, P, P, P, P, P, P]),
         "mgpu_test_join_counters": (I32, [P, P]),
+        "mgpu_test_fine_table": (I32, [P, P, P, P, P]),
         "mgpu_test_receive_blob": (I32, [P, P, I32, ctypes.POINTER(P)]),
         "mgpu_chips_polygons": (I32, [P, P, I64, ctypes.POINTER(I64)]),
         "mgpu_pip_join_count": (I32, [P, P, I32, I32, P, P, P, I64, I64, P, P, I32, P, ctypes.POINTER(MgpuStats)]),
diff --git a/mosaic_amd/chips.py b/mosaic_amd/chips.py
--- a/mosaic_amd/chips.py
+++ b/mosaic_amd/chips.py
@@ -78,6 +78,18 @@
         N.check(N.lib().mgpu_chips_raster_info(self.handle, ctypes.byref(m), ctypes.byref(k)))
         return {"chips": a.value, "cells": b.value, "vertices": c.value, "bytes": n, "raster_mode": m.value,
                 "raster_ncls": k.value}
+
+    def fine_table(self):
+        d, g = np.zeros(7, np.int64), np.zeros(8, np.float64)
+        N.check(N.lib().mgpu_test_fine_table(self.handle, d.ctypes.data, g.ctypes.data, None, None))
+        nx, ny, sx, sy, bnx, bny, built = (int(v) for v in d)
+        classes = np.zeros((ny, nx), np.uint16) if nx * ny else None
+        fine = np.zeros((bny, bnx), np.uint8) if built else None
+        N.check(N.lib().mgpu_test_fine_table(self.handle, d.ctypes.data, None,
+                                             None if classes is None else classes.ctypes.data,
+                                             None if fine is None else fine.ctypes.data))
+        return {"classes": classes, "sx": sx, "sy": sy, "fine": fine, "x0": g[0], "y0": g[1], "inv_dx": g[2],
+                "inv_dy": g[3], "bbox": tuple(g[4:])}
 
     def polygons(self):
         if getattr(self, "_polygons", None) is not None:
diff --git a/mosaic_amd/csrc/capi.cpp b/mosaic_amd/csrc/capi.cpp
--- a/mosaic_amd/csrc/capi.cpp
+++ b/mosaic_amd/csrc/capi.cpp
@@ -287,6 +287,9 @@
   } else if (k == "bng_split") {
     if (v != 0 && v != 1) return bad();
     o.bng_split = v;
+  } else if (k == "cfy_fine") {
+    if (v != 0 && v != 1) return bad();
+    o.cfy_fine = v;
   } else if (k == "count_lds_slots") {
     if (v < 0 || v > mgpu::kCountLdsSlotsMax) return bad();
     o.count_lds_slots = v;
@@ -339,7 +342,7 @@
       {"h3_libm", o.h3_libm},       {"pipeline", o.pipeline}, {"bin_count", o.bin_count},
       {"bin_min_mb", o.bin_min_mb}, {"bin_min_points", o.bin_min_points}, {"bin_xcd", o.bin_xcd},
       {"bin_keys", o.bin_keys},     {"spin_us", o.spin_us},   {"ring_batch", o.ring_batch},       {"raster", o.raster},     {"raster_bng", o.raster_bng},
-      {"bng_split", o.bng_split},   {"count_lds_slots", o.count_lds_slots}, {"count_groups", o.count_groups},
+      {"bng_split", o.bng_split},   {"cfy_fine", o.cfy_fine}, {"count_lds_slots", o.count_lds_slots}, {"count_groups", o.count_groups},
       {"kring_batch", o.kring_batch}, {"cellagg_groups", o.cellagg_groups}, {"cellagg_lds", o.cellagg_lds}, {"cellagg_bin_min", o.cellagg_bin_min},
       {"raster_sub", o.raster_sub}, {"raster_milli", o.raster_milli}, {"polyfill_slab", o.polyfill_slab},
       {"geomring_slab", o.geomring_slab}, {"geomring_lds_slots", o.geomring_lds_slots}};
@@ -561,6 +564,21 @@
   ch->index_system = hdr.index_system;
   ch->view = view_from_header(hdr, (uint8_t*)ch->blob);
   ch->n_vertices = hdr.n_vertices;
+  uint32_t sx = 0, sy = 0, bnx = 0, bny = 0;
+  if (ch->index_system == MGPU_H3 && fine_table_shape(ch->view, &sx, &sy, &bnx, &bny)) {
+    void* fine = nullptr;
+    hipError_t e = hipMalloc(&fine, ((size_t)bnx * bny + 3) & ~(size_t)3);
+    if (e == hipSuccess) e = launch_fine_table(ch->view, sx, sy, bnx, bny, (uint8_t*)fine, nullptr);
+    if (e == hipSuccess) e = hipStreamSynchronize(nullptr);
+    if (e != hipSuccess) {
+      if (fine) hipFree(fine);
+      delete ch;
+      return fail(MGPU_E_DEVICE, "fine block table: %s", hipGetErrorString(e));
+    }
+    ch->fine = fine;
+    ch->view.raster_fine = (const uint8_t*)fine;
+    ch->view.fine_sx = sx, ch->view.fine_sy = sy, ch->view.fine_bnx = bnx, ch->view.fine_bny = bny;
+  }
   *out = ch;
   return MGPU_OK;
 }
@@ -716,6 +734,7 @@
   if (!chips) return MGPU_OK;
   hipSetDevice(chips->device);
   if (chips->blob) hipFree(chips->blob);
+  if (chips->fine) hipFree(chips->fine);
   free_poly_slots(chips);
   delete chips;
   return MGPU_OK;
@@ -845,6 +864,7 @@
   a.res = res;
   a.res_match = (is == MGPU_BNG || chips->view.res < 0 || chips->view.res == res) ? 1 : 0;
   a.chips = chips->view;
+  if (!o.cfy_fine) a.chips.raster_fine = nullptr;
   a.counters = (unsigned long long*)base;
   a.pool_used = a.counters + 5;
   a.n_dirty = (uint32_t*)(a.counters + 6);
@@ -1729,6 +1749,26 @@
   return MGPU_OK;
 }
 
+int32_t mgpu_test_fine_table(const mgpu_chips* chips, int64_t* dims, double* geom, uint16_t* out_classes,
+                             uint8_t* out_fine) {
+  if (!chips || !dims) return fail(MGPU_E_INVALID_ARG, "bad arguments");
+  if (int32_t st = set_device(chips->device)) return st;
+  const mgpu::ChipTableView& v = chips->view;
+  const bool lonlat = v.raster_mode == mgpu::kRasterLonLat;
+  const int64_t d[7] = {lonlat ? v.raster_nx : 0, lonlat ? v.raster_ny : 0, v.fine_sx, v.fine_sy, v.fine_bnx, v.fine_bny,
+                        v.raster_fine ? 1 : 0};
+  memcpy(dims, d, sizeof d);
+  if (geom) {
+    const double g[8] = {v.raster_x0, v.raster_y0, v.raster_inv_dx, v.raster_inv_dy, v.bbox[0], v.bbox[1], v.bbox[2], v.bbox[3]};
+    memcpy(geom, g, sizeof g);
+  }
+  if (out_classes && d[0] * d[1])
+    HIP_TRY(hipMemcpy(out_classes, v.raster, (size_t)(d[0] * d[1]) * 2, hipMemcpyDeviceToHost));
+  if (out_fine && v.raster_fine)
+    HIP_TRY(hipMemcpy(out_fine, v.raster_fine, (size_t)(d[4] * d[5]), hipMemcpyDeviceToHost));
+  return MGPU_OK;
+}
+
 int32_t mgpu_test_internal_centroid(int64_t n, const int32_t* type_id, const int64_t* row_part, const int64_t* part_ring,
                                     const int64_t* ring_off, const double* xy, double* x, double* y, int32_t* status) {
   for (int64_t i = 0; i < n; i++)
diff --git a/mosaic_amd/csrc/capi_internal.h b/mosaic_amd/csrc/capi_internal.h
--- a/mosaic_amd/csrc/capi_internal.h
+++ b/mosaic_amd/csrc/capi_internal.h
@@ -26,6 +26,7 @@
   int64_t geomring_slab = (int64_t)1 << 16;
   int64_t geomring_lds_slots = 0;
   int64_t bng_split = 0;
+  int64_t cfy_fine = 1;
   int64_t raster = 1, raster_bng = 0, raster_sub = 16, raster_milli = 250;
 };
 
@@ -86,6 +87,7 @@
   mgpu::ChipTableView view{};
   int64_t n_vertices = 0;
   mutable void* slots = nullptr;
+  void* fine = nullptr;
 };
 
 namespace mgpu {
diff --git a/mosaic_amd/csrc/chip_build.cpp b/mosaic_amd/csrc/chip_build.cpp
--- a/mosaic_amd/csrc/chip_build.cpp
+++ b/mosaic_amd/csrc/chip_build.cpp
@@ -41,7 +41,7 @@
 
 namespace mgpu {
 mgpu::ChipTableView view_from_header(const BlobHeader& h, uint8_t* base) {
-  mgpu::ChipTableView v;
+  mgpu::ChipTableView v{};
   v.slots = (const mgpu::HashSlot*)(base + h.off[kArrSlots]);
   v.hash_mask = h.hash_mask;
   v.max_probe = h.max_probe;
diff --git a/mosaic_amd/csrc/chip_table.h b/mosaic_amd/csrc/chip_table.h
--- a/mosaic_amd/csrc/chip_table.h
+++ b/mosaic_amd/csrc/chip_table.h
@@ -121,7 +121,10 @@
   const uint8_t* raster_idx2;
   uint32_t raster_bshift, raster_bnx, raster_bny;
   const uint16_t* raster_blk;
+  uint32_t fine_sx, fine_sy, fine_bnx, fine_bny;
+  const uint8_t* raster_fine;
 };
+constexpr uint32_t kFineLookup = 0xFFu;
 
 enum RasterMode { kRasterNone = 0, kRasterLonLat = 1, kRasterBng = 2 };
 constexpr uint32_t kCellAnsChips = 15;
diff --git a/mosaic_amd/csrc/kernels.h b/mosaic_amd/csrc/kernels.h
--- a/mosaic_amd/csrc/kernels.h
+++ b/mosaic_amd/csrc/kernels.h
@@ -74,6 +74,9 @@
 hipError_t launch_split(int is, const SplitArgs& a, hipStream_t s, hipEvent_t after_classify, hipEvent_t after_mixed,
                         bool emit = true);
 hipError_t launch_split_emit(int is, const SplitArgs& a, hipStream_t s);
+bool fine_table_shape(const ChipTableView& t, uint32_t* sx, uint32_t* sy, uint32_t* bnx, uint32_t* bny);
+hipError_t launch_fine_table(const ChipTableView& t, uint32_t sx, uint32_t sy, uint32_t bnx, uint32_t bny, uint8_t* out,
+                             hipStream_t s);
 hipError_t launch_split_redo(int is, const SplitArgs& sa, const RedoArgs& R, int64_t n, hipStream_t s,
                              bool emit = true);
 
diff --git a/mosaic_amd/csrc/kernels.hip b/mosaic_amd/csrc/kernels.hip
--- a/mosaic_amd/csrc/kernels.hip
+++ b/mosaic_amd/csrc/kernels.hip
@@ -1140,7 +1140,7 @@
 #endif
 constexpr int kCfyBatch = MGPU_CFY_BATCH;
 
-template <int N>
+template <int N, bool FINE = false>
 __device__ __forceinline__ void raster_class_batch(const ChipTableView& t, const uint16_t* blk, const uint32_t* band,
                                                    const uint32_t (&ri)[N], const uint32_t (&bi)[N],
                                                    const uint32_t (&sub)[N], uint32_t (&cl)[N]) {
@@ -1149,12 +1149,13 @@
   bool pix[N], ref[N];
 #pragma unroll
   for (int k = 0; k < N; k++) {
-    c[k] = blk[bi[k] != kNoPixel ? bi[k] : 0u];
+    const uint32_t i = bi[k] != kNoPixel ? bi[k] : 0u;
+    c[k] = FINE ? (uint32_t)((const uint8_t*)blk)[i] : (uint32_t)blk[i];
     bb[k] = band[sub[k] >> 16];
   }
 #pragma unroll
   for (int k = 0; k < N; k++) {
-    pix[k] = ri[k] < kRasterFull && (bi[k] == kNoPixel || c[k] == kPixMixed);
+    pix[k] = ri[k] < kRasterFull && (bi[k] == kNoPixel || c[k] == (FINE ? kFineLookup : (uint32_t)kPixMixed));
     px[k] = t.raster[pix[k] ? ri[k] : 0u];
   }
 #pragma unroll
@@ -1168,9 +1169,20 @@
     cl[k] = ri[k] >= kRasterFull ? (ri[k] == kRasterFull ? kPixMixed : kPixEmpty) : ref[k] ? q[k] : pix[k] ? px[k] : c[k];
 }
 
-__device__ __forceinline__ bool cfy_staged(const ChipTableView& t, uint32_t nblk) {
+__host__ __device__ __forceinline__ bool cfy_staged(const ChipTableView& t, uint32_t nblk) {
   return t.raster_blk && nblk && t.raster_band && t.raster_nband && !t.raster_pal && t.raster_sub && t.raster_sub_n &&
          t.raster_nx && t.raster_ny;
+}
+
+#ifndef MGPU_CFY_FINE_BLOCK
+#define MGPU_CFY_FINE_BLOCK 768
+#endif
+constexpr int kCfyFineBlock = MGPU_CFY_FINE_BLOCK;
+static_assert(kCfyFineBlock == 512 || kCfyFineBlock == 768, "the fine classify kernels' launch shapes");
+constexpr size_t kCfyFineLds = kCfyFineBlock == 512 ? 53 * 1024 : 79 * 1024;
+constexpr int kCfyFineWaves = kCfyFineBlock == 768 ? 6 : MGPU_CFY_WAVES;
+__host__ __device__ __forceinline__ size_t cfy_fine_lds(uint32_t nfine, uint32_t nband) {
+  return (((size_t)nfine + 3) & ~(size_t)3) + (size_t)nband * 4;
 }
 
 template <int IS, class F>
@@ -1188,24 +1200,28 @@
   }
 }
 
-template <int IS>
-__global__ __launch_bounds__(kCfyBlock) __attribute__((amdgpu_waves_per_eu(MGPU_CFY_WAVES))) void classify_wave_kernel(SplitArgs sa, int64_t n_chunks) {
+template <int IS, int BLOCK = kCfyBlock, bool FINE = false>
+__global__ __launch_bounds__(BLOCK) __attribute__((amdgpu_waves_per_eu(FINE ? kCfyFineWaves : MGPU_CFY_WAVES))) void classify_wave_kernel(SplitArgs sa, int64_t n_chunks) {
   using Code = typename CodeOf<IS>::T;
-  constexpr int kW = kCfyBlock / 64;
+  static_assert(!FINE || IS == MGPU_H3, "raster_fine is a lonlat table");
+  constexpr int kW = BLOCK / 64;
   constexpr int kItems = kChunk / 64;
   static_assert(kItems % kCfyBatch == 0, "MGPU_CFY_BATCH must divide the points per lane of a chunk");
   const JoinArgs& a = sa.j;
   const ChipTableView& t = a.chips;
   extern __shared__ uint16_t s_blk[];
   const int lane = threadIdx.x & 63, wave = threadIdx.x >> 6;
-  const bool use_blk = IS == MGPU_H3 && t.raster_blk != nullptr;
+  const bool use_blk = IS == MGPU_H3 && (FINE || t.raster_blk != nullptr);
   const bool bng_grid = IS == MGPU_BNG && t.raster_mode == kRasterNone;
-  const uint32_t nblk = use_blk ? t.raster_bnx * t.raster_bny : 0u;
-  uint32_t* s_band = (uint32_t*)(s_blk + ((nblk + 1) & ~1u));
-  if (use_blk)
-    for (uint32_t i = threadIdx.x; i < nblk; i += kCfyBlock) s_blk[i] = t.raster_blk[i];
+  const uint32_t nblk = use_blk ? (FINE ? t.fine_bnx * t.fine_bny : t.raster_bnx * t.raster_bny) : 0u;
+  uint32_t* s_band = FINE ? (uint32_t*)s_blk + ((nblk + 3) >> 2) : (uint32_t*)(s_blk + ((nblk + 1) & ~1u));
+  if (FINE) {
+    for (uint32_t i = threadIdx.x; i < ((nblk + 3) >> 2); i += BLOCK) ((uint32_t*)s_blk)[i] = ((const uint32_t*)t.raster_fine)[i];
+  } else if (use_blk) {
+    for (uint32_t i = threadIdx.x; i < nblk; i += BLOCK) s_blk[i] = t.raster_blk[i];
+  }
   if (IS == MGPU_H3)
-    for (uint32_t i = threadIdx.x; i < t.raster_nband; i += kCfyBlock) s_band[i] = t.raster_band[i];
+    for (uint32_t i = threadIdx.x; i < t.raster_nband; i += BLOCK) s_band[i] = t.raster_band[i];
   __syncthreads();
   Code* codes = (Code*)sa.codes;
   const unsigned long long below = (1ull << lane) - 1ull;
@@ -1241,7 +1257,7 @@
             const uint32_t m = bng_grid_class(a, pk, bx[k], by[k], &ok, &g_);
             ri[k] = m == kPixMixed ? kRasterFull : m;
           } else {
-            ri[k] = raster_index<IS>(t, bx[k], by[k], &ok, &g_, &s_, &b_);
+            ri[k] = raster_index<IS, FINE>(t, bx[k], by[k], &ok, &g_, &s_, &b_);
           }
           gix[k] = g_;
           sb[k] = s_;
@@ -1255,7 +1271,7 @@
 #define MGPU_CFY_ABLATE 0
 #endif
       if constexpr (kStaged) {
-        raster_class_batch<kCfyBatch>(t, s_blk, s_band, ri, bi, sb, cl);
+        raster_class_batch<kCfyBatch, FINE>(t, s_blk, s_band, ri, bi, sb, cl);
 #pragma unroll
         for (int k = 0; k < kCfyBatch; k++) ge[k] = 0ull;
       } else {
@@ -1326,7 +1342,12 @@
       }
     }
   };
-  cfy_dispatch<IS>(cfy_staged(t, nblk), a.valid != nullptr, run);
+  if constexpr (FINE) {
+    if (a.valid != nullptr) run(std::true_type{}, std::true_type{});
+    else run(std::true_type{}, std::false_type{});
+  } else {
+    cfy_dispatch<IS>(cfy_staged(t, nblk), a.valid != nullptr, run);
+  }
   count_wave(&a.counters[2], any_bad);
 }
 
@@ -1335,10 +1356,11 @@
 #define MGPU_CFY_PAIR 1
 #endif
 typedef double dbl2_t __attribute__((ext_vector_type(2)));
-template <int IS>
-__global__ __launch_bounds__(kCfyBlock) __attribute__((amdgpu_waves_per_eu(MGPU_CFY_WAVES))) void classify_pair_kernel(SplitArgs sa, int64_t n_chunks) {
+template <int IS, int BLOCK = kCfyBlock, bool FINE = false>
+__global__ __launch_bounds__(BLOCK) __attribute__((amdgpu_waves_per_eu(FINE ? kCfyFineWaves : MGPU_CFY_WAVES))) void classify_pair_kernel(SplitArgs sa, int64_t n_chunks) {
   using Code = typename CodeOf<IS>::T;
-  constexpr int kW = kCfyBlock / 64;
+  static_assert(!FINE || IS == MGPU_H3, "raster_fine is a lonlat table");
+  constexpr int kW = BLOCK / 64;
   constexpr int kPairItems = kChunk / 128;
   constexpr int kPB = kCfyBatch / 2 > 0 ? kCfyBatch / 2 : 1;
   constexpr int kPts = 2 * kPB;
@@ -1347,14 +1369,17 @@
   const ChipTableView& t = a.chips;
   extern __shared__ uint16_t s_blk[];
   const int lane = threadIdx.x & 63, wave = threadIdx.x >> 6;
-  const bool use_blk = IS == MGPU_H3 && t.raster_blk != nullptr;
+  const bool use_blk = IS == MGPU_H3 && (FINE || t.raster_blk != nullptr);
   const bool bng_grid = IS == MGPU_BNG && t.raster_mode == kRasterNone;
-  const uint32_t nblk = use_blk ? t.raster_bnx * t.raster_bny : 0u;
-  uint32_t* s_band = (uint32_t*)(s_blk + ((nblk + 1) & ~1u));
-  if (use_blk)
-    for (uint32_t i = threadIdx.x; i < nblk; i += kCfyBlock) s_blk[i] = t.raster_blk[i];
+  const uint32_t nblk = use_blk ? (FINE ? t.fine_bnx * t.fine_bny : t.raster_bnx * t.raster_bny) : 0u;
+  uint32_t* s_band = FINE ? (uint32_t*)s_blk + ((nblk + 3) >> 2) : (uint32_t*)(s_blk + ((nblk + 1) & ~1u));
+  if (FINE) {
+    for (uint32_t i = threadIdx.x; i < ((nblk + 3) >> 2); i += BLOCK) ((uint32_t*)s_blk)[i] = ((const uint32_t*)t.raster_fine)[i];
+  } else if (use_blk) {
+    for (uint32_t i = threadIdx.x; i < nblk; i += BLOCK) s_blk[i] = t.raster_blk[i];
+  }
   if (IS == MGPU_H3)
-    for (uint32_t i = threadIdx.x; i < t.raster_nband; i += kCfyBlock) s_band[i] = t.raster_band[i];
+    for (uint32_t i = threadIdx.x; i < t.raster_nband; i += BLOCK) s_band[i] = t.raster_band[i];
   __syncthreads();
   Code* codes = (Code*)sa.codes;
   const unsigned long long below = (1ull << lane) - 1ull;
@@ -1393,7 +1418,7 @@
             const uint32_t m = bng_grid_class(a, pj, X[j], Y[j], &ok, &g_);
             ri[j] = m == kPixMixed ? kRasterFull : m;
           } else {
-            ri[j] = raster_index<IS>(t, X[j], Y[j], &ok, &g_, &s_, &b_);
+            ri[j] = raster_index<IS, FINE>(t, X[j], Y[j], &ok, &g_, &s_, &b_);
           }
           gix[j] = g_;
           sb[j] = s_;
@@ -1404,7 +1429,7 @@
       uint32_t cl[kPts];
       uint64_t ge[kPts];
       if constexpr (kStaged) {
-        raster_class_batch<kPts>(t, s_blk, s_band, ri, bi, sb, cl);
+        raster_class_batch<kPts, FINE>(t, s_blk, s_band, ri, bi, sb, cl);
 #pragma unroll
         for (int j = 0; j < kPts; j++) ge[j] = 0ull;
       } else {
@@ -1481,7 +1506,12 @@
       }
     }
   };
-  cfy_dispatch<IS>(cfy_staged(t, nblk), a.valid != nullptr, run);
+  if constexpr (FINE) {
+    if (a.valid != nullptr) run(std::true_type{}, std::true_type{});
+    else run(std::true_type{}, std::false_type{});
+  } else {
+    cfy_dispatch<IS>(cfy_staged(t, nblk), a.valid != nullptr, run);
+  }
   count_wave(&a.counters[2], any_bad);
 }
 
@@ -2952,6 +2982,55 @@
   hipLaunchKernelGGL(split_emit_kernel<IS>, dim3((unsigned)nc), dim3(kClsBlock), lds, s, a);
 }
 
+__global__ __launch_bounds__(256) void fine_table_kernel(const uint16_t* raster, uint32_t nx, uint32_t ny, uint32_t sx,
+                                                         uint32_t sy, uint32_t bnx, uint32_t nfine, uint8_t* out) {
+  const uint32_t i = blockIdx.x * 256u + threadIdx.x;
+  if (i >= nfine) return;
+  const uint32_t x0 = (i % bnx) << sx, y0 = (i / bnx) << sy;
+  const uint32_t x1 = min(x0 + (1u << sx), nx), y1 = min(y0 + (1u << sy), ny);
+  const uint32_t c = raster[(size_t)y0 * nx + x0];
+  bool same = true;
+  for (uint32_t y = y0; y < y1; y++)
+    for (uint32_t x = x0; x < x1; x++) same = same && raster[(size_t)y * nx + x] == c;
+  out[i] = (uint8_t)(same && c < kFineLookup ? c : kFineLookup);
+}
+
+bool fine_table_shape(const ChipTableView& t, uint32_t* sx, uint32_t* sy, uint32_t* bnx, uint32_t* bny) {
+  if (t.raster_mode != kRasterLonLat || !cfy_staged(t, t.raster_bnx * t.raster_bny)) return false;
+  const uint32_t shapes[3][2] = {{2, 2}, {3, 2}, {2, 3}};
+  for (const auto& sh : shapes) {
+    const uint64_t nx = ((uint64_t)t.raster_nx + (1u << sh[0]) - 1) >> sh[0], ny = ((uint64_t)t.raster_ny + (1u << sh[1]) - 1) >> sh[1];
+    if (nx * ny > kCfyFineLds || cfy_fine_lds((uint32_t)(nx * ny), t.raster_nband) > kCfyFineLds) continue;
+    *sx = sh[0], *sy = sh[1], *bnx = (uint32_t)nx, *bny = (uint32_t)ny;
+    return true;
+  }
+  return false;
+}
+
+hipError_t launch_fine_table(const ChipTableView& t, uint32_t sx, uint32_t sy, uint32_t bnx, uint32_t bny, uint8_t* out,
+                             hipStream_t s) {
+  const uint32_t nfine = bnx * bny;
+  if (hipError_t e = hipMemsetAsync(out, (int)kFineLookup, ((size_t)nfine + 3) & ~(size_t)3, s)) return e;
+  hipLaunchKernelGGL(fine_table_kernel, dim3((nfine + 255) / 256), dim3(256), 0, s, t.raster, t.raster_nx, t.raster_ny, sx,
+                     sy, bnx, nfine, out);
+  return hipGetLastError();
+}
+
+static void launch_classify_fine(const SplitArgs& a, int64_t nc, hipStream_t s) {
+  const ChipTableView& ct = a.j.chips;
+  const size_t lds = cfy_fine_lds(ct.fine_bnx * ct.fine_bny, ct.raster_nband);
+  const int64_t wg = (nc + kCfyFineBlock / 64 - 1) / (kCfyFineBlock / 64);
+  auto go = [&](auto kernel) {
+    if (lds > 64 * 1024) hipFuncSetAttribute((const void*)kernel, hipFuncAttributeMaxDynamicSharedMemorySize, (int)lds);
+    const int64_t grid = std::min<int64_t>(wg, (int64_t)resident_blocks((const void*)kernel, kCfyFineBlock, lds));
+    hipLaunchKernelGGL(kernel, dim3((unsigned)grid), dim3(kCfyFineBlock), lds, s, a, nc);
+  };
+  if (MGPU_CFY_PAIR && ((((uintptr_t)a.j.x) | ((uintptr_t)a.j.y)) & 15) == 0)
+    go(classify_pair_kernel<MGPU_H3, kCfyFineBlock, true>);
+  else
+    go(classify_wave_kernel<MGPU_H3, kCfyFineBlock, true>);
+}
+
 template <int IS>
 static void launch_split_t(const SplitArgs& a, hipStream_t s, hipEvent_t after_classify, hipEvent_t after_mixed, bool emit) {
   const int64_t nc = split_chunks(a.j.n);
@@ -2959,11 +3038,14 @@
   const size_t nblk = (IS == MGPU_H3 && ct.raster_blk) ? (size_t)ct.raster_bnx * ct.raster_bny : 0;
   const size_t lds = IS == MGPU_H3 ? ((nblk + 1) & ~(size_t)1) * 2 + (size_t)ct.raster_nband * 4 : 0;
   const int64_t wg = (nc + kCfyBlock / 64 - 1) / (kCfyBlock / 64);
-  if (lds > 64 * 1024) {
+  const bool fine = IS == MGPU_H3 && ct.raster_fine;
+  if (!fine && lds > 64 * 1024) {
     hipFuncSetAttribute((const void*)classify_pair_kernel<IS>, hipFuncAttributeMaxDynamicSharedMemorySize, (int)lds);
     hipFuncSetAttribute((const void*)classify_wave_kernel<IS>, hipFuncAttributeMaxDynamicSharedMemorySize, (int)lds);
   }
-  if (MGPU_CFY_PAIR && ((((uintptr_t)a.j.x) | ((uintptr_t)a.j.y)) & 15) == 0) {
+  if (fine) {
+    launch_classify_fine(a, nc, s);
+  } else if (MGPU_CFY_PAIR && ((((uintptr_t)a.j.x) | ((uintptr_t)a.j.y)) & 15) == 0) {
     const int64_t grid = std::min<int64_t>(wg, (int64_t)resident_blocks((const void*)classify_pair_kernel<IS>, kCfyBlock, lds));
     hipLaunchKernelGGL(classify_pair_kernel<IS>, dim3((unsigned)grid), dim3(kCfyBlock), lds, s, a, nc);
   } else {
diff --git a/mosaic_amd/csrc/raster.h b/mosaic_amd/csrc/raster.h
--- a/mosaic_amd/csrc/raster.h
+++ b/mosaic_amd/csrc/raster.h
@@ -21,7 +21,7 @@
   const uint32_t q = (uint32_t)((double)v * inv);
   return q * d > v ? q - 1 : ((q + 1) * d <= v ? q + 1 : q);
 }
-template <int IS>
+template <int IS, bool FINE = false>
 MGPU_HDI uint32_t raster_index(const ChipTableView& t, double px, double py, bool* ok, uint32_t* gi, uint32_t* sub,
                                uint32_t* blk = nullptr) {
   if (blk) *blk = kNoPixel;
@@ -51,7 +51,11 @@
   uint32_t ix = (uint32_t)tx, iy = (uint32_t)ty;
   ix = ix < t.raster_nx ? ix : t.raster_nx - 1;
   iy = iy < t.raster_ny ? iy : t.raster_ny - 1;
-  if (blk && t.raster_bshift) *blk = (iy >> t.raster_bshift) * t.raster_bnx + (ix >> t.raster_bshift);
+  if (FINE) {
+    if (blk) *blk = (iy >> t.fine_sy) * t.fine_bnx + (ix >> t.fine_sx);
+  } else if (blk && t.raster_bshift) {
+    *blk = (iy >> t.raster_bshift) * t.raster_bnx + (ix >> t.raster_bshift);
+  }
   if (t.raster_sub_n) {
     const double S = (double)t.raster_sub_n;
     uint32_t u = (uint32_t)((tx - (double)ix) * S), v = (uint32_t)((ty - (double)iy) * S);
```

Result: faster. 118.3 billion, median of 6 (+3.5%).
